# pydata/sparse

Measured on AMD Instinct MI355X. Metric: GCXS x dense SpMM throughput (GFLOP/s), higher is better.
Workload: dtype f32; 1 GPU; GCXS(CSR) 1000000x10000 @ 0.01 (100000000 nnz, int32 idx) in 1 nnz-balanced row block(s) x dense 10000x128 fp32; world_size=1, rows_rank0=1000000, idx_dtype=int32, parallelism=row-block x1, mul_add=fma, nan_warning=deferred, prewarm_products=40, default_settings=NAN_WARNING="sync" (verdict read inside every product), kernel=spmm_tiled (cached block stream)

## Files before the change

sparse_amd/csrc/build.py:

```python
import concurrent.futures as cf
import glob
import os
import shutil
import subprocess
import sys

HERE = os.path.dirname(os.path.abspath(__file__))
PKG = os.path.dirname(HERE)
OUT_DIR = os.path.join(PKG, "_lib")
OBJ_DIR = os.path.join(OUT_DIR, "obj")
LIB = os.path.join(OUT_DIR, "libsparse_amd.so")
ARCH = "gfx950"
CXXFLAGS = [
    f"--offload-arch={ARCH}", "-O3", "-std=c++17", "-fPIC", "-ffp-contract=off",
    "-fno-gpu-rdc", "-Wall", "-Wno-unused-function", "-Wno-unused-variable",
]


def _hipcc():
    for c in (os.environ.get("HIPCC"), shutil.which("hipcc"), "/opt/rocm/bin/hipcc"):
        if c and os.path.exists(c):
            return c
    raise RuntimeError("hipcc not found (need ROCm to build libsparse_amd.so)")


def sources():
    return sorted(glob.glob(os.path.join(HERE, "*.hip")))


def _deps():
    return sorted(glob.glob(os.path.join(HERE, "*.h"))) + sorted(glob.glob(os.path.join(HERE, "*.inc"))) + [
        os.path.join(os.path.dirname(PKG), "include", "sparse_amd.h"), os.path.abspath(__file__)]


def is_stale():
    if not os.path.exists(LIB):
        return True
    t = os.path.getmtime(LIB)
    return any(os.path.getmtime(p) > t for p in sources() + _deps())


def _own_deps(src, obj):
    dep = obj[:-2] + ".d"
    if not os.path.exists(dep):
        return _deps()
    words = open(dep).read().replace("\\\n", " ").split()
    files = [w for w in words[1:] if not w.startswith("/opt/") and not w.startswith("/usr/")]
    if any(not os.path.exists(f) for f in files):
        return _deps()
    return files + [os.path.abspath(__file__)]


NO_SPILL = {"spmm_tiled.hip": "spmm_tiled_kernel"}


def _spills(remarks, needle):
    out, name, sg = [], None, 0
    for ln in remarks.splitlines():
        if "Function Name:" in ln:
            name = ln.split("Function Name:")[1].split()[0]
        elif "SGPRs Spill:" in ln:
            sg = int(ln.split("SGPRs Spill:")[1].split()[0])
        elif "VGPRs Spill:" in ln and name is not None:
            vg = int(ln.split("VGPRs Spill:")[1].split()[0])
            if needle in name and (sg or vg):
                out.append((name, sg, vg))
    return out


def _compile(src, force):
    obj = os.path.join(OBJ_DIR, os.path.basename(src)[:-4] + ".o")
    newest = max(os.path.getmtime(p) for p in [src] + _own_deps(src, obj))
    if not force and os.path.exists(obj) and os.path.getmtime(obj) >= newest:
        return obj, ""
    needle = NO_SPILL.get(os.path.basename(src))
    extra = ["-Rpass-analysis=kernel-resource-usage"] if needle else []
    cmd = [_hipcc(), *CXXFLAGS, *extra, "-MD", "-MF", obj[:-2] + ".d", "-c", src, "-o", obj]
    r = subprocess.run(cmd, capture_output=True, text=True)
    if r.returncode != 0:
        raise RuntimeError(f"hipcc failed for {src}:\n{' '.join(cmd)}\n{r.stdout}\n{r.stderr}")
    if needle:
        bad = _spills(r.stderr, needle)
        if bad:
            os.remove(obj)
            raise RuntimeError(f"{os.path.basename(src)}: the compiler spilled registers in " +
                               ", ".join(f"{n[:60]} ({s} SGPR, {v} VGPR)" for n, s, v in bad[:4]) +
                               " - refused (see NO_SPILL in sparse_amd/csrc/build.py)")
        return obj, "\n".join(ln for ln in r.stderr.splitlines() if "-Rpass-analysis" not in ln and "remark:" not in ln)
    return obj, r.stderr


def build(force=False, verbose=False, jobs=None):
    if not force and not is_stale():
        return LIB
    os.makedirs(OBJ_DIR, exist_ok=True)
    srcs = sources()
    jobs = jobs or min(len(srcs), os.cpu_count() or 1)
    with cf.ThreadPoolExecutor(max_workers=jobs) as ex:
        results = list(ex.map(lambda s: _compile(s, force), srcs))
    objs = [o for o, _ in results]
    if verbose:
        for _, w in results:
            if w.strip():
                print(w, file=sys.stderr)
    cmd = [_hipcc(), f"--offload-arch={ARCH}", "-shared", "-fPIC", "-o", LIB + ".tmp", *objs]
    r = subprocess.run(cmd, capture_output=True, text=True)
    if r.returncode != 0:
        raise RuntimeError(f"link failed:\n{' '.join(cmd)}\n{r.stdout}\n{r.stderr}")
    os.replace(LIB + ".tmp", LIB)
    return LIB


if __name__ == "__main__":
    p = build(force="--force" in sys.argv, verbose=True)
    print(p)
```

sparse_amd/csrc/spmm_tiled.hip:

```cpp
#include "common.h"
#include "spmm_tiled_asm.inc"
#include <stdlib.h>
#include <mutex>
#include <set>

namespace spamd {

constexpr int TL_RG = TL_ASM_RG;
constexpr int TL_WAVES = TL_ASM_WAVES;
#ifndef SPAMD_TL_EXPERIMENTAL
static_assert(TL_RG == 35 && TL_WAVES == 16, "experimental tiled-SpMM geometry: build with -DSPAMD_TL_EXPERIMENTAL");
#endif
constexpr int TL_KB = TL_ASM_KB;
constexpr int TL_NBUF = 2;
__host__ __device__ constexpr int tl_d0(int lc, int lr) { return ((lc >> 1) << 11) | ((lc & 1) << 9) | (2 + 2 * lr); }
constexpr int TL_BLOCK_INTS = 16;

template <typename T>
struct TlFmt;
template <>
struct TlFmt<float> {
  static constexpr int EPB = 8, PANEL = 128;
  __device__ static void put(int* stream, int64_t entry, int d0, float v) {
    int* b = stream + (entry / EPB) * TL_BLOCK_INTS + (entry % EPB) * 2;
    typedef int int2v __attribute__((ext_vector_type(2)));
    int2v e;
    e.x = d0;
    e.y = __builtin_bit_cast(int, v);
    *reinterpret_cast<int2v*>(b) = e;
  }
};
template <>
struct TlFmt<double> {
  static constexpr int EPB = 5, PANEL = 64;
  __device__ static void put(int* stream, int64_t entry, int d0, double v) {
    int* b = stream + (entry / EPB) * TL_BLOCK_INTS;
    const int slot = (int)(entry % EPB);
    const long long bits = __builtin_bit_cast(long long, v);
    b[slot] = d0;
    if (slot == 0) b[5] = 0;
    *reinterpret_cast<long long*>(b + 6 + 2 * slot) = bits;
  }
};
typedef int tl_srd_t __attribute__((ext_vector_type(4)));
constexpr int TL_TILE = TL_KB * 512;
constexpr int TL_LDS = TL_NBUF * TL_TILE;
constexpr int TL_DMA_PER_TILE = TL_TILE / 16 / (TL_WAVES * 64);
static_assert(TL_LDS <= 160 * 1024 && TL_KB % (2 * TL_WAVES) == 0 && TL_DMA_PER_TILE == TL_ASM_DMA_PER_TILE,
              "tile geometry is baked into gen_tiled_asm.py");
constexpr int TL_SLACK_BLOCKS = 68;

#define GRID_STRIDE(i, n)                                                          \
  for (int64_t i = (int64_t)blockIdx.x * blockDim.x + threadIdx.x; i < (n);        \
       i += (int64_t)gridDim.x * blockDim.x)

__global__ void __launch_bounds__(256) tl_keys_kernel(const int64_t* __restrict__ rc_keys, int64_t nnz, int64_t K,
                                                      int64_t ntiles, int64_t* __restrict__ out) {
  GRID_STRIDE(i, nnz) {
    const int64_t k = rc_keys[i];
    const int64_t row = k / K, col = k - row * K;
    const int64_t g = row / TL_RG, lr = row - g * TL_RG, t = col / TL_KB, lc = col - t * TL_KB;
    out[i] = ((g * ntiles + t) * TL_RG + lr) * TL_KB + lc;
  }
}

__global__ void __launch_bounds__(256) tl_seg_start_kernel(const int64_t* __restrict__ keys, int64_t nnz,
                                                           int64_t nseg, int64_t* __restrict__ seg_start) {
  GRID_STRIDE(i, nnz + 1) {
    const int64_t hi = i < nnz ? keys[i] / (TL_RG * TL_KB) : nseg;
    const int64_t lo = i > 0 ? keys[i - 1] / (TL_RG * TL_KB) + 1 : 0;
    for (int64_t s = lo; s <= hi; ++s) seg_start[s] = i;
  }
}

__global__ void __launch_bounds__(256) tl_blocks_kernel(const int64_t* __restrict__ seg_start, int64_t nseg, int epb,
                                                        int64_t* __restrict__ nblk) {
  GRID_STRIDE(s, nseg + 1) {
    nblk[s] = s < nseg ? (seg_start[s + 1] - seg_start[s] + epb - 1) / epb : 0;
  }
}

template <typename T>
__global__ void __launch_bounds__(256) tl_pack_kernel(const int64_t* __restrict__ keys, const T* __restrict__ vals,
                                                      int64_t nnz, const int64_t* __restrict__ seg_start,
                                                      const int64_t* __restrict__ blk_off, int* __restrict__ stream) {
  GRID_STRIDE(i, nnz) {
    const int64_t k = keys[i];
    const int64_t lc = k % TL_KB, r1 = k / TL_KB, lr = r1 % TL_RG, s = r1 / TL_RG;
    const int64_t dst = blk_off[s] * TlFmt<T>::EPB + (i - seg_start[s]);
    TlFmt<T>::put(stream, dst, tl_d0((int)lc, (int)lr), vals[i]);
  }
}

constexpr int TL_DIRECT_MAX_TILES = 256;

template <typename I>
__device__ __forceinline__ int tl_row_of(const int64_t* rs, int64_t e) {
  static_assert(TL_RG <= 128, "seven bisection steps");
  int lo = 0, hi = TL_RG;
#pragma unroll
  for (int it = 0; it < (TL_RG <= 64 ? 6 : 7); ++it) {
    const int mid = (lo + hi) >> 1;
    if (hi - lo > 1) {
      if (rs[mid] <= e) lo = mid; else hi = mid;
    }
  }
  return lo;
}

template <typename I>
__global__ void __launch_bounds__(256) tl_count_kernel(int64_t M, int ntiles, int epb, const I* __restrict__ indices,
                                                       const I* __restrict__ indptr, int64_t* __restrict__ nblk,
                                                       int* __restrict__ flags) {
  __shared__ int cnt[TL_DIRECT_MAX_TILES];
  __shared__ int64_t rs[TL_RG + 1];
  const int tid = threadIdx.x;
  const int64_t r0 = (int64_t)blockIdx.x * TL_RG;
  if (tid <= TL_RG) {
    const int64_t r = r0 + tid;
    rs[tid] = (int64_t)indptr[r < M ? r : M];
  }
  for (int t = tid; t < ntiles; t += 256) cnt[t] = 0;
  __syncthreads();
  const int64_t e0 = rs[0], e1 = rs[TL_RG];
  bool bad = false;
  for (int64_t e = e0 + tid; e < e1; e += 256) {
    const int64_t c = (int64_t)indices[e];
    atomicAdd(&cnt[(int)(c / TL_KB)], 1);
    if (e > e0 && (int64_t)indices[e - 1] > c && rs[tl_row_of<I>(rs, e)] != e) bad = true;
  }
  if (bad) flags[0] = 1;
  __syncthreads();
  for (int t = tid; t < ntiles; t += 256) nblk[(int64_t)blockIdx.x * ntiles + t] = (cnt[t] + epb - 1) / epb;
}

template <typename I, typename T>
__global__ void __launch_bounds__(256) tl_fill_kernel(int64_t M, int ntiles, const T* __restrict__ vals,
                                                      const I* __restrict__ indices, const I* __restrict__ indptr,
                                                      const int64_t* __restrict__ blk_off, int* __restrict__ stream) {
  extern __shared__ int tl_fill_lds[];
  __shared__ int64_t rs[TL_RG + 1];
  int* const before = tl_fill_lds;
  int* const runstart = before + TL_RG * ntiles;
  const int tid = threadIdx.x;
  const int64_t r0 = (int64_t)blockIdx.x * TL_RG;
  if (tid <= TL_RG) {
    const int64_t r = r0 + tid;
    rs[tid] = (int64_t)indptr[r < M ? r : M];
  }
  for (int i = tid; i < TL_RG * ntiles; i += 256) before[i] = 0;
  __syncthreads();
  const int64_t e0 = rs[0], e1 = rs[TL_RG];
  for (int64_t e = e0 + tid; e < e1; e += 256) {
    const int t = (int)((int64_t)indices[e] / TL_KB);
    const int lr = tl_row_of<I>(rs, e);
    atomicAdd(&before[lr * ntiles + t], 1);
    if (e == rs[lr] || (int)((int64_t)indices[e - 1] / TL_KB) != t) runstart[lr * ntiles + t] = (int)(e - e0);
  }
  __syncthreads();
  for (int t = tid; t < ntiles; t += 256) {
    int run = 0;
    for (int lr = 0; lr < TL_RG; ++lr) {
      const int c = before[lr * ntiles + t];
      before[lr * ntiles + t] = run;
      run += c;
    }
  }
  __syncthreads();
  const int64_t* const goff = blk_off + (int64_t)blockIdx.x * ntiles;
  for (int64_t e = e0 + tid; e < e1; e += 256) {
    const int64_t c = (int64_t)indices[e];
    const int t = (int)(c / TL_KB), lc = (int)(c - (int64_t)t * TL_KB);
    const int lr = tl_row_of<I>(rs, e);
    const int64_t dst = goff[t] * TlFmt<T>::EPB + before[lr * ntiles + t] + ((int)(e - e0) - runstart[lr * ntiles + t]);
    TlFmt<T>::put(stream, dst, tl_d0(lc, lr), vals[e]);
  }
}

__host__ __device__ inline int64_t tl_group_first_block(int64_t e0, int64_t g, int64_t ntiles, int64_t epb) {
  return (e0 + g * ntiles * (epb - 1) + epb - 1) / epb;
}

template <typename I, typename T, bool MAPPED>
__global__ void __launch_bounds__(256) tl_inspect_kernel(int64_t M, int ntiles, int64_t groups, const T* __restrict__ vals,
                                                         const I* __restrict__ indices, const I* __restrict__ indptr,
                                                         unsigned long long* __restrict__ state, int* __restrict__ blk_off,
                                                         int* __restrict__ stream, const int* __restrict__ rowmap,
                                                         const int64_t* __restrict__ vstart) {
  extern __shared__ int tl_fill_lds[];
  __shared__ __attribute__((aligned(16))) int64_t rsab[2 * (TL_RG + 1)];
  __shared__ int wtot[5];
  __shared__ int group_bad;
  constexpr int EPB = TlFmt<T>::EPB;
  int* const before = tl_fill_lds;
  int* const runstart = before + TL_RG * ntiles;
  int* const loff = runstart + TL_RG * ntiles;
  const int tid = threadIdx.x;
  const int64_t g = blockIdx.x;
  const int64_t r0 = g * TL_RG;
  if (tid < TL_RG) {
    if constexpr (MAPPED) {
      const int r = rowmap[r0 + tid];
      rsab[2 * (tid)] = r >= 0 ? (int64_t)indptr[r] : 0;
      rsab[2 * (tid) + 1] = r >= 0 ? (int64_t)indptr[r + 1] : 0;
    } else {
      const int64_t r = r0 + tid;
      rsab[2 * (tid)] = (int64_t)indptr[r < M ? r : M];
      rsab[2 * (tid) + 1] = (int64_t)indptr[r + 1 < M ? r + 1 : M];
    }
  }
  for (int i = tid; i < TL_RG * ntiles; i += 256) before[i] = 0;
  if (tid == 0) group_bad = 0;
  __syncthreads();
  const int64_t e0 = MAPPED ? vstart[g] : rsab[2 * (0)], e1 = MAPPED ? vstart[g + 1] : rsab[2 * (TL_RG - 1) + 1];
  bool bad = false;
  constexpr int RPW = (TL_RG + 3) / 4;
  constexpr int TL_PRE = 2;
  const int wv = tid >> 6, lane = tid & 63;
  unsigned cpre[RPW][TL_PRE];
  T vpre[RPW][TL_PRE];
#pragma unroll
  for (int i = 0; i < RPW; ++i) {
    const int lr = wv + 4 * i;
    const int64_t ra = lr < TL_RG ? rsab[2 * (lr)] : 0, rb = lr < TL_RG ? rsab[2 * (lr) + 1] : 0;
#pragma unroll
    for (int p = 0; p < TL_PRE; ++p) {
      const int64_t e = ra + lane + 64 * p;
      cpre[i][p] = e < rb ? (unsigned)indices[e] : 0xffffffffu;
      vpre[i][p] = e < rb ? vals[e] : T(0);
    }
  }
  auto count_one = [&](int lr, int64_t ra, int64_t e, unsigned c, unsigned cp, bool row_start) {
    const int t = (int)(c / (unsigned)TL_KB);
    atomicAdd(&before[lr * ntiles + t], 1);
    if (!row_start && cp > c) bad = true;
    if (row_start || (int)(cp / (unsigned)TL_KB) != t) runstart[lr * ntiles + t] = (int)(e - (MAPPED ? ra : e0));
  };
#pragma unroll
  for (int i = 0; i < RPW; ++i) {
    const int lr = wv + 4 * i;
    if (lr >= TL_RG) break;
    const int64_t ra = rsab[2 * (lr)], rb = rsab[2 * (lr) + 1];
#pragma unroll
    for (int p = 0; p < TL_PRE; ++p) {
      const int64_t e = ra + lane + 64 * p;
      const unsigned c = cpre[i][p];
      unsigned cp = (unsigned)__shfl_up((int)c, 1, 64);
      if (p > 0) {
        const unsigned last = (unsigned)__builtin_amdgcn_readlane((int)cpre[i][p > 0 ? p - 1 : 0], 63);
        if (lane == 0) cp = last;
      }
      if (e < rb) count_one(lr, ra, e, c, cp, p == 0 && lane == 0);
    }
    for (int64_t e = ra + lane + 64 * TL_PRE; e < rb; e += 64)
      count_one(lr, ra, e, (unsigned)indices[e], (unsigned)indices[e - 1], false);
  }
  if (bad) {
    atomicOr(&state[0], 1ull);
    group_bad = 1;
  }
  __syncthreads();
  int nb = 0, cnt_t = 0;
  for (int t = tid; t < ntiles; t += 256) {
    int c[TL_RG];
#pragma unroll
    for (int lr = 0; lr < TL_RG; ++lr) c[lr] = before[lr * ntiles + t];
    int run = 0;
#pragma unroll
    for (int lr = 0; lr < TL_RG; ++lr) {
      before[lr * ntiles + t] = run;
      run += c[lr];
    }
    cnt_t = run;
    nb = (run + EPB - 1) / EPB;
  }
  const int wid = wv;
  int x = nb;
#pragma unroll
  for (int d = 1; d < 64; d <<= 1) {
    const int y = __shfl_up(x, d, 64);
    if (lane >= d) x += y;
  }
  if (lane == 63) wtot[wid] = x;
  __syncthreads();
  int woff = 0;
  for (int w = 0; w < wid; ++w) woff += wtot[w];
  const int gtotal = wtot[0] + wtot[1] + wtot[2] + wtot[3];
  const int my_off = woff + x - nb;
  const int64_t goff = tl_group_first_block(e0, g, ntiles, EPB);
  const int64_t gnext = tl_group_first_block(e1, g + 1, ntiles, EPB);
  if (tid < ntiles) loff[tid] = my_off;
  __syncthreads();
  if (tid < ntiles) blk_off[g * (ntiles + 1) + tid] = (int)(goff + my_off);
  if (tid == 0) blk_off[g * (ntiles + 1) + ntiles] = (int)(goff + gtotal);
  for (int64_t i = (goff + gtotal) * TL_BLOCK_INTS + tid; i < gnext * TL_BLOCK_INTS; i += 256) stream[i] = 0;
  if (group_bad) {
    for (int64_t i = goff * TL_BLOCK_INTS + tid; i < (goff + gtotal) * TL_BLOCK_INTS; i += 256) stream[i] = 0;
    return;
  }
  auto fill_one = [&](int lr, int64_t ra, int64_t e, unsigned c, T v) {
    const int t = (int)(c / (unsigned)TL_KB);
    const int lc = (int)(c - (unsigned)t * (unsigned)TL_KB);
    const int64_t dst = (goff + loff[t]) * EPB + before[lr * ntiles + t] + ((int)(e - (MAPPED ? ra : e0)) - runstart[lr * ntiles + t]);
    TlFmt<T>::put(stream, dst, tl_d0(lc, lr), v);
  };
#pragma unroll
  for (int i = 0; i < RPW; ++i) {
    const int lr = wv + 4 * i;
    if (lr >= TL_RG) break;
    const int64_t ra = rsab[2 * (lr)], rb = rsab[2 * (lr) + 1];
#pragma unroll
    for (int p = 0; p < TL_PRE; ++p) {
      const int64_t e = ra + lane + 64 * p;
      if (e < rb) fill_one(lr, ra, e, cpre[i][p], vpre[i][p]);
    }
    for (int64_t e = ra + lane + 64 * TL_PRE; e < rb; e += 64) fill_one(lr, ra, e, (unsigned)indices[e], vals[e]);
  }
  if (tid < ntiles) {
    const int64_t first = (goff + my_off) * EPB;
    for (int i = cnt_t; i < nb * EPB; ++i) TlFmt<T>::put(stream, first + i, 0, T(0));
  }
}

__device__ __forceinline__ void tl_dma16(unsigned lds_base, const void* src) {
  asm volatile("s_mov_b32 m0, %0\n\ts_nop 0\n\tglobal_load_lds_dwordx4 %1, off"
               :
               : "s"(lds_base), "v"(src)
               : "memory", "m0");
}

template <int MODE>
__device__ __forceinline__ void tl_phases(const int* stream, int t0, int te, int o0, int o1, int o2, int offreg, int obase,
                                          int ntiles, int nfull, int toff, int mask, unsigned m0wave,
                                          unsigned row_step, int voff, tl_srd_t srd, unsigned& soff) {
  const int lane = threadIdx.x & 63;
  const unsigned blo = (unsigned)((uintptr_t)stream & 0xffffffffu), bhi = (unsigned)((uintptr_t)stream >> 32);
  const int lane8 = lane * 8;
#define TL_PHASES_OPERANDS                                                                                        \
  [soff] "+s"(soff)                                                                                               \
  : [blo] "s"(blo), [bhi] "s"(bhi), [t0] "s"(t0), [te] "s"(te), [o0] "s"(o0), [o1] "s"(o1), [o2] "s"(o2),         \
    [obase] "s"(obase), [ntiles] "s"(ntiles), [nfull] "s"(nfull), [m0wave] "s"(m0wave), [step] "s"(row_step),      \
    [toff] "v"(toff), [lane8] "v"(lane8), [mask] "v"(mask), [offreg] "v"(offreg), [voff] "v"(voff), [srd] "s"(srd)  \
  : "memory", "m0", "scc", "vcc", TL_CLOB_SGPR, TL_CLOB_TMP, TL_CLOB_ACC
  if (MODE == 6)
    asm volatile(TL_ASM_PHASES_I32 : TL_PHASES_OPERANDS);
  else if (MODE == 4)
    asm volatile(TL_ASM_PHASES_F64 : TL_PHASES_OPERANDS);
  else if (MODE == 5)
    asm volatile(TL_ASM_PHASES_F64_EXACT : TL_PHASES_OPERANDS);
  else if (MODE == 3)
    asm volatile(TL_ASM_PHASES_EXACT : TL_PHASES_OPERANDS);
  else if (MODE == 1)
    asm volatile(TL_ASM_PHASES_NOFMA : TL_PHASES_OPERANDS);
  else if (MODE == 2)
    asm volatile(TL_ASM_PHASES_NOLDS : TL_PHASES_OPERANDS);
  else
    asm volatile(TL_ASM_PHASES : TL_PHASES_OPERANDS);
#undef TL_PHASES_OPERANDS
}

__device__ __forceinline__ void tl_block_map(unsigned L, int npanels, int nblocks, int& bx, int& by) {
  const unsigned pin = npanels > 1 ? 2u : 1u;
  const unsigned per_chunk = (unsigned)((nblocks + 7) / 8) * 8u * pin;
  const unsigned chunk = L / per_chunk, l = L % per_chunk;
  const unsigned seq = l >> 3;
  by = uniform((int)(chunk * pin + seq % pin));
  bx = uniform((int)((seq / pin) * 8u + (l & 7u)));
}

template <int DBG, int MODE, typename T>
__global__ void __launch_bounds__(TL_WAVES * 64) __attribute__((amdgpu_num_vgpr(TL_ASM_COMP)))
spmm_tiled_kernel(int64_t M, int64_t K, int ntiles, int touch_lines, const int* __restrict__ stream,
                  const int* __restrict__ blk_off, const T* __restrict__ b, int64_t ldb,
                  T* __restrict__ out, int64_t ldo, int last_cols, int npanels, int nblocks, const int* __restrict__ rowmap) {
  constexpr int PANEL = TlFmt<T>::PANEL;
  constexpr int CPL = PANEL / 64;
  extern __shared__ __attribute__((aligned(16))) char lds[];
  const int tid = threadIdx.x;
  const int lane = tid & 63;
  const int wv = uniform(tid >> 6);
  int bx, by;
  tl_block_map(blockIdx.x, npanels, nblocks, bx, by);
  if (bx >= nblocks || by >= npanels) return;
  const int g = bx * TL_WAVES + wv;
  b += (int64_t)by * PANEL;
  out += (int64_t)by * PANEL;

  asm volatile(TL_ASM_ZERO ::: "memory", TL_CLOB_ACC);

  const int nfull = DBG == 2 ? 0 : (int)(K / TL_KB);
  const unsigned row_step = (unsigned)((2 * TL_WAVES) * ldb * (int64_t)sizeof(T));
  const unsigned m0wave = (unsigned)wv * 2048u;
  const uint64_t bbase = (uint64_t)(uintptr_t)b;
  tl_srd_t srd;
  srd[0] = (int)(bbase & 0xffffffffu);
  srd[1] = (int)((bbase >> 32) & 0xffffu);
  srd[2] = (int)0xffffffffu;
  srd[3] = 0x00020000;
  const int voff = (int)((int64_t)(tid >> 5) * ldb * (int64_t)sizeof(T)) + (tid & 31) * 16;
  unsigned soff = 0;
  auto issue_partial = [&](int t) {
#pragma unroll
    for (int i = 0; i < TL_DMA_PER_TILE; ++i) {
      const int e = (i * (TL_WAVES * 64) + tid) * 16;
      int64_t r = (int64_t)t * TL_KB + (e >> 9);
      if (r >= K) r = K - 1;
      tl_dma16(((unsigned)(i * TL_WAVES + wv) * 2u + (unsigned)(t & 1)) * 1024u,
               reinterpret_cast<const char*>(b + r * ldb) + (e & 511));
    }
  };
  const bool has_partial = DBG != 2 && (int64_t)nfull * TL_KB < K;

  if (nfull > 0)
    asm volatile(TL_ASM_TILE0 : [soff] "+s"(soff) : [m0wave] "s"(m0wave), [step] "s"(row_step), [voff] "v"(voff), [srd] "s"(srd) : "memory", "m0", "scc", "vcc", "s89");
  else if (has_partial)
    issue_partial(0);
  asm volatile("s_waitcnt vmcnt(0)" ::: "memory");
  __syncthreads();

  const int* const myoff = blk_off + (int64_t)g * (ntiles + (touch_lines >> 16));
  touch_lines &= 0xffff;
  const int toff = (lane < touch_lines ? lane : touch_lines - 1) * 64;
  int t = 0;
  while (t < ntiles) {
    const int obase = t;
    const int q = obase + lane;
    int offreg = myoff[q < ntiles ? q : ntiles];
    asm volatile("" : "+v"(offreg));
    int te = obase + 61 < ntiles ? obase + 61 : ntiles;
    if (has_partial && t < nfull - 1 && nfull - 1 < te) te = nfull - 1;
    if (has_partial && t == nfull - 1) issue_partial(nfull);
    auto o = [&](int tt) { return wave_bcast(offreg, (tt < ntiles ? tt : ntiles) - obase); };
    const int o0 = o(t), o1 = o(t + 1), o2 = o(t + 2);
    if (t == 0) {
      const int n = o2 - o0, l = lane < n ? lane : 0;
      asm volatile("global_load_dword " TL_ASM_TOUCH ", %0, off" ::"v"(reinterpret_cast<const char*>(stream + (int64_t)o0 * 16) + l * 64)
                   : "memory", TL_ASM_TOUCH);
    }
    tl_phases<MODE>(stream, t, te, o0, o1, o2, offreg, obase, ntiles, nfull, toff, (int)0xfffffe00, m0wave, row_step, voff, srd, soff);
    t = te;
  }
  asm volatile("s_waitcnt vmcnt(0) lgkmcnt(0)" ::: "memory");

  const int64_t row0 = (int64_t)g * TL_RG;
  const int64_t left = M - row0;
  const int nvalid = left <= 0 ? 0 : (left < TL_RG ? (int)left : TL_RG);
  T* const obase_p = out + row0 * ldo + lane * CPL;
  const int64_t stride_bytes = ldo * (int64_t)sizeof(T);
  int bx2, by2;
  tl_block_map(blockIdx.x, npanels, nblocks, bx2, by2);
  const int ncols = (last_cols > 0 && by2 == npanels - 1) ? last_cols : PANEL;
  if (rowmap) {
    const int* const rm = rowmap + (int64_t)g * TL_RG;
    T* const base_p = out + lane * CPL;
    if (lane * CPL + CPL <= ncols)
      asm volatile(TL_ASM_STORE_PERM
                   :
                   : [lo] "v"((unsigned)((uintptr_t)base_p & 0xffffffffu)), [hi] "v"((unsigned)((uintptr_t)base_p >> 32)),
                     [stride] "s"((unsigned)stride_bytes), [rm] "s"(rm)
                   : "memory", "scc", TL_CLOB_SGPR, TL_CLOB_TMP, TL_CLOB_ACC);
    if constexpr (CPL == 2) {
      if (lane * CPL + 1 == ncols)
        asm volatile(TL_ASM_STORE1_PERM
                     :
                     : [lo] "v"((unsigned)((uintptr_t)base_p & 0xffffffffu)), [hi] "v"((unsigned)((uintptr_t)base_p >> 32)),
                       [stride] "s"((unsigned)stride_bytes), [rm] "s"(rm)
                     : "memory", "scc", TL_CLOB_SGPR, TL_CLOB_TMP);
    }
    return;
  }
  if (lane * CPL + CPL <= ncols)
    asm volatile(TL_ASM_STORE
                 :
                 : [lo] "v"((unsigned)((uintptr_t)obase_p & 0xffffffffu)), [hi] "v"((unsigned)((uintptr_t)obase_p >> 32)),
                   [stride] "s"(stride_bytes), [n] "s"(nvalid)
                 : "memory", "scc", "s36", TL_ASM_BASE, TL_ASM_TOUCH, TL_CLOB_ACC);
  if constexpr (CPL == 2) {
    if (lane * CPL + 1 == ncols)
      asm volatile(TL_ASM_STORE1
                   :
                   : [lo] "v"((unsigned)((uintptr_t)obase_p & 0xffffffffu)), [hi] "v"((unsigned)((uintptr_t)obase_p >> 32)),
                     [stride] "s"(stride_bytes), [n] "s"(nvalid)
                   : "memory", "scc", "s36", TL_ASM_BASE, TL_ASM_TOUCH);
  }
}

static int64_t tl_grid_groups(int64_t M) { return ceil_div(ceil_div(M, (int64_t)TL_RG), (int64_t)TL_WAVES) * TL_WAVES; }

}

using namespace spamd;

static int tl_epb(int val_dtype) { return val_dtype == SPAMD_F32 ? TlFmt<float>::EPB : (val_dtype == SPAMD_F64 ? TlFmt<double>::EPB : 0); }

extern "C" int spamd_spmm_tiled_params(int val_dtype, int* rows_per_group, int* tile_rows, int* groups_per_block,
                                       int* entries_per_block, int* slack_blocks, int* direct_max_tiles,
                                       int* panel_cols) {
  if (!tl_epb(val_dtype)) return SPAMD_ETYPE;
  if (direct_max_tiles) *direct_max_tiles = TL_DIRECT_MAX_TILES;
  if (rows_per_group) *rows_per_group = TL_RG;
  if (tile_rows) *tile_rows = TL_KB;
  if (groups_per_block) *groups_per_block = TL_WAVES;
  if (entries_per_block) *entries_per_block = tl_epb(val_dtype);
  if (slack_blocks) *slack_blocks = TL_SLACK_BLOCKS;
  if (panel_cols) *panel_cols = val_dtype == SPAMD_F32 ? TlFmt<float>::PANEL : TlFmt<double>::PANEL;
  return 0;
}

static unsigned tl_blocks_for(int64_t n) {
  int64_t blocks = ceil_div(n, (int64_t)256);
  if (blocks > 8192) blocks = 8192;
  if (blocks < 1) blocks = 1;
  return (unsigned)blocks;
}

extern "C" int spamd_spmm_tiled_keys(int64_t nnz, const int64_t* rowcol_keys, int64_t K, int64_t* tiled_keys,
                                     void* stream) {
  if (nnz < 0 || K <= 0) return SPAMD_EINVAL;
  if (nnz == 0) return 0;
  hipLaunchKernelGGL(tl_keys_kernel, dim3(tl_blocks_for(nnz)), dim3(256), 0, (hipStream_t)stream, rowcol_keys, nnz, K,
                     ceil_div(K, (int64_t)TL_KB), tiled_keys);
  return launch_status();
}

extern "C" int spamd_spmm_tiled_lists(int val_dtype, int64_t nnz, const int64_t* tiled_keys_sorted, int64_t M, int64_t K,
                                      int64_t* seg_start, int64_t* nblk, void* stream) {
  if (nnz < 0 || M < 0 || K <= 0) return SPAMD_EINVAL;
  if (!tl_epb(val_dtype)) return SPAMD_ETYPE;
  const int64_t nseg = tl_grid_groups(M) * ceil_div(K, (int64_t)TL_KB);
  hipLaunchKernelGGL(tl_seg_start_kernel, dim3(tl_blocks_for(nnz + 1)), dim3(256), 0, (hipStream_t)stream,
                     tiled_keys_sorted, nnz, nseg, seg_start);
  hipLaunchKernelGGL(tl_blocks_kernel, dim3(tl_blocks_for(nseg + 1)), dim3(256), 0, (hipStream_t)stream, seg_start,
                     nseg, tl_epb(val_dtype), nblk);
  return launch_status();
}

static int tl_clear_blocks(int64_t total_blocks, int* blocks, hipStream_t s) {
  return (int)hipMemsetAsync(blocks, 0, (size_t)(total_blocks + TL_SLACK_BLOCKS) * TL_BLOCK_INTS * sizeof(int), s);
}

extern "C" int spamd_spmm_tiled_pack(int val_dtype, int64_t nnz, const int64_t* tiled_keys_sorted, const void* vals_sorted,
                                     const int64_t* seg_start, const int64_t* blk_off, int64_t total_blocks,
                                     int* blocks, void* stream) {
  if (nnz < 0 || total_blocks < 0) return SPAMD_EINVAL;
  if (!tl_epb(val_dtype)) return SPAMD_ETYPE;
  int rc = tl_clear_blocks(total_blocks, blocks, (hipStream_t)stream);
  if (rc) return rc;
  if (nnz == 0) return 0;
  if (val_dtype == SPAMD_F32)
    hipLaunchKernelGGL(tl_pack_kernel<float>, dim3(tl_blocks_for(nnz)), dim3(256), 0, (hipStream_t)stream, tiled_keys_sorted,
                       (const float*)vals_sorted, nnz, seg_start, blk_off, blocks);
  else
    hipLaunchKernelGGL(tl_pack_kernel<double>, dim3(tl_blocks_for(nnz)), dim3(256), 0, (hipStream_t)stream, tiled_keys_sorted,
                       (const double*)vals_sorted, nnz, seg_start, blk_off, blocks);
  return launch_status();
}

extern "C" int spamd_spmm_tiled_count(int val_dtype, int idx_dtype, int64_t M, int64_t K, const void* a_indices,
                                      const void* a_indptr, int64_t* nblk, int* flags, void* stream) {
  if (M < 0 || K <= 0) return SPAMD_EINVAL;
  if (!tl_epb(val_dtype)) return SPAMD_ETYPE;
  const int64_t ntiles = ceil_div(K, (int64_t)TL_KB);
  if (ntiles > TL_DIRECT_MAX_TILES) return SPAMD_EINVAL;
  const int64_t groups = tl_grid_groups(M);
  hipError_t e = hipMemsetAsync(flags, 0, sizeof(int), (hipStream_t)stream);
  if (e != hipSuccess) return (int)e;
  e = hipMemsetAsync(nblk + groups * ntiles, 0, sizeof(int64_t), (hipStream_t)stream);
  if (e != hipSuccess) return (int)e;
  if (groups == 0) return 0;
  SPAMD_DISPATCH_IDX(idx_dtype, I, hipLaunchKernelGGL(tl_count_kernel<I>, dim3((unsigned)groups), dim3(256), 0,
                                                    (hipStream_t)stream, M, (int)ntiles, tl_epb(val_dtype),
                                                    (const I*)a_indices, (const I*)a_indptr, nblk, flags))
  return launch_status();
}

template <typename I, typename T>
static int tl_launch_fill(int64_t M, int64_t ntiles, const T* a_data, const I* a_indices, const I* a_indptr,
                          const int64_t* blk_off, int* blocks, hipStream_t s) {
  const int lds = (int)(2 * TL_RG * ntiles * sizeof(int));
  auto kern = &tl_fill_kernel<I, T>;
  if (lds > 48 * 1024) {
    hipError_t e = hipFuncSetAttribute(reinterpret_cast<const void*>(kern), hipFuncAttributeMaxDynamicSharedMemorySize, lds);
    if (e != hipSuccess) return (int)e;
  }
  hipLaunchKernelGGL(kern, dim3((unsigned)tl_grid_groups(M)), dim3(256), lds, s, M, (int)ntiles, a_data, a_indices, a_indptr,
                     blk_off, blocks);
  return launch_status();
}

extern "C" int spamd_spmm_tiled_fill(int val_dtype, int idx_dtype, int64_t M, int64_t K, const void* a_data,
                                     const void* a_indices, const void* a_indptr, const int64_t* blk_off,
                                     int64_t total_blocks, int* blocks, void* stream) {
  if (M < 0 || K <= 0 || total_blocks < 0) return SPAMD_EINVAL;
  if (!tl_epb(val_dtype)) return SPAMD_ETYPE;
  const int64_t ntiles = ceil_div(K, (int64_t)TL_KB);
  if (ntiles > TL_DIRECT_MAX_TILES) return SPAMD_EINVAL;
  int rc = tl_clear_blocks(total_blocks, blocks, (hipStream_t)stream);
  if (rc) return rc;
  if (tl_grid_groups(M) == 0) return 0;
  SPAMD_DISPATCH_IDX(idx_dtype, I, {
    if (val_dtype == SPAMD_F32)
      return tl_launch_fill<I, float>(M, ntiles, (const float*)a_data, (const I*)a_indices, (const I*)a_indptr, blk_off,
                                      blocks, (hipStream_t)stream);
    return tl_launch_fill<I, double>(M, ntiles, (const double*)a_data, (const I*)a_indices, (const I*)a_indptr, blk_off,
                                     blocks, (hipStream_t)stream);
  })
  return SPAMD_ETYPE;
}

template <typename I, typename T>
static int tl_launch_inspect(int64_t M, int64_t ntiles, const T* a_data, const I* a_indices, const I* a_indptr,
                             unsigned long long* state, int* blk_off, int* blocks, hipStream_t s, int64_t map_groups = 0,
                             const int* rowmap = nullptr, const int64_t* vstart = nullptr) {
  const int64_t groups = rowmap ? map_groups : tl_grid_groups(M);
  const int lds = (int)((2 * TL_RG * ntiles + ntiles + 1) * sizeof(int));
  auto kern = rowmap ? &tl_inspect_kernel<I, T, true> : &tl_inspect_kernel<I, T, false>;
  if (lds > 48 * 1024) {
    hipError_t e = hipFuncSetAttribute(reinterpret_cast<const void*>(kern), hipFuncAttributeMaxDynamicSharedMemorySize, lds);
    if (e != hipSuccess) return (int)e;
  }
  hipLaunchKernelGGL(kern, dim3((unsigned)groups), dim3(256), lds, s, M, (int)ntiles, groups, a_data, a_indices, a_indptr,
                     state, blk_off, blocks, rowmap, vstart);
  return launch_status();
}

constexpr int TL_MAP_CLASSES = 6;
__host__ __device__ inline int tl_map_slots(int c) { return c == 5 ? TL_RG : (1 << c); }
__host__ __device__ inline int tl_map_class(int64_t len, int64_t cap) {
  return len > cap / 2 ? 0 : (len > cap / 4 ? 1 : (len > cap / 8 ? 2 : (len > cap / 16 ? 3 : (len > cap / 32 ? 4 : 5))));
}

template <typename I>
__global__ void __launch_bounds__(256) tl_map_stats_kernel(int64_t M, int64_t cap, int64_t maxlen, const I* __restrict__ indptr,
                                                           int64_t* __restrict__ keys, int* __restrict__ rows,
                                                           unsigned long long* __restrict__ stats) {
  __shared__ unsigned cnt[TL_MAP_CLASSES];
  if (threadIdx.x < TL_MAP_CLASSES) cnt[threadIdx.x] = 0;
  __syncthreads();
  const int lane = threadIdx.x & 63;
  const int64_t stride = (int64_t)gridDim.x * blockDim.x;
  for (int64_t r0 = (int64_t)blockIdx.x * blockDim.x; r0 < M; r0 += stride) {
    const int64_t r = r0 + threadIdx.x;
    int c = -1;
    if (r < M) {
      const int64_t len = (int64_t)indptr[r + 1] - (int64_t)indptr[r];
      c = tl_map_class(len, cap);
      keys[r] = len < maxlen ? maxlen - len : 0;
      rows[r] = (int)r;
    }
#pragma unroll
    for (int k = 0; k < TL_MAP_CLASSES; ++k) {
      const unsigned long long m = __ballot(c == k);
      if (lane == 0 && m) atomicAdd(&cnt[k], (unsigned)__popcll(m));
    }
  }
  __syncthreads();
  if (threadIdx.x < TL_MAP_CLASSES && cnt[threadIdx.x]) atomicAdd(&stats[threadIdx.x], (unsigned long long)cnt[threadIdx.x]);
}

template <typename I>
__global__ void __launch_bounds__(256) tl_map_skew_kernel(int64_t M, const I* __restrict__ indptr,
                                                          unsigned long long* __restrict__ stats) {
  const int64_t groups = (M + TL_RG - 1) / TL_RG;
  unsigned long long mine = 0;
  GRID_STRIDE(g, groups) {
    const int64_t r = g * TL_RG, e = r + TL_RG < M ? r + TL_RG : M;
    const unsigned long long load = (unsigned long long)((int64_t)indptr[e] - (int64_t)indptr[r]);
    mine = load > mine ? load : mine;
  }
#pragma unroll
  for (int d = 32; d > 0; d >>= 1) {
    const unsigned long long y = __shfl_xor(mine, d, 64);
    mine = y > mine ? y : mine;
  }
  if ((threadIdx.x & 63) == 0 && mine) atomicMax(&stats[6], mine);
}

struct TlMapPlan {
  int64_t cstart[TL_MAP_CLASSES];
  int64_t gstart[TL_MAP_CLASSES];
};

template <typename I>
__global__ void __launch_bounds__(256) tl_map_build_kernel(int64_t M, int64_t cap, const I* __restrict__ indptr,
                                                           const int* __restrict__ rows_sorted, TlMapPlan plan,
                                                           int* __restrict__ rowmap, unsigned long long* __restrict__ gload) {
  GRID_STRIDE(i, M) {
    const int r = rows_sorted[i];
    const int64_t len = (int64_t)indptr[r + 1] - (int64_t)indptr[r];
    const int c = tl_map_class(len, cap);
    const int64_t j = i - plan.cstart[c];
    const int sl = tl_map_slots(c);
    const int64_t group = plan.gstart[c] + j / sl;
    rowmap[group * TL_RG + (int)(j % sl)] = r;
    if (len) atomicAdd(&gload[group], (unsigned long long)len);
  }
}

extern "C" int spamd_spmm_tiled_inspect(int val_dtype, int idx_dtype, int64_t M, int64_t K, const void* a_data,
                                        const void* a_indices, const void* a_indptr, void* state, int* blk_off, int* blocks,
                                        void* stream) {
  if (M < 0 || K <= 0) return SPAMD_EINVAL;
  if (!tl_epb(val_dtype)) return SPAMD_ETYPE;
  const int64_t ntiles = ceil_div(K, (int64_t)TL_KB);
  if (ntiles > TL_DIRECT_MAX_TILES) return SPAMD_EINVAL;
  const int64_t groups = tl_grid_groups(M);
  hipError_t e = hipMemsetAsync(state, 0, sizeof(unsigned long long), (hipStream_t)stream);
  if (e != hipSuccess) return (int)e;
  if (groups == 0) return 0;
  SPAMD_DISPATCH_IDX(idx_dtype, I, {
    if (val_dtype == SPAMD_F32)
      return tl_launch_inspect<I, float>(M, ntiles, (const float*)a_data, (const I*)a_indices, (const I*)a_indptr,
                                         (unsigned long long*)state, blk_off, blocks, (hipStream_t)stream);
    return tl_launch_inspect<I, double>(M, ntiles, (const double*)a_data, (const I*)a_indices, (const I*)a_indptr,
                                        (unsigned long long*)state, blk_off, blocks, (hipStream_t)stream);
  })
  return SPAMD_ETYPE;
}

extern "C" int spamd_spmm_tiled_map_stats(int idx_dtype, int64_t M, int64_t K, int64_t cap, const void* a_indptr, int64_t* keys,
                                          int* rows, int64_t* stats, void* stream) {
  if (M < 0 || M >= ((int64_t)1 << 31) || K <= 0 || cap < 32 || (cap & (cap - 1)) || (keys != nullptr) != (rows != nullptr) || !stats)
    return SPAMD_EINVAL;
  hipStream_t s = (hipStream_t)stream;
  if (hipError_t e = hipMemsetAsync(stats, 0, 8 * sizeof(int64_t), s); e != hipSuccess) return (int)e;
  if (M == 0) return 0;
  SPAMD_DISPATCH_IDX(idx_dtype, I, {
    hipLaunchKernelGGL((tl_map_skew_kernel<I>), dim3(tl_blocks_for(ceil_div(M, (int64_t)TL_RG))), dim3(256), 0, s, M, (const I*)a_indptr,
                       (unsigned long long*)stats);
    if (keys)
      hipLaunchKernelGGL((tl_map_stats_kernel<I>), dim3(tl_blocks_for(M)), dim3(256), 0, s, M, cap, K, (const I*)a_indptr, keys, rows,
                         (unsigned long long*)stats);
    return launch_status();
  })
  return SPAMD_ETYPE;
}

extern "C" int64_t spamd_spmm_tiled_map_groups(const int64_t* class_counts) {
  if (!class_counts) return -1;
  int64_t g = 0;
  for (int c = 0; c < TL_MAP_CLASSES; ++c) {
    if (class_counts[c] < 0) return -1;
    g += ceil_div(class_counts[c], (int64_t)tl_map_slots(c));
  }
  return ceil_div(g, (int64_t)TL_WAVES) * TL_WAVES;
}

extern "C" int spamd_spmm_tiled_map_build(int idx_dtype, int64_t M, int64_t cap, const void* a_indptr, const int* rows_sorted,
                                          const int64_t* class_counts, int* rowmap, int64_t* gload, void* stream) {
  const int64_t groups = spamd_spmm_tiled_map_groups(class_counts);
  if (M < 0 || M >= ((int64_t)1 << 31) || groups <= 0 || !rowmap || !gload || !rows_sorted) return SPAMD_EINVAL;
  hipStream_t s = (hipStream_t)stream;
  if (hipError_t e = hipMemsetAsync(rowmap, 0xff, (size_t)(groups * TL_RG + 16) * sizeof(int), s); e != hipSuccess) return (int)e;
  if (hipError_t e = hipMemsetAsync(gload, 0, (size_t)(groups + 1) * sizeof(int64_t), s); e != hipSuccess) return (int)e;
  TlMapPlan plan;
  int64_t pos = 0, g = 0;
  for (int c = 0; c < TL_MAP_CLASSES; ++c) {
    plan.cstart[c] = pos;
    plan.gstart[c] = g;
    pos += class_counts[c];
    g += ceil_div(class_counts[c], (int64_t)tl_map_slots(c));
  }
  if (pos != M) return SPAMD_EINVAL;
  if (M == 0) return 0;
  SPAMD_DISPATCH_IDX(idx_dtype, I, {
    hipLaunchKernelGGL((tl_map_build_kernel<I>), dim3(tl_blocks_for(M)), dim3(256), 0, s, M, cap, (const I*)a_indptr, rows_sorted,
                       plan, rowmap, (unsigned long long*)gload);
    return launch_status();
  })
  return SPAMD_ETYPE;
}

extern "C" int spamd_spmm_tiled_inspect_mapped(int val_dtype, int idx_dtype, int64_t M, int64_t K, int64_t groups,
                                               const void* a_data, const void* a_indices, const void* a_indptr,
                                               const int* rowmap, const int64_t* vstart, void* state, int* blk_off, int* blocks,
                                               void* stream) {
  if (M < 0 || K <= 0 || groups <= 0 || groups % TL_WAVES || !rowmap || !vstart) return SPAMD_EINVAL;
  if (!tl_epb(val_dtype)) return SPAMD_ETYPE;
  const int64_t ntiles = ceil_div(K, (int64_t)TL_KB);
  if (ntiles > TL_DIRECT_MAX_TILES) return SPAMD_EINVAL;
  hipError_t e = hipMemsetAsync(state, 0, sizeof(unsigned long long), (hipStream_t)stream);
  if (e != hipSuccess) return (int)e;
  SPAMD_DISPATCH_IDX(idx_dtype, I, {
    if (val_dtype == SPAMD_F32)
      return tl_launch_inspect<I, float>(M, ntiles, (const float*)a_data, (const I*)a_indices, (const I*)a_indptr,
                                         (unsigned long long*)state, blk_off, blocks, (hipStream_t)stream, groups, rowmap, vstart);
    return tl_launch_inspect<I, double>(M, ntiles, (const double*)a_data, (const I*)a_indices, (const I*)a_indptr,
// ... 691 lines not shown
```

sparse_amd/csrc/spmm_tiled_asm.inc:

```

#define TL_ASM_KB 160
#define TL_ASM_DMA_PER_TILE 5
#define TL_ASM_RG 35
#define TL_ASM_WAVES 16
#define TL_ASM_COMP 22
#define TL_ASM_TOUCH "v23"
#define TL_ASM_BASE "v22"

#define TL_ASM_PHASES \
  "s_mov_b32 s39, 0\n\t" \
  "s_mov_b32 s90, %[t0]\n\t" \
  "s_mov_b32 s91, %[o0]\n\t" \
  "s_mov_b32 s92, %[o1]\n\t" \
  "s_mov_b32 s93, %[o2]\n\t" \
  "s_add_u32 s88, s90, 1\n\t" \
  "s_and_b32 s88, s88, 1\n\t" \
  "s_lshl_b32 s88, s88, 10\n\t" \
  "s_add_u32 s89, s88, %[m0wave]\n\t" \
  "s_and_b32 s88, s90, 1\n\t" \
  "s_lshl_b32 s88, s88, 10\n\t" \
  "v_or_b32 v22, s88, %[lane8]\n\t" \
  "s_lshl_b32 s36, s91, 6\n\t" \
  "s_lshr_b32 s37, s91, 26\n\t" \
  "s_add_u32 s36, s36, %[blo]\n\t" \
  "s_addc_u32 s37, s37, %[bhi]\n\t" \
  "s_sub_u32 s88, s92, s91\n\t" \
  "s_cmp_lt_u32 s88, 3\n\t" \
  "s_cbranch_scc1 22f\n\t" \
  "s_load_dwordx16 s[40:55], s[36:37], 0x0\n\t" \
  "s_load_dwordx16 s[56:71], s[36:37], 0x40\n\t" \
  "s_load_dwordx16 s[72:87], s[36:37], 0x80\n\t" \
  "20:\n\t" \
  "1:\n\t" \
  "s_sub_u32 s38, s92, s91\n\t" \
  "s_add_u32 s88, s90, 1\n\t" \
  "s_cmp_lt_u32 s88, %[nfull]\n\t" \
  "s_cselect_b64 vcc, 31, 0\n\t" \
  "s_cmp_eq_u32 s38, 0\n\t" \
  "s_cbranch_scc1 12f\n\t" \
  "s_cbranch_vccz 6f\n\t" \
  "s_mov_b32 m0, s89\n\t" \
  "s_add_u32 s89, s89, 0x8000\n\t" \
  "buffer_load_dwordx4 %[voff], %[srd], %[soff] offen lds\n\t" \
  "s_add_u32 %[soff], %[soff], %[step]\n\t" \
  "s_lshr_b64 vcc, vcc, 1\n\t" \
  "6:\n\t" \
  "s_cbranch_vccz 6f\n\t" \
  "s_mov_b32 m0, s89\n\t" \
  "s_add_u32 s89, s89, 0x8000\n\t" \
  "buffer_load_dwordx4 %[voff], %[srd], %[soff] offen lds\n\t" \
  "s_add_u32 %[soff], %[soff], %[step]\n\t" \
  "s_lshr_b64 vcc, vcc, 1\n\t" \
  "6:\n\t" \
  "s_waitcnt lgkmcnt(0)\n\t" \
  "v_and_or_b32 v40, s40, %[mask], v22\n\t" \
  "v_and_or_b32 v42, s42, %[mask], v22\n\t" \
  "v_and_or_b32 v44, s44, %[mask], v22\n\t" \
  "v_and_or_b32 v46, s46, %[mask], v22\n\t" \
  "ds_read_b64 v[40:41], v40\n\t" \
  "ds_read_b64 v[42:43], v42\n\t" \
  "ds_read_b64 v[44:45], v44\n\t" \
  "ds_read_b64 v[46:47], v46\n\t" \
  "v_and_or_b32 v48, s48, %[mask], v22\n\t" \
  "v_and_or_b32 v50, s50, %[mask], v22\n\t" \
  "v_and_or_b32 v52, s52, %[mask], v22\n\t" \
  "v_and_or_b32 v54, s54, %[mask], v22\n\t" \
  "ds_read_b64 v[48:49], v48\n\t" \
  "ds_read_b64 v[50:51], v50\n\t" \
  "ds_read_b64 v[52:53], v52\n\t" \
  "ds_read_b64 v[54:55], v54\n\t" \
  "s_waitcnt lgkmcnt(0)\n\t" \
  "s_cmp_lt_u32 s38, 4\n\t" \
  "s_cbranch_scc1 40f\n\t" \
  "s_sub_u32 s38, s38, 3\n\t" \
  "11:\n\t" \
  "s_sub_u32 s38, s38, 1\n\t" \
  "s_cbranch_scc1 30f\n\t" \
  "v_and_or_b32 v24, s56, %[mask], v22\n\t" \
  "v_and_or_b32 v26, s58, %[mask], v22\n\t" \
  "v_and_or_b32 v28, s60, %[mask], v22\n\t" \
  "v_and_or_b32 v30, s62, %[mask], v22\n\t" \
  "ds_read_b64 v[24:25], v24\n\t" \
  "ds_read_b64 v[26:27], v26\n\t" \
  "ds_read_b64 v[28:29], v28\n\t" \
  "ds_read_b64 v[30:31], v30\n\t" \
  "v_and_or_b32 v32, s64, %[mask], v22\n\t" \
  "v_and_or_b32 v34, s66, %[mask], v22\n\t" \
  "v_and_or_b32 v36, s68, %[mask], v22\n\t" \
  "v_and_or_b32 v38, s70, %[mask], v22\n\t" \
  "ds_read_b64 v[32:33], v32\n\t" \
  "ds_read_b64 v[34:35], v34\n\t" \
  "ds_read_b64 v[36:37], v36\n\t" \
  "ds_read_b64 v[38:39], v38\n\t" \
  "s_set_gpr_idx_on s40, gpr_idx(SRC2,DST)\n\t" \
  "v_pk_fma_f32 v[56:57], v[40:41], s[40:41], v[56:57] op_sel:[0,1,0] op_sel_hi:[1,1,1]\n\t" \
  "s_set_gpr_idx_idx s42\n\t" \
  "v_pk_fma_f32 v[56:57], v[42:43], s[42:43], v[56:57] op_sel:[0,1,0] op_sel_hi:[1,1,1]\n\t" \
  "s_set_gpr_idx_idx s44\n\t" \
  "v_pk_fma_f32 v[56:57], v[44:45], s[44:45], v[56:57] op_sel:[0,1,0] op_sel_hi:[1,1,1]\n\t" \
  "s_set_gpr_idx_idx s46\n\t" \
  "v_pk_fma_f32 v[56:57], v[46:47], s[46:47], v[56:57] op_sel:[0,1,0] op_sel_hi:[1,1,1]\n\t" \
  "s_set_gpr_idx_idx s48\n\t" \
  "v_pk_fma_f32 v[56:57], v[48:49], s[48:49], v[56:57] op_sel:[0,1,0] op_sel_hi:[1,1,1]\n\t" \
  "s_set_gpr_idx_idx s50\n\t" \
  "v_pk_fma_f32 v[56:57], v[50:51], s[50:51], v[56:57] op_sel:[0,1,0] op_sel_hi:[1,1,1]\n\t" \
  "s_set_gpr_idx_idx s52\n\t" \
  "v_pk_fma_f32 v[56:57], v[52:53], s[52:53], v[56:57] op_sel:[0,1,0] op_sel_hi:[1,1,1]\n\t" \
  "s_set_gpr_idx_idx s54\n\t" \
  "v_pk_fma_f32 v[56:57], v[54:55], s[54:55], v[56:57] op_sel:[0,1,0] op_sel_hi:[1,1,1]\n\t" \
  "s_set_gpr_idx_off\n\t" \
  "s_waitcnt lgkmcnt(0)\n\t" \
  "s_load_dwordx16 s[40:55], s[36:37], 0xc0\n\t" \
  "s_cbranch_vccz 6f\n\t" \
  "s_mov_b32 m0, s89\n\t" \
  "s_add_u32 s89, s89, 0x8000\n\t" \
  "buffer_load_dwordx4 %[voff], %[srd], %[soff] offen lds\n\t" \
  "s_add_u32 %[soff], %[soff], %[step]\n\t" \
  "s_lshr_b64 vcc, vcc, 1\n\t" \
  "6:\n\t" \
  "s_sub_u32 s38, s38, 1\n\t" \
  "s_cbranch_scc1 31f\n\t" \
  "v_and_or_b32 v40, s72, %[mask], v22\n\t" \
  "v_and_or_b32 v42, s74, %[mask], v22\n\t" \
  "v_and_or_b32 v44, s76, %[mask], v22\n\t" \
  "v_and_or_b32 v46, s78, %[mask], v22\n\t" \
  "ds_read_b64 v[40:41], v40\n\t" \
  "ds_read_b64 v[42:43], v42\n\t" \
  "ds_read_b64 v[44:45], v44\n\t" \
  "ds_read_b64 v[46:47], v46\n\t" \
  "v_and_or_b32 v48, s80, %[mask], v22\n\t" \
  "v_and_or_b32 v50, s82, %[mask], v22\n\t" \
  "v_and_or_b32 v52, s84, %[mask], v22\n\t" \
  "v_and_or_b32 v54, s86, %[mask], v22\n\t" \
  "ds_read_b64 v[48:49], v48\n\t" \
  "ds_read_b64 v[50:51], v50\n\t" \
  "ds_read_b64 v[52:53], v52\n\t" \
  "ds_read_b64 v[54:55], v54\n\t" \
  "s_set_gpr_idx_on s56, gpr_idx(SRC2,DST)\n\t" \
  "v_pk_fma_f32 v[56:57], v[24:25], s[56:57], v[56:57] op_sel:[0,1,0] op_sel_hi:[1,1,1]\n\t" \
  "s_set_gpr_idx_idx s58\n\t" \
  "v_pk_fma_f32 v[56:57], v[26:27], s[58:59], v[56:57] op_sel:[0,1,0] op_sel_hi:[1,1,1]\n\t" \
  "s_set_gpr_idx_idx s60\n\t" \
  "v_pk_fma_f32 v[56:57], v[28:29], s[60:61], v[56:57] op_sel:[0,1,0] op_sel_hi:[1,1,1]\n\t" \
  "s_set_gpr_idx_idx s62\n\t" \
  "v_pk_fma_f32 v[56:57], v[30:31], s[62:63], v[56:57] op_sel:[0,1,0] op_sel_hi:[1,1,1]\n\t" \
  "s_set_gpr_idx_idx s64\n\t" \
  "v_pk_fma_f32 v[56:57], v[32:33], s[64:65], v[56:57] op_sel:[0,1,0] op_sel_hi:[1,1,1]\n\t" \
  "s_set_gpr_idx_idx s66\n\t" \
  "v_pk_fma_f32 v[56:57], v[34:35], s[66:67], v[56:57] op_sel:[0,1,0] op_sel_hi:[1,1,1]\n\t" \
  "s_set_gpr_idx_idx s68\n\t" \
  "v_pk_fma_f32 v[56:57], v[36:37], s[68:69], v[56:57] op_sel:[0,1,0] op_sel_hi:[1,1,1]\n\t" \
  "s_set_gpr_idx_idx s70\n\t" \
  "v_pk_fma_f32 v[56:57], v[38:39], s[70:71], v[56:57] op_sel:[0,1,0] op_sel_hi:[1,1,1]\n\t" \
  "s_set_gpr_idx_off\n\t" \
  "s_waitcnt lgkmcnt(0)\n\t" \
  "s_load_dwordx16 s[56:71], s[36:37], 0x100\n\t" \
  "s_cbranch_vccz 6f\n\t" \
  "s_mov_b32 m0, s89\n\t" \
  "s_add_u32 s89, s89, 0x8000\n\t" \
  "buffer_load_dwordx4 %[voff], %[srd], %[soff] offen lds\n\t" \
  "s_add_u32 %[soff], %[soff], %[step]\n\t" \
  "s_lshr_b64 vcc, vcc, 1\n\t" \
  "6:\n\t" \
  "s_sub_u32 s38, s38, 1\n\t" \
  "s_cbranch_scc1 32f\n\t" \
  "v_and_or_b32 v24, s40, %[mask], v22\n\t" \
  "v_and_or_b32 v26, s42, %[mask], v22\n\t" \
  "v_and_or_b32 v28, s44, %[mask], v22\n\t" \
  "v_and_or_b32 v30, s46, %[mask], v22\n\t" \
  "ds_read_b64 v[24:25], v24\n\t" \
  "ds_read_b64 v[26:27], v26\n\t" \
  "ds_read_b64 v[28:29], v28\n\t" \
  "ds_read_b64 v[30:31], v30\n\t" \
  "v_and_or_b32 v32, s48, %[mask], v22\n\t" \
  "v_and_or_b32 v34, s50, %[mask], v22\n\t" \
  "v_and_or_b32 v36, s52, %[mask], v22\n\t" \
  "v_and_or_b32 v38, s54, %[mask], v22\n\t" \
  "ds_read_b64 v[32:33], v32\n\t" \
  "ds_read_b64 v[34:35], v34\n\t" \
  "ds_read_b64 v[36:37], v36\n\t" \
  "ds_read_b64 v[38:39], v38\n\t" \
  "s_set_gpr_idx_on s72, gpr_idx(SRC2,DST)\n\t" \
  "v_pk_fma_f32 v[56:57], v[40:41], s[72:73], v[56:57] op_sel:[0,1,0] op_sel_hi:[1,1,1]\n\t" \
  "s_set_gpr_idx_idx s74\n\t" \
  "v_pk_fma_f32 v[56:57], v[42:43], s[74:75], v[56:57] op_sel:[0,1,0] op_sel_hi:[1,1,1]\n\t" \
  "s_set_gpr_idx_idx s76\n\t" \
  "v_pk_fma_f32 v[56:57], v[44:45], s[76:77], v[56:57] op_sel:[0,1,0] op_sel_hi:[1,1,1]\n\t" \
  "s_set_gpr_idx_idx s78\n\t" \
  "v_pk_fma_f32 v[56:57], v[46:47], s[78:79], v[56:57] op_sel:[0,1,0] op_sel_hi:[1,1,1]\n\t" \
  "s_set_gpr_idx_idx s80\n\t" \
  "v_pk_fma_f32 v[56:57], v[48:49], s[80:81], v[56:57] op_sel:[0,1,0] op_sel_hi:[1,1,1]\n\t" \
  "s_set_gpr_idx_idx s82\n\t" \
  "v_pk_fma_f32 v[56:57], v[50:51], s[82:83], v[56:57] op_sel:[0,1,0] op_sel_hi:[1,1,1]\n\t" \
  "s_set_gpr_idx_idx s84\n\t" \
  "v_pk_fma_f32 v[56:57], v[52:53], s[84:85], v[56:57] op_sel:[0,1,0] op_sel_hi:[1,1,1]\n\t" \
  "s_set_gpr_idx_idx s86\n\t" \
  "v_pk_fma_f32 v[56:57], v[54:55], s[86:87], v[56:57] op_sel:[0,1,0] op_sel_hi:[1,1,1]\n\t" \
  "s_set_gpr_idx_off\n\t" \
  "s_waitcnt lgkmcnt(0)\n\t" \
  "s_load_dwordx16 s[72:87], s[36:37], 0x140\n\t" \
  "s_cbranch_vccz 6f\n\t" \
  "s_mov_b32 m0, s89\n\t" \
  "s_add_u32 s89, s89, 0x8000\n\t" \
  "buffer_load_dwordx4 %[voff], %[srd], %[soff] offen lds\n\t" \
  "s_add_u32 %[soff], %[soff], %[step]\n\t" \
  "s_lshr_b64 vcc, vcc, 1\n\t" \
  "6:\n\t" \
  "s_sub_u32 s38, s38, 1\n\t" \
  "s_cbranch_scc1 33f\n\t" \
  "v_and_or_b32 v40, s56, %[mask], v22\n\t" \
  "v_and_or_b32 v42, s58, %[mask], v22\n\t" \
  "v_and_or_b32 v44, s60, %[mask], v22\n\t" \
  "v_and_or_b32 v46, s62, %[mask], v22\n\t" \
  "ds_read_b64 v[40:41], v40\n\t" \
  "ds_read_b64 v[42:43], v42\n\t" \
  "ds_read_b64 v[44:45], v44\n\t" \
  "ds_read_b64 v[46:47], v46\n\t" \
  "v_and_or_b32 v48, s64, %[mask], v22\n\t" \
  "v_and_or_b32 v50, s66, %[mask], v22\n\t" \
  "v_and_or_b32 v52, s68, %[mask], v22\n\t" \
  "v_and_or_b32 v54, s70, %[mask], v22\n\t" \
  "ds_read_b64 v[48:49], v48\n\t" \
  "ds_read_b64 v[50:51], v50\n\t" \
  "ds_read_b64 v[52:53], v52\n\t" \
  "ds_read_b64 v[54:55], v54\n\t" \
  "s_set_gpr_idx_on s40, gpr_idx(SRC2,DST)\n\t" \
  "v_pk_fma_f32 v[56:57], v[24:25], s[40:41], v[56:57] op_sel:[0,1,0] op_sel_hi:[1,1,1]\n\t" \
  "s_set_gpr_idx_idx s42\n\t" \
  "v_pk_fma_f32 v[56:57], v[26:27], s[42:43], v[56:57] op_sel:[0,1,0] op_sel_hi:[1,1,1]\n\t" \
  "s_set_gpr_idx_idx s44\n\t" \
  "v_pk_fma_f32 v[56:57], v[28:29], s[44:45], v[56:57] op_sel:[0,1,0] op_sel_hi:[1,1,1]\n\t" \
  "s_set_gpr_idx_idx s46\n\t" \
  "v_pk_fma_f32 v[56:57], v[30:31], s[46:47], v[56:57] op_sel:[0,1,0] op_sel_hi:[1,1,1]\n\t" \
  "s_set_gpr_idx_idx s48\n\t" \
  "v_pk_fma_f32 v[56:57], v[32:33], s[48:49], v[56:57] op_sel:[0,1,0] op_sel_hi:[1,1,1]\n\t" \
  "s_set_gpr_idx_idx s50\n\t" \
  "v_pk_fma_f32 v[56:57], v[34:35], s[50:51], v[56:57] op_sel:[0,1,0] op_sel_hi:[1,1,1]\n\t" \
  "s_set_gpr_idx_idx s52\n\t" \
  "v_pk_fma_f32 v[56:57], v[36:37], s[52:53], v[56:57] op_sel:[0,1,0] op_sel_hi:[1,1,1]\n\t" \
  "s_set_gpr_idx_idx s54\n\t" \
  "v_pk_fma_f32 v[56:57], v[38:39], s[54:55], v[56:57] op_sel:[0,1,0] op_sel_hi:[1,1,1]\n\t" \
  "s_set_gpr_idx_off\n\t" \
  "s_waitcnt lgkmcnt(0)\n\t" \
  "s_load_dwordx16 s[40:55], s[36:37], 0x180\n\t" \
  "s_cbranch_vccz 6f\n\t" \
  "s_mov_b32 m0, s89\n\t" \
  "s_add_u32 s89, s89, 0x8000\n\t" \
  "buffer_load_dwordx4 %[voff], %[srd], %[soff] offen lds\n\t" \
  "s_add_u32 %[soff], %[soff], %[step]\n\t" \
  "s_lshr_b64 vcc, vcc, 1\n\t" \
  "6:\n\t" \
  "s_sub_u32 s38, s38, 1\n\t" \
  "s_cbranch_scc1 34f\n\t" \
  "v_and_or_b32 v24, s72, %[mask], v22\n\t" \
  "v_and_or_b32 v26, s74, %[mask], v22\n\t" \
  "v_and_or_b32 v28, s76, %[mask], v22\n\t" \
  "v_and_or_b32 v30, s78, %[mask], v22\n\t" \
  "ds_read_b64 v[24:25], v24\n\t" \
  "ds_read_b64 v[26:27], v26\n\t" \
  "ds_read_b64 v[28:29], v28\n\t" \
  "ds_read_b64 v[30:31], v30\n\t" \
  "v_and_or_b32 v32, s80, %[mask], v22\n\t" \
  "v_and_or_b32 v34, s82, %[mask], v22\n\t" \
  "v_and_or_b32 v36, s84, %[mask], v22\n\t" \
  "v_and_or_b32 v38, s86, %[mask], v22\n\t" \
  "ds_read_b64 v[32:33], v32\n\t" \
  "ds_read_b64 v[34:35], v34\n\t" \
  "ds_read_b64 v[36:37], v36\n\t" \
  "ds_read_b64 v[38:39], v38\n\t" \
  "s_set_gpr_idx_on s56, gpr_idx(SRC2,DST)\n\t" \
  "v_pk_fma_f32 v[56:57], v[40:41], s[56:57], v[56:57] op_sel:[0,1,0] op_sel_hi:[1,1,1]\n\t" \
  "s_set_gpr_idx_idx s58\n\t" \
  "v_pk_fma_f32 v[56:57], v[42:43], s[58:59], v[56:57] op_sel:[0,1,0] op_sel_hi:[1,1,1]\n\t" \
  "s_set_gpr_idx_idx s60\n\t" \
  "v_pk_fma_f32 v[56:57], v[44:45], s[60:61], v[56:57] op_sel:[0,1,0] op_sel_hi:[1,1,1]\n\t" \
  "s_set_gpr_idx_idx s62\n\t" \
  "v_pk_fma_f32 v[56:57], v[46:47], s[62:63], v[56:57] op_sel:[0,1,0] op_sel_hi:[1,1,1]\n\t" \
  "s_set_gpr_idx_idx s64\n\t" \
  "v_pk_fma_f32 v[56:57], v[48:49], s[64:65], v[56:57] op_sel:[0,1,0] op_sel_hi:[1,1,1]\n\t" \
  "s_set_gpr_idx_idx s66\n\t" \
  "v_pk_fma_f32 v[56:57], v[50:51], s[66:67], v[56:57] op_sel:[0,1,0] op_sel_hi:[1,1,1]\n\t" \
  "s_set_gpr_idx_idx s68\n\t" \
  "v_pk_fma_f32 v[56:57], v[52:53], s[68:69], v[56:57] op_sel:[0,1,0] op_sel_hi:[1,1,1]\n\t" \
  "s_set_gpr_idx_idx s70\n\t" \
  "v_pk_fma_f32 v[56:57], v[54:55], s[70:71], v[56:57] op_sel:[0,1,0] op_sel_hi:[1,1,1]\n\t" \
  "s_set_gpr_idx_off\n\t" \
  "s_waitcnt lgkmcnt(0)\n\t" \
  "s_load_dwordx16 s[56:71], s[36:37], 0x1c0\n\t" \
  "s_cbranch_vccz 6f\n\t" \
  "s_mov_b32 m0, s89\n\t" \
  "s_add_u32 s89, s89, 0x8000\n\t" \
  "buffer_load_dwordx4 %[voff], %[srd], %[soff] offen lds\n\t" \
  "s_add_u32 %[soff], %[soff], %[step]\n\t" \
  "s_lshr_b64 vcc, vcc, 1\n\t" \
  "6:\n\t" \
  "s_sub_u32 s38, s38, 1\n\t" \
  "s_cbranch_scc1 35f\n\t" \
  "v_and_or_b32 v40, s40, %[mask], v22\n\t" \
  "v_and_or_b32 v42, s42, %[mask], v22\n\t" \
  "v_and_or_b32 v44, s44, %[mask], v22\n\t" \
  "v_and_or_b32 v46, s46, %[mask], v22\n\t" \
  "ds_read_b64 v[40:41], v40\n\t" \
  "ds_read_b64 v[42:43], v42\n\t" \
  "ds_read_b64 v[44:45], v44\n\t" \
  "ds_read_b64 v[46:47], v46\n\t" \
  "v_and_or_b32 v48, s48, %[mask], v22\n\t" \
  "v_and_or_b32 v50, s50, %[mask], v22\n\t" \
  "v_and_or_b32 v52, s52, %[mask], v22\n\t" \
  "v_and_or_b32 v54, s54, %[mask], v22\n\t" \
  "ds_read_b64 v[48:49], v48\n\t" \
// ... 6095 lines not shown
  "8:\n\t" \
  "s_set_gpr_idx_on s56, gpr_idx(SRC1,DST)\n\t" \
  "v_add_u32 v56, v24, v56\n\t" \
  "v_add_u32 v57, v25, v57\n\t" \
  "s_set_gpr_idx_idx s58\n\t" \
  "v_add_u32 v56, v26, v56\n\t" \
  "v_add_u32 v57, v27, v57\n\t" \
  "s_set_gpr_idx_idx s60\n\t" \
  "v_add_u32 v56, v28, v56\n\t" \
  "v_add_u32 v57, v29, v57\n\t" \
  "s_set_gpr_idx_idx s62\n\t" \
  "v_add_u32 v56, v30, v56\n\t" \
  "v_add_u32 v57, v31, v57\n\t" \
  "s_cmp_eq_u32 s64, 0\n\t" \
  "s_cbranch_scc1 8f\n\t" \
  "s_set_gpr_idx_idx s64\n\t" \
  "v_add_u32 v56, v32, v56\n\t" \
  "v_add_u32 v57, v33, v57\n\t" \
  "s_set_gpr_idx_idx s66\n\t" \
  "v_add_u32 v56, v34, v56\n\t" \
  "v_add_u32 v57, v35, v57\n\t" \
  "s_set_gpr_idx_idx s68\n\t" \
  "v_add_u32 v56, v36, v56\n\t" \
  "v_add_u32 v57, v37, v57\n\t" \
  "s_set_gpr_idx_idx s70\n\t" \
  "v_add_u32 v56, v38, v56\n\t" \
  "v_add_u32 v57, v39, v57\n\t" \
  "8:\n\t" \
  "s_set_gpr_idx_off\n\t" \
  "s_branch 12f\n\t" \
  "40:\n\t" \
  "s_cmp_lt_u32 s38, 2\n\t" \
  "s_cbranch_scc1 7f\n\t" \
  "v_and_or_b32 v24, s56, %[mask], v22\n\t" \
  "v_and_or_b32 v26, s58, %[mask], v22\n\t" \
  "v_and_or_b32 v28, s60, %[mask], v22\n\t" \
  "v_and_or_b32 v30, s62, %[mask], v22\n\t" \
  "ds_read_b64 v[24:25], v24\n\t" \
  "ds_read_b64 v[26:27], v26\n\t" \
  "ds_read_b64 v[28:29], v28\n\t" \
  "ds_read_b64 v[30:31], v30\n\t" \
  "v_and_or_b32 v32, s64, %[mask], v22\n\t" \
  "v_and_or_b32 v34, s66, %[mask], v22\n\t" \
  "v_and_or_b32 v36, s68, %[mask], v22\n\t" \
  "v_and_or_b32 v38, s70, %[mask], v22\n\t" \
  "ds_read_b64 v[32:33], v32\n\t" \
  "ds_read_b64 v[34:35], v34\n\t" \
  "ds_read_b64 v[36:37], v36\n\t" \
  "ds_read_b64 v[38:39], v38\n\t" \
  "7:\n\t" \
  "v_mul_lo_u32 v40, v40, s41\n\t" \
  "v_mul_lo_u32 v41, v41, s41\n\t" \
  "v_mul_lo_u32 v42, v42, s43\n\t" \
  "v_mul_lo_u32 v43, v43, s43\n\t" \
  "v_mul_lo_u32 v44, v44, s45\n\t" \
  "v_mul_lo_u32 v45, v45, s45\n\t" \
  "v_mul_lo_u32 v46, v46, s47\n\t" \
  "v_mul_lo_u32 v47, v47, s47\n\t" \
  "v_mul_lo_u32 v48, v48, s49\n\t" \
  "v_mul_lo_u32 v49, v49, s49\n\t" \
  "v_mul_lo_u32 v50, v50, s51\n\t" \
  "v_mul_lo_u32 v51, v51, s51\n\t" \
  "v_mul_lo_u32 v52, v52, s53\n\t" \
  "v_mul_lo_u32 v53, v53, s53\n\t" \
  "v_mul_lo_u32 v54, v54, s55\n\t" \
  "v_mul_lo_u32 v55, v55, s55\n\t" \
  "s_set_gpr_idx_on s40, gpr_idx(SRC1,DST)\n\t" \
  "v_add_u32 v56, v40, v56\n\t" \
  "v_add_u32 v57, v41, v57\n\t" \
  "s_set_gpr_idx_idx s42\n\t" \
  "v_add_u32 v56, v42, v56\n\t" \
  "v_add_u32 v57, v43, v57\n\t" \
  "s_set_gpr_idx_idx s44\n\t" \
  "v_add_u32 v56, v44, v56\n\t" \
  "v_add_u32 v57, v45, v57\n\t" \
  "s_set_gpr_idx_idx s46\n\t" \
  "v_add_u32 v56, v46, v56\n\t" \
  "v_add_u32 v57, v47, v57\n\t" \
  "s_set_gpr_idx_idx s48\n\t" \
  "v_add_u32 v56, v48, v56\n\t" \
  "v_add_u32 v57, v49, v57\n\t" \
  "s_set_gpr_idx_idx s50\n\t" \
  "v_add_u32 v56, v50, v56\n\t" \
  "v_add_u32 v57, v51, v57\n\t" \
  "s_set_gpr_idx_idx s52\n\t" \
  "v_add_u32 v56, v52, v56\n\t" \
  "v_add_u32 v57, v53, v57\n\t" \
  "s_set_gpr_idx_idx s54\n\t" \
  "v_add_u32 v56, v54, v56\n\t" \
  "v_add_u32 v57, v55, v57\n\t" \
  "s_set_gpr_idx_off\n\t" \
  "s_waitcnt lgkmcnt(0)\n\t" \
  "s_cbranch_vccz 6f\n\t" \
  "s_mov_b32 m0, s89\n\t" \
  "s_add_u32 s89, s89, 0x8000\n\t" \
  "buffer_load_dwordx4 %[voff], %[srd], %[soff] offen lds\n\t" \
  "s_add_u32 %[soff], %[soff], %[step]\n\t" \
  "s_lshr_b64 vcc, vcc, 1\n\t" \
  "6:\n\t" \
  "s_cmp_lt_u32 s38, 2\n\t" \
  "s_cbranch_scc1 12f\n\t" \
  "s_cmp_lt_u32 s38, 3\n\t" \
  "s_cbranch_scc1 7f\n\t" \
  "v_and_or_b32 v40, s72, %[mask], v22\n\t" \
  "v_and_or_b32 v42, s74, %[mask], v22\n\t" \
  "v_and_or_b32 v44, s76, %[mask], v22\n\t" \
  "v_and_or_b32 v46, s78, %[mask], v22\n\t" \
  "ds_read_b64 v[40:41], v40\n\t" \
  "ds_read_b64 v[42:43], v42\n\t" \
  "ds_read_b64 v[44:45], v44\n\t" \
  "ds_read_b64 v[46:47], v46\n\t" \
  "v_and_or_b32 v48, s80, %[mask], v22\n\t" \
  "v_and_or_b32 v50, s82, %[mask], v22\n\t" \
  "v_and_or_b32 v52, s84, %[mask], v22\n\t" \
  "v_and_or_b32 v54, s86, %[mask], v22\n\t" \
  "ds_read_b64 v[48:49], v48\n\t" \
  "ds_read_b64 v[50:51], v50\n\t" \
  "ds_read_b64 v[52:53], v52\n\t" \
  "ds_read_b64 v[54:55], v54\n\t" \
  "7:\n\t" \
  "v_mul_lo_u32 v24, v24, s57\n\t" \
  "v_mul_lo_u32 v25, v25, s57\n\t" \
  "v_mul_lo_u32 v26, v26, s59\n\t" \
  "v_mul_lo_u32 v27, v27, s59\n\t" \
  "v_mul_lo_u32 v28, v28, s61\n\t" \
  "v_mul_lo_u32 v29, v29, s61\n\t" \
  "v_mul_lo_u32 v30, v30, s63\n\t" \
  "v_mul_lo_u32 v31, v31, s63\n\t" \
  "v_mul_lo_u32 v32, v32, s65\n\t" \
  "v_mul_lo_u32 v33, v33, s65\n\t" \
  "v_mul_lo_u32 v34, v34, s67\n\t" \
  "v_mul_lo_u32 v35, v35, s67\n\t" \
  "v_mul_lo_u32 v36, v36, s69\n\t" \
  "v_mul_lo_u32 v37, v37, s69\n\t" \
  "v_mul_lo_u32 v38, v38, s71\n\t" \
  "v_mul_lo_u32 v39, v39, s71\n\t" \
  "s_set_gpr_idx_on s56, gpr_idx(SRC1,DST)\n\t" \
  "v_add_u32 v56, v24, v56\n\t" \
  "v_add_u32 v57, v25, v57\n\t" \
  "s_set_gpr_idx_idx s58\n\t" \
  "v_add_u32 v56, v26, v56\n\t" \
  "v_add_u32 v57, v27, v57\n\t" \
  "s_set_gpr_idx_idx s60\n\t" \
  "v_add_u32 v56, v28, v56\n\t" \
  "v_add_u32 v57, v29, v57\n\t" \
  "s_set_gpr_idx_idx s62\n\t" \
  "v_add_u32 v56, v30, v56\n\t" \
  "v_add_u32 v57, v31, v57\n\t" \
  "s_set_gpr_idx_idx s64\n\t" \
  "v_add_u32 v56, v32, v56\n\t" \
  "v_add_u32 v57, v33, v57\n\t" \
  "s_set_gpr_idx_idx s66\n\t" \
  "v_add_u32 v56, v34, v56\n\t" \
  "v_add_u32 v57, v35, v57\n\t" \
  "s_set_gpr_idx_idx s68\n\t" \
  "v_add_u32 v56, v36, v56\n\t" \
  "v_add_u32 v57, v37, v57\n\t" \
  "s_set_gpr_idx_idx s70\n\t" \
  "v_add_u32 v56, v38, v56\n\t" \
  "v_add_u32 v57, v39, v57\n\t" \
  "s_set_gpr_idx_off\n\t" \
  "s_waitcnt lgkmcnt(0)\n\t" \
  "s_cbranch_vccz 6f\n\t" \
  "s_mov_b32 m0, s89\n\t" \
  "s_add_u32 s89, s89, 0x8000\n\t" \
  "buffer_load_dwordx4 %[voff], %[srd], %[soff] offen lds\n\t" \
  "s_add_u32 %[soff], %[soff], %[step]\n\t" \
  "s_lshr_b64 vcc, vcc, 1\n\t" \
  "6:\n\t" \
  "s_cmp_lt_u32 s38, 3\n\t" \
  "s_cbranch_scc1 12f\n\t" \
  "v_mul_lo_u32 v40, v40, s73\n\t" \
  "v_mul_lo_u32 v41, v41, s73\n\t" \
  "v_mul_lo_u32 v42, v42, s75\n\t" \
  "v_mul_lo_u32 v43, v43, s75\n\t" \
  "v_mul_lo_u32 v44, v44, s77\n\t" \
  "v_mul_lo_u32 v45, v45, s77\n\t" \
  "v_mul_lo_u32 v46, v46, s79\n\t" \
  "v_mul_lo_u32 v47, v47, s79\n\t" \
  "v_mul_lo_u32 v48, v48, s81\n\t" \
  "v_mul_lo_u32 v49, v49, s81\n\t" \
  "v_mul_lo_u32 v50, v50, s83\n\t" \
  "v_mul_lo_u32 v51, v51, s83\n\t" \
  "v_mul_lo_u32 v52, v52, s85\n\t" \
  "v_mul_lo_u32 v53, v53, s85\n\t" \
  "v_mul_lo_u32 v54, v54, s87\n\t" \
  "v_mul_lo_u32 v55, v55, s87\n\t" \
  "s_set_gpr_idx_on s72, gpr_idx(SRC1,DST)\n\t" \
  "v_add_u32 v56, v40, v56\n\t" \
  "v_add_u32 v57, v41, v57\n\t" \
  "s_set_gpr_idx_idx s74\n\t" \
  "v_add_u32 v56, v42, v56\n\t" \
  "v_add_u32 v57, v43, v57\n\t" \
  "s_set_gpr_idx_idx s76\n\t" \
  "v_add_u32 v56, v44, v56\n\t" \
  "v_add_u32 v57, v45, v57\n\t" \
  "s_set_gpr_idx_idx s78\n\t" \
  "v_add_u32 v56, v46, v56\n\t" \
  "v_add_u32 v57, v47, v57\n\t" \
  "s_set_gpr_idx_idx s80\n\t" \
  "v_add_u32 v56, v48, v56\n\t" \
  "v_add_u32 v57, v49, v57\n\t" \
  "s_set_gpr_idx_idx s82\n\t" \
  "v_add_u32 v56, v50, v56\n\t" \
  "v_add_u32 v57, v51, v57\n\t" \
  "s_set_gpr_idx_idx s84\n\t" \
  "v_add_u32 v56, v52, v56\n\t" \
  "v_add_u32 v57, v53, v57\n\t" \
  "s_set_gpr_idx_idx s86\n\t" \
  "v_add_u32 v56, v54, v56\n\t" \
  "v_add_u32 v57, v55, v57\n\t" \
  "s_set_gpr_idx_off\n\t" \
  "s_cbranch_vccz 6f\n\t" \
  "s_mov_b32 m0, s89\n\t" \
  "s_add_u32 s89, s89, 0x8000\n\t" \
  "buffer_load_dwordx4 %[voff], %[srd], %[soff] offen lds\n\t" \
  "s_add_u32 %[soff], %[soff], %[step]\n\t" \
  "s_lshr_b64 vcc, vcc, 1\n\t" \
  "6:\n\t" \
  "12:\n\t" \
  "13:\n\t" \
  "s_cbranch_vccz 14f\n\t" \
  "s_mov_b32 m0, s89\n\t" \
  "s_add_u32 s89, s89, 0x8000\n\t" \
  "buffer_load_dwordx4 %[voff], %[srd], %[soff] offen lds\n\t" \
  "s_add_u32 %[soff], %[soff], %[step]\n\t" \
  "s_lshr_b64 vcc, vcc, 1\n\t" \
  "s_branch 13b\n\t" \
  "14:\n\t" \
  "s_add_u32 s88, s90, 1\n\t" \
  "s_cmp_lt_u32 s88, %[te]\n\t" \
  "s_cbranch_scc0 21f\n\t" \
  "s_lshl_b32 s36, s92, 6\n\t" \
  "s_lshr_b32 s37, s92, 26\n\t" \
  "s_add_u32 s36, s36, %[blo]\n\t" \
  "s_addc_u32 s37, s37, %[bhi]\n\t" \
  "s_sub_u32 s88, s93, s92\n\t" \
  "s_cmp_lt_u32 s88, 3\n\t" \
  "s_cbranch_scc1 23f\n\t" \
  "s_load_dwordx16 s[40:55], s[36:37], 0x0\n\t" \
  "s_load_dwordx16 s[56:71], s[36:37], 0x40\n\t" \
  "s_load_dwordx16 s[72:87], s[36:37], 0x80\n\t" \
  "21:\n\t" \
  "s_add_u32 s38, s90, 3\n\t" \
  "s_min_u32 s38, s38, %[ntiles]\n\t" \
  "s_sub_u32 s38, s38, %[obase]\n\t" \
  "s_lshl_b32 s94, s93, 6\n\t" \
  "s_lshr_b32 s95, s93, 26\n\t" \
  "s_add_u32 s94, s94, %[blo]\n\t" \
  "s_addc_u32 s95, s95, %[bhi]\n\t" \
  "v_readlane_b32 s88, %[offreg], s38\n\t" \
  "s_mov_b32 s91, s92\n\t" \
  "s_mov_b32 s92, s93\n\t" \
  "v_xor_b32 v22, 0x400, v22\n\t" \
  "s_sub_u32 s89, s89, 0x28000\n\t" \
  "s_xor_b32 s89, s89, 0x400\n\t" \
  "global_load_dword v23, %[toff], s[94:95]\n\t" \
  "s_mov_b32 s93, s88\n\t" \
  "s_waitcnt vmcnt(1)\n\t" \
  "s_barrier\n\t" \
  "s_add_u32 s90, s90, 1\n\t" \
  "s_cmp_lt_u32 s90, %[te]\n\t" \
  "s_cbranch_scc1 1b\n\t" \
  "s_waitcnt lgkmcnt(0)\n\t" \
  "s_branch 29f\n\t" \
  "22:\n\t" \
  "s_cmp_eq_u32 s88, 0\n\t" \
  "s_cbranch_scc1 20b\n\t" \
  "s_load_dwordx16 s[40:55], s[36:37], 0x0\n\t" \
  "s_cmp_lt_u32 s88, 2\n\t" \
  "s_cbranch_scc1 20b\n\t" \
  "s_load_dwordx16 s[56:71], s[36:37], 0x40\n\t" \
  "s_branch 20b\n\t" \
  "23:\n\t" \
  "s_cmp_eq_u32 s88, 0\n\t" \
  "s_cbranch_scc1 21b\n\t" \
  "s_load_dwordx16 s[40:55], s[36:37], 0x0\n\t" \
  "s_cmp_lt_u32 s88, 2\n\t" \
  "s_cbranch_scc1 21b\n\t" \
  "s_load_dwordx16 s[56:71], s[36:37], 0x40\n\t" \
  "s_branch 21b\n\t" \
  "29:\n\t"

#define TL_ASM_TILE0 \
  "s_mov_b32 s89, %[m0wave]\n\t" \
  "s_mov_b64 vcc, 31\n\t" \
  "13:\n\t" \
  "s_cbranch_vccz 14f\n\t" \
  "s_mov_b32 m0, s89\n\t" \
  "s_add_u32 s89, s89, 0x8000\n\t" \
  "buffer_load_dwordx4 %[voff], %[srd], %[soff] offen lds\n\t" \
  "s_add_u32 %[soff], %[soff], %[step]\n\t" \
  "s_lshr_b64 vcc, vcc, 1\n\t" \
  "s_branch 13b\n\t" \
  "14:\n\t"

#define TL_ASM_STORE \
  "v_mov_b32 v22, %[lo]\n\t" \
  "v_mov_b32 v23, %[hi]\n\t" \
  "s_mov_b32 s36, 0\n\t" \
  "s_cmp_ge_i32 s36, %[n]\n\t" \
  "s_cbranch_scc1 9f\n\t" \
  "global_store_dwordx2 v[22:23], v[58:59], off nt\n\t" \
  "v_lshl_add_u64 v[22:23], %[stride], 0, v[22:23]\n\t" \
  "s_add_i32 s36, s36, 1\n\t" \
  "s_cmp_ge_i32 s36, %[n]\n\t" \
  "s_cbranch_scc1 9f\n\t" \
  "global_store_dwordx2 v[22:23], v[60:61], off nt\n\t" \
  "v_lshl_add_u64 v[22:23], %[stride], 0, v[22:23]\n\t" \
  "s_add_i32 s36, s36, 1\n\t" \
  "s_cmp_ge_i32 s36, %[n]\n\t" \
  "s_cbranch_scc1 9f\n\t" \
  "global_store_dwordx2 v[22:23], v[62:63], off nt\n\t" \
  "v_lshl_add_u64 v[22:23], %[stride], 0, v[22:23]\n\t" \
  "s_add_i32 s36, s36, 1\n\t" \
  "s_cmp_ge_i32 s36, %[n]\n\t" \
  "s_cbranch_scc1 9f\n\t" \
  "global_store_dwordx2 v[22:23], v[64:65], off nt\n\t" \
  "v_lshl_add_u64 v[22:23], %[stride], 0, v[22:23]\n\t" \
  "s_add_i32 s36, s36, 1\n\t" \
  "s_cmp_ge_i32 s36, %[n]\n\t" \
  "s_cbranch_scc1 9f\n\t" \
  "global_store_dwordx2 v[22:23], v[66:67], off nt\n\t" \
  "v_lshl_add_u64 v[22:23], %[stride], 0, v[22:23]\n\t" \
  "s_add_i32 s36, s36, 1\n\t" \
  "s_cmp_ge_i32 s36, %[n]\n\t" \
  "s_cbranch_scc1 9f\n\t" \
  "global_store_dwordx2 v[22:23], v[68:69], off nt\n\t" \
  "v_lshl_add_u64 v[22:23], %[stride], 0, v[22:23]\n\t" \
  "s_add_i32 s36, s36, 1\n\t" \
  "s_cmp_ge_i32 s36, %[n]\n\t" \
  "s_cbranch_scc1 9f\n\t" \
  "global_store_dwordx2 v[22:23], v[70:71], off nt\n\t" \
  "v_lshl_add_u64 v[22:23], %[stride], 0, v[22:23]\n\t" \
  "s_add_i32 s36, s36, 1\n\t" \
  "s_cmp_ge_i32 s36, %[n]\n\t" \
  "s_cbranch_scc1 9f\n\t" \
  "global_store_dwordx2 v[22:23], v[72:73], off nt\n\t" \
  "v_lshl_add_u64 v[22:23], %[stride], 0, v[22:23]\n\t" \
  "s_add_i32 s36, s36, 1\n\t" \
  "s_cmp_ge_i32 s36, %[n]\n\t" \
  "s_cbranch_scc1 9f\n\t" \
  "global_store_dwordx2 v[22:23], v[74:75], off nt\n\t" \
  "v_lshl_add_u64 v[22:23], %[stride], 0, v[22:23]\n\t" \
  "s_add_i32 s36, s36, 1\n\t" \
  "s_cmp_ge_i32 s36, %[n]\n\t" \
  "s_cbranch_scc1 9f\n\t" \
  "global_store_dwordx2 v[22:23], v[76:77], off nt\n\t" \
  "v_lshl_add_u64 v[22:23], %[stride], 0, v[22:23]\n\t" \
  "s_add_i32 s36, s36, 1\n\t" \
  "s_cmp_ge_i32 s36, %[n]\n\t" \
  "s_cbranch_scc1 9f\n\t" \
  "global_store_dwordx2 v[22:23], v[78:79], off nt\n\t" \
  "v_lshl_add_u64 v[22:23], %[stride], 0, v[22:23]\n\t" \
  "s_add_i32 s36, s36, 1\n\t" \
  "s_cmp_ge_i32 s36, %[n]\n\t" \
  "s_cbranch_scc1 9f\n\t" \
  "global_store_dwordx2 v[22:23], v[80:81], off nt\n\t" \
  "v_lshl_add_u64 v[22:23], %[stride], 0, v[22:23]\n\t" \
  "s_add_i32 s36, s36, 1\n\t" \
  "s_cmp_ge_i32 s36, %[n]\n\t" \
  "s_cbranch_scc1 9f\n\t" \
  "global_store_dwordx2 v[22:23], v[82:83], off nt\n\t" \
  "v_lshl_add_u64 v[22:23], %[stride], 0, v[22:23]\n\t" \
  "s_add_i32 s36, s36, 1\n\t" \
  "s_cmp_ge_i32 s36, %[n]\n\t" \
  "s_cbranch_scc1 9f\n\t" \
  "global_store_dwordx2 v[22:23], v[84:85], off nt\n\t" \
  "v_lshl_add_u64 v[22:23], %[stride], 0, v[22:23]\n\t" \
  "s_add_i32 s36, s36, 1\n\t" \
  "s_cmp_ge_i32 s36, %[n]\n\t" \
  "s_cbranch_scc1 9f\n\t" \
  "global_store_dwordx2 v[22:23], v[86:87], off nt\n\t" \
  "v_lshl_add_u64 v[22:23], %[stride], 0, v[22:23]\n\t" \
  "s_add_i32 s36, s36, 1\n\t" \
  "s_cmp_ge_i32 s36, %[n]\n\t" \
  "s_cbranch_scc1 9f\n\t" \
  "global_store_dwordx2 v[22:23], v[88:89], off nt\n\t" \
  "v_lshl_add_u64 v[22:23], %[stride], 0, v[22:23]\n\t" \
  "s_add_i32 s36, s36, 1\n\t" \
  "s_cmp_ge_i32 s36, %[n]\n\t" \
  "s_cbranch_scc1 9f\n\t" \
  "global_store_dwordx2 v[22:23], v[90:91], off nt\n\t" \
  "v_lshl_add_u64 v[22:23], %[stride], 0, v[22:23]\n\t" \
  "s_add_i32 s36, s36, 1\n\t" \
  "s_cmp_ge_i32 s36, %[n]\n\t" \
  "s_cbranch_scc1 9f\n\t" \
  "global_store_dwordx2 v[22:23], v[92:93], off nt\n\t" \
  "v_lshl_add_u64 v[22:23], %[stride], 0, v[22:23]\n\t" \
  "s_add_i32 s36, s36, 1\n\t" \
  "s_cmp_ge_i32 s36, %[n]\n\t" \
  "s_cbranch_scc1 9f\n\t" \
  "global_store_dwordx2 v[22:23], v[94:95], off nt\n\t" \
  "v_lshl_add_u64 v[22:23], %[stride], 0, v[22:23]\n\t" \
  "s_add_i32 s36, s36, 1\n\t" \
  "s_cmp_ge_i32 s36, %[n]\n\t" \
  "s_cbranch_scc1 9f\n\t" \
  "global_store_dwordx2 v[22:23], v[96:97], off nt\n\t" \
  "v_lshl_add_u64 v[22:23], %[stride], 0, v[22:23]\n\t" \
  "s_add_i32 s36, s36, 1\n\t" \
  "s_cmp_ge_i32 s36, %[n]\n\t" \
  "s_cbranch_scc1 9f\n\t" \
  "global_store_dwordx2 v[22:23], v[98:99], off nt\n\t" \
  "v_lshl_add_u64 v[22:23], %[stride], 0, v[22:23]\n\t" \
  "s_add_i32 s36, s36, 1\n\t" \
  "s_cmp_ge_i32 s36, %[n]\n\t" \
  "s_cbranch_scc1 9f\n\t" \
  "global_store_dwordx2 v[22:23], v[100:101], off nt\n\t" \
  "v_lshl_add_u64 v[22:23], %[stride], 0, v[22:23]\n\t" \
  "s_add_i32 s36, s36, 1\n\t" \
  "s_cmp_ge_i32 s36, %[n]\n\t" \
  "s_cbranch_scc1 9f\n\t" \
  "global_store_dwordx2 v[22:23], v[102:103], off nt\n\t" \
  "v_lshl_add_u64 v[22:23], %[stride], 0, v[22:23]\n\t" \
  "s_add_i32 s36, s36, 1\n\t" \
  "s_cmp_ge_i32 s36, %[n]\n\t" \
  "s_cbranch_scc1 9f\n\t" \
  "global_store_dwordx2 v[22:23], v[104:105], off nt\n\t" \
  "v_lshl_add_u64 v[22:23], %[stride], 0, v[22:23]\n\t" \
  "s_add_i32 s36, s36, 1\n\t" \
  "s_cmp_ge_i32 s36, %[n]\n\t" \
  "s_cbranch_scc1 9f\n\t" \
  "global_store_dwordx2 v[22:23], v[106:107], off nt\n\t" \
  "v_lshl_add_u64 v[22:23], %[stride], 0, v[22:23]\n\t" \
  "s_add_i32 s36, s36, 1\n\t" \
  "s_cmp_ge_i32 s36, %[n]\n\t" \
  "s_cbranch_scc1 9f\n\t" \
  "global_store_dwordx2 v[22:23], v[108:109], off nt\n\t" \
  "v_lshl_add_u64 v[22:23], %[stride], 0, v[22:23]\n\t" \
  "s_add_i32 s36, s36, 1\n\t" \
  "s_cmp_ge_i32 s36, %[n]\n\t" \
  "s_cbranch_scc1 9f\n\t" \
  "global_store_dwordx2 v[22:23], v[110:111], off nt\n\t" \
  "v_lshl_add_u64 v[22:23], %[stride], 0, v[22:23]\n\t" \
  "s_add_i32 s36, s36, 1\n\t" \
  "s_cmp_ge_i32 s36, %[n]\n\t" \
  "s_cbranch_scc1 9f\n\t" \
  "global_store_dwordx2 v[22:23], v[112:113], off nt\n\t" \
  "v_lshl_add_u64 v[22:23], %[stride], 0, v[22:23]\n\t" \
  "s_add_i32 s36, s36, 1\n\t" \
  "s_cmp_ge_i32 s36, %[n]\n\t" \
  "s_cbranch_scc1 9f\n\t" \
  "global_store_dwordx2 v[22:23], v[114:115], off nt\n\t" \
  "v_lshl_add_u64 v[22:23], %[stride], 0, v[22:23]\n\t" \
  "s_add_i32 s36, s36, 1\n\t" \
  "s_cmp_ge_i32 s36, %[n]\n\t" \
  "s_cbranch_scc1 9f\n\t" \
  "global_store_dwordx2 v[22:23], v[116:117], off nt\n\t" \
  "v_lshl_add_u64 v[22:23], %[stride], 0, v[22:23]\n\t" \
  "s_add_i32 s36, s36, 1\n\t" \
  "s_cmp_ge_i32 s36, %[n]\n\t" \
  "s_cbranch_scc1 9f\n\t" \
  "global_store_dwordx2 v[22:23], v[118:119], off nt\n\t" \
  "v_lshl_add_u64 v[22:23], %[stride], 0, v[22:23]\n\t" \
  "s_add_i32 s36, s36, 1\n\t" \
  "s_cmp_ge_i32 s36, %[n]\n\t" \
  "s_cbranch_scc1 9f\n\t" \
  "global_store_dwordx2 v[22:23], v[120:121], off nt\n\t" \
  "v_lshl_add_u64 v[22:23], %[stride], 0, v[22:23]\n\t" \
  "s_add_i32 s36, s36, 1\n\t" \
  "s_cmp_ge_i32 s36, %[n]\n\t" \
  "s_cbranch_scc1 9f\n\t" \
  "global_store_dwordx2 v[22:23], v[122:123], off nt\n\t" \
  "v_lshl_add_u64 v[22:23], %[stride], 0, v[22:23]\n\t" \
  "s_add_i32 s36, s36, 1\n\t" \
  "s_cmp_ge_i32 s36, %[n]\n\t" \
  "s_cbranch_scc1 9f\n\t" \
  "global_store_dwordx2 v[22:23], v[124:125], off nt\n\t" \
  "v_lshl_add_u64 v[22:23], %[stride], 0, v[22:23]\n\t" \
  "s_add_i32 s36, s36, 1\n\t" \
  "s_cmp_ge_i32 s36, %[n]\n\t" \
  "s_cbranch_scc1 9f\n\t" \
  "global_store_dwordx2 v[22:23], v[126:127], off nt\n\t" \
  "v_lshl_add_u64 v[22:23], %[stride], 0, v[22:23]\n\t" \
  "s_add_i32 s36, s36, 1\n\t" \
  "9:\n\t"

#define TL_ASM_STORE1 \
  "v_mov_b32 v22, %[lo]\n\t" \
  "v_mov_b32 v23, %[hi]\n\t" \
  "s_mov_b32 s36, 0\n\t" \
  "s_cmp_ge_i32 s36, %[n]\n\t" \
  "s_cbranch_scc1 9f\n\t" \
  "global_store_dword v[22:23], v58, off nt\n\t" \
  "v_lshl_add_u64 v[22:23], %[stride], 0, v[22:23]\n\t" \
  "s_add_i32 s36, s36, 1\n\t" \
  "s_cmp_ge_i32 s36, %[n]\n\t" \
  "s_cbranch_scc1 9f\n\t" \
  "global_store_dword v[22:23], v60, off nt\n\t" \
  "v_lshl_add_u64 v[22:23], %[stride], 0, v[22:23]\n\t" \
  "s_add_i32 s36, s36, 1\n\t" \
  "s_cmp_ge_i32 s36, %[n]\n\t" \
  "s_cbranch_scc1 9f\n\t" \
  "global_store_dword v[22:23], v62, off nt\n\t" \
  "v_lshl_add_u64 v[22:23], %[stride], 0, v[22:23]\n\t" \
  "s_add_i32 s36, s36, 1\n\t" \
  "s_cmp_ge_i32 s36, %[n]\n\t" \
  "s_cbranch_scc1 9f\n\t" \
  "global_store_dword v[22:23], v64, off nt\n\t" \
  "v_lshl_add_u64 v[22:23], %[stride], 0, v[22:23]\n\t" \
  "s_add_i32 s36, s36, 1\n\t" \
  "s_cmp_ge_i32 s36, %[n]\n\t" \
  "s_cbranch_scc1 9f\n\t" \
  "global_store_dword v[22:23], v66, off nt\n\t" \
  "v_lshl_add_u64 v[22:23], %[stride], 0, v[22:23]\n\t" \
  "s_add_i32 s36, s36, 1\n\t" \
  "s_cmp_ge_i32 s36, %[n]\n\t" \
  "s_cbranch_scc1 9f\n\t" \
  "global_store_dword v[22:23], v68, off nt\n\t" \
  "v_lshl_add_u64 v[22:23], %[stride], 0, v[22:23]\n\t" \
  "s_add_i32 s36, s36, 1\n\t" \
  "s_cmp_ge_i32 s36, %[n]\n\t" \
  "s_cbranch_scc1 9f\n\t" \
  "global_store_dword v[22:23], v70, off nt\n\t" \
  "v_lshl_add_u64 v[22:23], %[stride], 0, v[22:23]\n\t" \
  "s_add_i32 s36, s36, 1\n\t" \
  "s_cmp_ge_i32 s36, %[n]\n\t" \
  "s_cbranch_scc1 9f\n\t" \
  "global_store_dword v[22:23], v72, off nt\n\t" \
  "v_lshl_add_u64 v[22:23], %[stride], 0, v[22:23]\n\t" \
  "s_add_i32 s36, s36, 1\n\t" \
  "s_cmp_ge_i32 s36, %[n]\n\t" \
  "s_cbranch_scc1 9f\n\t" \
  "global_store_dword v[22:23], v74, off nt\n\t" \
  "v_lshl_add_u64 v[22:23], %[stride], 0, v[22:23]\n\t" \
  "s_add_i32 s36, s36, 1\n\t" \
  "s_cmp_ge_i32 s36, %[n]\n\t" \
  "s_cbranch_scc1 9f\n\t" \
  "global_store_dword v[22:23], v76, off nt\n\t" \
  "v_lshl_add_u64 v[22:23], %[stride], 0, v[22:23]\n\t" \
  "s_add_i32 s36, s36, 1\n\t" \
  "s_cmp_ge_i32 s36, %[n]\n\t" \
  "s_cbranch_scc1 9f\n\t" \
  "global_store_dword v[22:23], v78, off nt\n\t" \
  "v_lshl_add_u64 v[22:23], %[stride], 0, v[22:23]\n\t" \
  "s_add_i32 s36, s36, 1\n\t" \
  "s_cmp_ge_i32 s36, %[n]\n\t" \
  "s_cbranch_scc1 9f\n\t" \
  "global_store_dword v[22:23], v80, off nt\n\t" \
  "v_lshl_add_u64 v[22:23], %[stride], 0, v[22:23]\n\t" \
  "s_add_i32 s36, s36, 1\n\t" \
  "s_cmp_ge_i32 s36, %[n]\n\t" \
  "s_cbranch_scc1 9f\n\t" \
  "global_store_dword v[22:23], v82, off nt\n\t" \
  "v_lshl_add_u64 v[22:23], %[stride], 0, v[22:23]\n\t" \
  "s_add_i32 s36, s36, 1\n\t" \
  "s_cmp_ge_i32 s36, %[n]\n\t" \
  "s_cbranch_scc1 9f\n\t" \
  "global_store_dword v[22:23], v84, off nt\n\t" \
  "v_lshl_add_u64 v[22:23], %[stride], 0, v[22:23]\n\t" \
  "s_add_i32 s36, s36, 1\n\t" \
  "s_cmp_ge_i32 s36, %[n]\n\t" \
  "s_cbranch_scc1 9f\n\t" \
  "global_store_dword v[22:23], v86, off nt\n\t" \
  "v_lshl_add_u64 v[22:23], %[stride], 0, v[22:23]\n\t" \
  "s_add_i32 s36, s36, 1\n\t" \
  "s_cmp_ge_i32 s36, %[n]\n\t" \
  "s_cbranch_scc1 9f\n\t" \
  "global_store_dword v[22:23], v88, off nt\n\t" \
  "v_lshl_add_u64 v[22:23], %[stride], 0, v[22:23]\n\t" \
  "s_add_i32 s36, s36, 1\n\t" \
  "s_cmp_ge_i32 s36, %[n]\n\t" \
  "s_cbranch_scc1 9f\n\t" \
  "global_store_dword v[22:23], v90, off nt\n\t" \
  "v_lshl_add_u64 v[22:23], %[stride], 0, v[22:23]\n\t" \
  "s_add_i32 s36, s36, 1\n\t" \
  "s_cmp_ge_i32 s36, %[n]\n\t" \
  "s_cbranch_scc1 9f\n\t" \
  "global_store_dword v[22:23], v92, off nt\n\t" \
  "v_lshl_add_u64 v[22:23], %[stride], 0, v[22:23]\n\t" \
  "s_add_i32 s36, s36, 1\n\t" \
  "s_cmp_ge_i32 s36, %[n]\n\t" \
  "s_cbranch_scc1 9f\n\t" \
  "global_store_dword v[22:23], v94, off nt\n\t" \
  "v_lshl_add_u64 v[22:23], %[stride], 0, v[22:23]\n\t" \
  "s_add_i32 s36, s36, 1\n\t" \
  "s_cmp_ge_i32 s36, %[n]\n\t" \
  "s_cbranch_scc1 9f\n\t" \
  "global_store_dword v[22:23], v96, off nt\n\t" \
  "v_lshl_add_u64 v[22:23], %[stride], 0, v[22:23]\n\t" \
  "s_add_i32 s36, s36, 1\n\t" \
  "s_cmp_ge_i32 s36, %[n]\n\t" \
  "s_cbranch_scc1 9f\n\t" \
  "global_store_dword v[22:23], v98, off nt\n\t" \
  "v_lshl_add_u64 v[22:23], %[stride], 0, v[22:23]\n\t" \
  "s_add_i32 s36, s36, 1\n\t" \
  "s_cmp_ge_i32 s36, %[n]\n\t" \
  "s_cbranch_scc1 9f\n\t" \
  "global_store_dword v[22:23], v100, off nt\n\t" \
  "v_lshl_add_u64 v[22:23], %[stride], 0, v[22:23]\n\t" \
  "s_add_i32 s36, s36, 1\n\t" \
  "s_cmp_ge_i32 s36, %[n]\n\t" \
  "s_cbranch_scc1 9f\n\t" \
  "global_store_dword v[22:23], v102, off nt\n\t" \
  "v_lshl_add_u64 v[22:23], %[stride], 0, v[22:23]\n\t" \
  "s_add_i32 s36, s36, 1\n\t" \
  "s_cmp_ge_i32 s36, %[n]\n\t" \
  "s_cbranch_scc1 9f\n\t" \
  "global_store_dword v[22:23], v104, off nt\n\t" \
  "v_lshl_add_u64 v[22:23], %[stride], 0, v[22:23]\n\t" \
  "s_add_i32 s36, s36, 1\n\t" \
  "s_cmp_ge_i32 s36, %[n]\n\t" \
  "s_cbranch_scc1 9f\n\t" \
  "global_store_dword v[22:23], v106, off nt\n\t" \
  "v_lshl_add_u64 v[22:23], %[stride], 0, v[22:23]\n\t" \
  "s_add_i32 s36, s36, 1\n\t" \
  "s_cmp_ge_i32 s36, %[n]\n\t" \
  "s_cbranch_scc1 9f\n\t" \
  "global_store_dword v[22:23], v108, off nt\n\t" \
  "v_lshl_add_u64 v[22:23], %[stride], 0, v[22:23]\n\t" \
  "s_add_i32 s36, s36, 1\n\t" \
  "s_cmp_ge_i32 s36, %[n]\n\t" \
  "s_cbranch_scc1 9f\n\t" \
  "global_store_dword v[22:23], v110, off nt\n\t" \
  "v_lshl_add_u64 v[22:23], %[stride], 0, v[22:23]\n\t" \
  "s_add_i32 s36, s36, 1\n\t" \
  "s_cmp_ge_i32 s36, %[n]\n\t" \
  "s_cbranch_scc1 9f\n\t" \
  "global_store_dword v[22:23], v112, off nt\n\t" \
  "v_lshl_add_u64 v[22:23], %[stride], 0, v[22:23]\n\t" \
  "s_add_i32 s36, s36, 1\n\t" \
  "s_cmp_ge_i32 s36, %[n]\n\t" \
  "s_cbranch_scc1 9f\n\t" \
  "global_store_dword v[22:23], v114, off nt\n\t" \
  "v_lshl_add_u64 v[22:23], %[stride], 0, v[22:23]\n\t" \
  "s_add_i32 s36, s36, 1\n\t" \
  "s_cmp_ge_i32 s36, %[n]\n\t" \
  "s_cbranch_scc1 9f\n\t" \
  "global_store_dword v[22:23], v116, off nt\n\t" \
  "v_lshl_add_u64 v[22:23], %[stride], 0, v[22:23]\n\t" \
  "s_add_i32 s36, s36, 1\n\t" \
  "s_cmp_ge_i32 s36, %[n]\n\t" \
  "s_cbranch_scc1 9f\n\t" \
  "global_store_dword v[22:23], v118, off nt\n\t" \
  "v_lshl_add_u64 v[22:23], %[stride], 0, v[22:23]\n\t" \
  "s_add_i32 s36, s36, 1\n\t" \
  "s_cmp_ge_i32 s36, %[n]\n\t" \
  "s_cbranch_scc1 9f\n\t" \
  "global_store_dword v[22:23], v120, off nt\n\t" \
  "v_lshl_add_u64 v[22:23], %[stride], 0, v[22:23]\n\t" \
  "s_add_i32 s36, s36, 1\n\t" \
  "s_cmp_ge_i32 s36, %[n]\n\t" \
  "s_cbranch_scc1 9f\n\t" \
  "global_store_dword v[22:23], v122, off nt\n\t" \
  "v_lshl_add_u64 v[22:23], %[stride], 0, v[22:23]\n\t" \
  "s_add_i32 s36, s36, 1\n\t" \
  "s_cmp_ge_i32 s36, %[n]\n\t" \
  "s_cbranch_scc1 9f\n\t" \
  "global_store_dword v[22:23], v124, off nt\n\t" \
  "v_lshl_add_u64 v[22:23], %[stride], 0, v[22:23]\n\t" \
  "s_add_i32 s36, s36, 1\n\t" \
  "s_cmp_ge_i32 s36, %[n]\n\t" \
  "s_cbranch_scc1 9f\n\t" \
  "global_store_dword v[22:23], v126, off nt\n\t" \
  "v_lshl_add_u64 v[22:23], %[stride], 0, v[22:23]\n\t" \
  "s_add_i32 s36, s36, 1\n\t" \
  "9:\n\t"

#define TL_ASM_STORE_PERM \
  "v_mov_b32 v22, %[lo]\n\t" \
  "v_mov_b32 v23, %[hi]\n\t" \
  "s_load_dwordx16 s[40:55], %[rm], 0x0\n\t" \
  "s_load_dwordx16 s[56:71], %[rm], 0x40\n\t" \
  "s_load_dwordx4 s[72:75], %[rm], 0x80\n\t" \
  "s_waitcnt lgkmcnt(0)\n\t" \
  "s_cmp_lt_i32 s40, 0\n\t" \
  "s_cbranch_scc1 200f\n\t" \
  "s_mul_hi_u32 s89, s40, %[stride]\n\t" \
  "s_mul_i32 s88, s40, %[stride]\n\t" \
  "v_lshl_add_u64 v[24:25], s[88:89], 0, v[22:23]\n\t" \
  "global_store_dwordx2 v[24:25], v[58:59], off nt\n\t" \
  "200:\n\t" \
  "s_cmp_lt_i32 s41, 0\n\t" \
  "s_cbranch_scc1 201f\n\t" \
  "s_mul_hi_u32 s89, s41, %[stride]\n\t" \
  "s_mul_i32 s88, s41, %[stride]\n\t" \
  "v_lshl_add_u64 v[24:25], s[88:89], 0, v[22:23]\n\t" \
  "global_store_dwordx2 v[24:25], v[60:61], off nt\n\t" \
  "201:\n\t" \
  "s_cmp_lt_i32 s42, 0\n\t" \
  "s_cbranch_scc1 202f\n\t" \
  "s_mul_hi_u32 s89, s42, %[stride]\n\t" \
  "s_mul_i32 s88, s42, %[stride]\n\t" \
  "v_lshl_add_u64 v[24:25], s[88:89], 0, v[22:23]\n\t" \
  "global_store_dwordx2 v[24:25], v[62:63], off nt\n\t" \
  "202:\n\t" \
  "s_cmp_lt_i32 s43, 0\n\t" \
  "s_cbranch_scc1 203f\n\t" \
  "s_mul_hi_u32 s89, s43, %[stride]\n\t" \
  "s_mul_i32 s88, s43, %[stride]\n\t" \
  "v_lshl_add_u64 v[24:25], s[88:89], 0, v[22:23]\n\t" \
  "global_store_dwordx2 v[24:25], v[64:65], off nt\n\t" \
  "203:\n\t" \
  "s_cmp_lt_i32 s44, 0\n\t" \
  "s_cbranch_scc1 204f\n\t" \
  "s_mul_hi_u32 s89, s44, %[stride]\n\t" \
  "s_mul_i32 s88, s44, %[stride]\n\t" \
  "v_lshl_add_u64 v[24:25], s[88:89], 0, v[22:23]\n\t" \
  "global_store_dwordx2 v[24:25], v[66:67], off nt\n\t" \
  "204:\n\t" \
  "s_cmp_lt_i32 s45, 0\n\t" \
  "s_cbranch_scc1 205f\n\t" \
  "s_mul_hi_u32 s89, s45, %[stride]\n\t" \
  "s_mul_i32 s88, s45, %[stride]\n\t" \
  "v_lshl_add_u64 v[24:25], s[88:89], 0, v[22:23]\n\t" \
  "global_store_dwordx2 v[24:25], v[68:69], off nt\n\t" \
  "205:\n\t" \
  "s_cmp_lt_i32 s46, 0\n\t" \
  "s_cbranch_scc1 206f\n\t" \
  "s_mul_hi_u32 s89, s46, %[stride]\n\t" \
  "s_mul_i32 s88, s46, %[stride]\n\t" \
  "v_lshl_add_u64 v[24:25], s[88:89], 0, v[22:23]\n\t" \
  "global_store_dwordx2 v[24:25], v[70:71], off nt\n\t" \
  "206:\n\t" \
  "s_cmp_lt_i32 s47, 0\n\t" \
  "s_cbranch_scc1 207f\n\t" \
  "s_mul_hi_u32 s89, s47, %[stride]\n\t" \
  "s_mul_i32 s88, s47, %[stride]\n\t" \
  "v_lshl_add_u64 v[24:25], s[88:89], 0, v[22:23]\n\t" \
  "global_store_dwordx2 v[24:25], v[72:73], off nt\n\t" \
  "207:\n\t" \
  "s_cmp_lt_i32 s48, 0\n\t" \
  "s_cbranch_scc1 208f\n\t" \
  "s_mul_hi_u32 s89, s48, %[stride]\n\t" \
  "s_mul_i32 s88, s48, %[stride]\n\t" \
  "v_lshl_add_u64 v[24:25], s[88:89], 0, v[22:23]\n\t" \
  "global_store_dwordx2 v[24:25], v[74:75], off nt\n\t" \
  "208:\n\t" \
  "s_cmp_lt_i32 s49, 0\n\t" \
  "s_cbranch_scc1 209f\n\t" \
  "s_mul_hi_u32 s89, s49, %[stride]\n\t" \
  "s_mul_i32 s88, s49, %[stride]\n\t" \
  "v_lshl_add_u64 v[24:25], s[88:89], 0, v[22:23]\n\t" \
  "global_store_dwordx2 v[24:25], v[76:77], off nt\n\t" \
  "209:\n\t" \
  "s_cmp_lt_i32 s50, 0\n\t" \
  "s_cbranch_scc1 210f\n\t" \
  "s_mul_hi_u32 s89, s50, %[stride]\n\t" \
  "s_mul_i32 s88, s50, %[stride]\n\t" \
  "v_lshl_add_u64 v[24:25], s[88:89], 0, v[22:23]\n\t" \
  "global_store_dwordx2 v[24:25], v[78:79], off nt\n\t" \
  "210:\n\t" \
  "s_cmp_lt_i32 s51, 0\n\t" \
  "s_cbranch_scc1 211f\n\t" \
  "s_mul_hi_u32 s89, s51, %[stride]\n\t" \
  "s_mul_i32 s88, s51, %[stride]\n\t" \
  "v_lshl_add_u64 v[24:25], s[88:89], 0, v[22:23]\n\t" \
  "global_store_dwordx2 v[24:25], v[80:81], off nt\n\t" \
  "211:\n\t" \
  "s_cmp_lt_i32 s52, 0\n\t" \
  "s_cbranch_scc1 212f\n\t" \
  "s_mul_hi_u32 s89, s52, %[stride]\n\t" \
  "s_mul_i32 s88, s52, %[stride]\n\t" \
  "v_lshl_add_u64 v[24:25], s[88:89], 0, v[22:23]\n\t" \
  "global_store_dwordx2 v[24:25], v[82:83], off nt\n\t" \
  "212:\n\t" \
  "s_cmp_lt_i32 s53, 0\n\t" \
  "s_cbranch_scc1 213f\n\t" \
  "s_mul_hi_u32 s89, s53, %[stride]\n\t" \
  "s_mul_i32 s88, s53, %[stride]\n\t" \
  "v_lshl_add_u64 v[24:25], s[88:89], 0, v[22:23]\n\t" \
  "global_store_dwordx2 v[24:25], v[84:85], off nt\n\t" \
  "213:\n\t" \
  "s_cmp_lt_i32 s54, 0\n\t" \
  "s_cbranch_scc1 214f\n\t" \
  "s_mul_hi_u32 s89, s54, %[stride]\n\t" \
  "s_mul_i32 s88, s54, %[stride]\n\t" \
  "v_lshl_add_u64 v[24:25], s[88:89], 0, v[22:23]\n\t" \
  "global_store_dwordx2 v[24:25], v[86:87], off nt\n\t" \
  "214:\n\t" \
  "s_cmp_lt_i32 s55, 0\n\t" \
  "s_cbranch_scc1 215f\n\t" \
  "s_mul_hi_u32 s89, s55, %[stride]\n\t" \
  "s_mul_i32 s88, s55, %[stride]\n\t" \
  "v_lshl_add_u64 v[24:25], s[88:89], 0, v[22:23]\n\t" \
  "global_store_dwordx2 v[24:25], v[88:89], off nt\n\t" \
  "215:\n\t" \
  "s_cmp_lt_i32 s56, 0\n\t" \
  "s_cbranch_scc1 216f\n\t" \
  "s_mul_hi_u32 s89, s56, %[stride]\n\t" \
  "s_mul_i32 s88, s56, %[stride]\n\t" \
  "v_lshl_add_u64 v[24:25], s[88:89], 0, v[22:23]\n\t" \
  "global_store_dwordx2 v[24:25], v[90:91], off nt\n\t" \
  "216:\n\t" \
  "s_cmp_lt_i32 s57, 0\n\t" \
  "s_cbranch_scc1 217f\n\t" \
  "s_mul_hi_u32 s89, s57, %[stride]\n\t" \
  "s_mul_i32 s88, s57, %[stride]\n\t" \
  "v_lshl_add_u64 v[24:25], s[88:89], 0, v[22:23]\n\t" \
  "global_store_dwordx2 v[24:25], v[92:93], off nt\n\t" \
  "217:\n\t" \
  "s_cmp_lt_i32 s58, 0\n\t" \
  "s_cbranch_scc1 218f\n\t" \
  "s_mul_hi_u32 s89, s58, %[stride]\n\t" \
  "s_mul_i32 s88, s58, %[stride]\n\t" \
  "v_lshl_add_u64 v[24:25], s[88:89], 0, v[22:23]\n\t" \
  "global_store_dwordx2 v[24:25], v[94:95], off nt\n\t" \
  "218:\n\t" \
  "s_cmp_lt_i32 s59, 0\n\t" \
  "s_cbranch_scc1 219f\n\t" \
  "s_mul_hi_u32 s89, s59, %[stride]\n\t" \
  "s_mul_i32 s88, s59, %[stride]\n\t" \
  "v_lshl_add_u64 v[24:25], s[88:89], 0, v[22:23]\n\t" \
  "global_store_dwordx2 v[24:25], v[96:97], off nt\n\t" \
  "219:\n\t" \
  "s_cmp_lt_i32 s60, 0\n\t" \
  "s_cbranch_scc1 220f\n\t" \
  "s_mul_hi_u32 s89, s60, %[stride]\n\t" \
  "s_mul_i32 s88, s60, %[stride]\n\t" \
  "v_lshl_add_u64 v[24:25], s[88:89], 0, v[22:23]\n\t" \
  "global_store_dwordx2 v[24:25], v[98:99], off nt\n\t" \
  "220:\n\t" \
  "s_cmp_lt_i32 s61, 0\n\t" \
  "s_cbranch_scc1 221f\n\t" \
  "s_mul_hi_u32 s89, s61, %[stride]\n\t" \
  "s_mul_i32 s88, s61, %[stride]\n\t" \
  "v_lshl_add_u64 v[24:25], s[88:89], 0, v[22:23]\n\t" \
  "global_store_dwordx2 v[24:25], v[100:101], off nt\n\t" \
  "221:\n\t" \
  "s_cmp_lt_i32 s62, 0\n\t" \
  "s_cbranch_scc1 222f\n\t" \
  "s_mul_hi_u32 s89, s62, %[stride]\n\t" \
  "s_mul_i32 s88, s62, %[stride]\n\t" \
  "v_lshl_add_u64 v[24:25], s[88:89], 0, v[22:23]\n\t" \
  "global_store_dwordx2 v[24:25], v[102:103], off nt\n\t" \
  "222:\n\t" \
  "s_cmp_lt_i32 s63, 0\n\t" \
  "s_cbranch_scc1 223f\n\t" \
  "s_mul_hi_u32 s89, s63, %[stride]\n\t" \
  "s_mul_i32 s88, s63, %[stride]\n\t" \
  "v_lshl_add_u64 v[24:25], s[88:89], 0, v[22:23]\n\t" \
  "global_store_dwordx2 v[24:25], v[104:105], off nt\n\t" \
  "223:\n\t" \
  "s_cmp_lt_i32 s64, 0\n\t" \
  "s_cbranch_scc1 224f\n\t" \
  "s_mul_hi_u32 s89, s64, %[stride]\n\t" \
  "s_mul_i32 s88, s64, %[stride]\n\t" \
  "v_lshl_add_u64 v[24:25], s[88:89], 0, v[22:23]\n\t" \
  "global_store_dwordx2 v[24:25], v[106:107], off nt\n\t" \
  "224:\n\t" \
  "s_cmp_lt_i32 s65, 0\n\t" \
  "s_cbranch_scc1 225f\n\t" \
  "s_mul_hi_u32 s89, s65, %[stride]\n\t" \
  "s_mul_i32 s88, s65, %[stride]\n\t" \
  "v_lshl_add_u64 v[24:25], s[88:89], 0, v[22:23]\n\t" \
  "global_store_dwordx2 v[24:25], v[108:109], off nt\n\t" \
  "225:\n\t" \
  "s_cmp_lt_i32 s66, 0\n\t" \
  "s_cbranch_scc1 226f\n\t" \
  "s_mul_hi_u32 s89, s66, %[stride]\n\t" \
  "s_mul_i32 s88, s66, %[stride]\n\t" \
  "v_lshl_add_u64 v[24:25], s[88:89], 0, v[22:23]\n\t" \
  "global_store_dwordx2 v[24:25], v[110:111], off nt\n\t" \
  "226:\n\t" \
  "s_cmp_lt_i32 s67, 0\n\t" \
  "s_cbranch_scc1 227f\n\t" \
  "s_mul_hi_u32 s89, s67, %[stride]\n\t" \
  "s_mul_i32 s88, s67, %[stride]\n\t" \
  "v_lshl_add_u64 v[24:25], s[88:89], 0, v[22:23]\n\t" \
  "global_store_dwordx2 v[24:25], v[112:113], off nt\n\t" \
  "227:\n\t" \
  "s_cmp_lt_i32 s68, 0\n\t" \
  "s_cbranch_scc1 228f\n\t" \
  "s_mul_hi_u32 s89, s68, %[stride]\n\t" \
  "s_mul_i32 s88, s68, %[stride]\n\t" \
  "v_lshl_add_u64 v[24:25], s[88:89], 0, v[22:23]\n\t" \
  "global_store_dwordx2 v[24:25], v[114:115], off nt\n\t" \
  "228:\n\t" \
  "s_cmp_lt_i32 s69, 0\n\t" \
  "s_cbranch_scc1 229f\n\t" \
  "s_mul_hi_u32 s89, s69, %[stride]\n\t" \
  "s_mul_i32 s88, s69, %[stride]\n\t" \
  "v_lshl_add_u64 v[24:25], s[88:89], 0, v[22:23]\n\t" \
  "global_store_dwordx2 v[24:25], v[116:117], off nt\n\t" \
  "229:\n\t" \
  "s_cmp_lt_i32 s70, 0\n\t" \
  "s_cbranch_scc1 230f\n\t" \
  "s_mul_hi_u32 s89, s70, %[stride]\n\t" \
  "s_mul_i32 s88, s70, %[stride]\n\t" \
  "v_lshl_add_u64 v[24:25], s[88:89], 0, v[22:23]\n\t" \
  "global_store_dwordx2 v[24:25], v[118:119], off nt\n\t" \
  "230:\n\t" \
  "s_cmp_lt_i32 s71, 0\n\t" \
  "s_cbranch_scc1 231f\n\t" \
  "s_mul_hi_u32 s89, s71, %[stride]\n\t" \
  "s_mul_i32 s88, s71, %[stride]\n\t" \
  "v_lshl_add_u64 v[24:25], s[88:89], 0, v[22:23]\n\t" \
  "global_store_dwordx2 v[24:25], v[120:121], off nt\n\t" \
  "231:\n\t" \
  "s_cmp_lt_i32 s72, 0\n\t" \
  "s_cbranch_scc1 232f\n\t" \
  "s_mul_hi_u32 s89, s72, %[stride]\n\t" \
  "s_mul_i32 s88, s72, %[stride]\n\t" \
  "v_lshl_add_u64 v[24:25], s[88:89], 0, v[22:23]\n\t" \
  "global_store_dwordx2 v[24:25], v[122:123], off nt\n\t" \
  "232:\n\t" \
  "s_cmp_lt_i32 s73, 0\n\t" \
  "s_cbranch_scc1 233f\n\t" \
  "s_mul_hi_u32 s89, s73, %[stride]\n\t" \
  "s_mul_i32 s88, s73, %[stride]\n\t" \
  "v_lshl_add_u64 v[24:25], s[88:89], 0, v[22:23]\n\t" \
  "global_store_dwordx2 v[24:25], v[124:125], off nt\n\t" \
  "233:\n\t" \
  "s_cmp_lt_i32 s74, 0\n\t" \
  "s_cbranch_scc1 234f\n\t" \
  "s_mul_hi_u32 s89, s74, %[stride]\n\t" \
  "s_mul_i32 s88, s74, %[stride]\n\t" \
  "v_lshl_add_u64 v[24:25], s[88:89], 0, v[22:23]\n\t" \
  "global_store_dwordx2 v[24:25], v[126:127], off nt\n\t" \
  "234:\n\t"

#define TL_ASM_STORE1_PERM \
  "v_mov_b32 v22, %[lo]\n\t" \
  "v_mov_b32 v23, %[hi]\n\t" \
  "s_load_dwordx16 s[40:55], %[rm], 0x0\n\t" \
  "s_load_dwordx16 s[56:71], %[rm], 0x40\n\t" \
  "s_load_dwordx4 s[72:75], %[rm], 0x80\n\t" \
  "s_waitcnt lgkmcnt(0)\n\t" \
  "s_cmp_lt_i32 s40, 0\n\t" \
  "s_cbranch_scc1 200f\n\t" \
  "s_mul_hi_u32 s89, s40, %[stride]\n\t" \
  "s_mul_i32 s88, s40, %[stride]\n\t" \
  "v_lshl_add_u64 v[24:25], s[88:89], 0, v[22:23]\n\t" \
  "global_store_dword v[24:25], v58, off nt\n\t" \
  "200:\n\t" \
  "s_cmp_lt_i32 s41, 0\n\t" \
  "s_cbranch_scc1 201f\n\t" \
  "s_mul_hi_u32 s89, s41, %[stride]\n\t" \
  "s_mul_i32 s88, s41, %[stride]\n\t" \
  "v_lshl_add_u64 v[24:25], s[88:89], 0, v[22:23]\n\t" \
  "global_store_dword v[24:25], v60, off nt\n\t" \
  "201:\n\t" \
  "s_cmp_lt_i32 s42, 0\n\t" \
  "s_cbranch_scc1 202f\n\t" \
  "s_mul_hi_u32 s89, s42, %[stride]\n\t" \
  "s_mul_i32 s88, s42, %[stride]\n\t" \
  "v_lshl_add_u64 v[24:25], s[88:89], 0, v[22:23]\n\t" \
  "global_store_dword v[24:25], v62, off nt\n\t" \
  "202:\n\t" \
  "s_cmp_lt_i32 s43, 0\n\t" \
  "s_cbranch_scc1 203f\n\t" \
  "s_mul_hi_u32 s89, s43, %[stride]\n\t" \
  "s_mul_i32 s88, s43, %[stride]\n\t" \
  "v_lshl_add_u64 v[24:25], s[88:89], 0, v[22:23]\n\t" \
  "global_store_dword v[24:25], v64, off nt\n\t" \
  "203:\n\t" \
  "s_cmp_lt_i32 s44, 0\n\t" \
  "s_cbranch_scc1 204f\n\t" \
  "s_mul_hi_u32 s89, s44, %[stride]\n\t" \
  "s_mul_i32 s88, s44, %[stride]\n\t" \
  "v_lshl_add_u64 v[24:25], s[88:89], 0, v[22:23]\n\t" \
  "global_store_dword v[24:25], v66, off nt\n\t" \
  "204:\n\t" \
  "s_cmp_lt_i32 s45, 0\n\t" \
  "s_cbranch_scc1 205f\n\t" \
  "s_mul_hi_u32 s89, s45, %[stride]\n\t" \
  "s_mul_i32 s88, s45, %[stride]\n\t" \
  "v_lshl_add_u64 v[24:25], s[88:89], 0, v[22:23]\n\t" \
  "global_store_dword v[24:25], v68, off nt\n\t" \
  "205:\n\t" \
  "s_cmp_lt_i32 s46, 0\n\t" \
  "s_cbranch_scc1 206f\n\t" \
  "s_mul_hi_u32 s89, s46, %[stride]\n\t" \
  "s_mul_i32 s88, s46, %[stride]\n\t" \
  "v_lshl_add_u64 v[24:25], s[88:89], 0, v[22:23]\n\t" \
  "global_store_dword v[24:25], v70, off nt\n\t" \
  "206:\n\t" \
  "s_cmp_lt_i32 s47, 0\n\t" \
  "s_cbranch_scc1 207f\n\t" \
  "s_mul_hi_u32 s89, s47, %[stride]\n\t" \
  "s_mul_i32 s88, s47, %[stride]\n\t" \
  "v_lshl_add_u64 v[24:25], s[88:89], 0, v[22:23]\n\t" \
  "global_store_dword v[24:25], v72, off nt\n\t" \
  "207:\n\t" \
  "s_cmp_lt_i32 s48, 0\n\t" \
  "s_cbranch_scc1 208f\n\t" \
  "s_mul_hi_u32 s89, s48, %[stride]\n\t" \
  "s_mul_i32 s88, s48, %[stride]\n\t" \
  "v_lshl_add_u64 v[24:25], s[88:89], 0, v[22:23]\n\t" \
  "global_store_dword v[24:25], v74, off nt\n\t" \
  "208:\n\t" \
  "s_cmp_lt_i32 s49, 0\n\t" \
  "s_cbranch_scc1 209f\n\t" \
  "s_mul_hi_u32 s89, s49, %[stride]\n\t" \
  "s_mul_i32 s88, s49, %[stride]\n\t" \
  "v_lshl_add_u64 v[24:25], s[88:89], 0, v[22:23]\n\t" \
  "global_store_dword v[24:25], v76, off nt\n\t" \
  "209:\n\t" \
  "s_cmp_lt_i32 s50, 0\n\t" \
  "s_cbranch_scc1 210f\n\t" \
  "s_mul_hi_u32 s89, s50, %[stride]\n\t" \
  "s_mul_i32 s88, s50, %[stride]\n\t" \
  "v_lshl_add_u64 v[24:25], s[88:89], 0, v[22:23]\n\t" \
  "global_store_dword v[24:25], v78, off nt\n\t" \
  "210:\n\t" \
  "s_cmp_lt_i32 s51, 0\n\t" \
  "s_cbranch_scc1 211f\n\t" \
  "s_mul_hi_u32 s89, s51, %[stride]\n\t" \
  "s_mul_i32 s88, s51, %[stride]\n\t" \
  "v_lshl_add_u64 v[24:25], s[88:89], 0, v[22:23]\n\t" \
  "global_store_dword v[24:25], v80, off nt\n\t" \
  "211:\n\t" \
  "s_cmp_lt_i32 s52, 0\n\t" \
  "s_cbranch_scc1 212f\n\t" \
  "s_mul_hi_u32 s89, s52, %[stride]\n\t" \
  "s_mul_i32 s88, s52, %[stride]\n\t" \
  "v_lshl_add_u64 v[24:25], s[88:89], 0, v[22:23]\n\t" \
  "global_store_dword v[24:25], v82, off nt\n\t" \
  "212:\n\t" \
  "s_cmp_lt_i32 s53, 0\n\t" \
  "s_cbranch_scc1 213f\n\t" \
  "s_mul_hi_u32 s89, s53, %[stride]\n\t" \
  "s_mul_i32 s88, s53, %[stride]\n\t" \
  "v_lshl_add_u64 v[24:25], s[88:89], 0, v[22:23]\n\t" \
  "global_store_dword v[24:25], v84, off nt\n\t" \
  "213:\n\t" \
  "s_cmp_lt_i32 s54, 0\n\t" \
  "s_cbranch_scc1 214f\n\t" \
  "s_mul_hi_u32 s89, s54, %[stride]\n\t" \
  "s_mul_i32 s88, s54, %[stride]\n\t" \
  "v_lshl_add_u64 v[24:25], s[88:89], 0, v[22:23]\n\t" \
  "global_store_dword v[24:25], v86, off nt\n\t" \
  "214:\n\t" \
  "s_cmp_lt_i32 s55, 0\n\t" \
  "s_cbranch_scc1 215f\n\t" \
  "s_mul_hi_u32 s89, s55, %[stride]\n\t" \
  "s_mul_i32 s88, s55, %[stride]\n\t" \
  "v_lshl_add_u64 v[24:25], s[88:89], 0, v[22:23]\n\t" \
  "global_store_dword v[24:25], v88, off nt\n\t" \
  "215:\n\t" \
  "s_cmp_lt_i32 s56, 0\n\t" \
  "s_cbranch_scc1 216f\n\t" \
  "s_mul_hi_u32 s89, s56, %[stride]\n\t" \
  "s_mul_i32 s88, s56, %[stride]\n\t" \
  "v_lshl_add_u64 v[24:25], s[88:89], 0, v[22:23]\n\t" \
  "global_store_dword v[24:25], v90, off nt\n\t" \
  "216:\n\t" \
  "s_cmp_lt_i32 s57, 0\n\t" \
  "s_cbranch_scc1 217f\n\t" \
  "s_mul_hi_u32 s89, s57, %[stride]\n\t" \
  "s_mul_i32 s88, s57, %[stride]\n\t" \
  "v_lshl_add_u64 v[24:25], s[88:89], 0, v[22:23]\n\t" \
  "global_store_dword v[24:25], v92, off nt\n\t" \
  "217:\n\t" \
  "s_cmp_lt_i32 s58, 0\n\t" \
  "s_cbranch_scc1 218f\n\t" \
  "s_mul_hi_u32 s89, s58, %[stride]\n\t" \
  "s_mul_i32 s88, s58, %[stride]\n\t" \
  "v_lshl_add_u64 v[24:25], s[88:89], 0, v[22:23]\n\t" \
  "global_store_dword v[24:25], v94, off nt\n\t" \
  "218:\n\t" \
  "s_cmp_lt_i32 s59, 0\n\t" \
  "s_cbranch_scc1 219f\n\t" \
  "s_mul_hi_u32 s89, s59, %[stride]\n\t" \
  "s_mul_i32 s88, s59, %[stride]\n\t" \
  "v_lshl_add_u64 v[24:25], s[88:89], 0, v[22:23]\n\t" \
  "global_store_dword v[24:25], v96, off nt\n\t" \
  "219:\n\t" \
  "s_cmp_lt_i32 s60, 0\n\t" \
  "s_cbranch_scc1 220f\n\t" \
  "s_mul_hi_u32 s89, s60, %[stride]\n\t" \
  "s_mul_i32 s88, s60, %[stride]\n\t" \
  "v_lshl_add_u64 v[24:25], s[88:89], 0, v[22:23]\n\t" \
  "global_store_dword v[24:25], v98, off nt\n\t" \
  "220:\n\t" \
  "s_cmp_lt_i32 s61, 0\n\t" \
  "s_cbranch_scc1 221f\n\t" \
  "s_mul_hi_u32 s89, s61, %[stride]\n\t" \
  "s_mul_i32 s88, s61, %[stride]\n\t" \
  "v_lshl_add_u64 v[24:25], s[88:89], 0, v[22:23]\n\t" \
  "global_store_dword v[24:25], v100, off nt\n\t" \
  "221:\n\t" \
  "s_cmp_lt_i32 s62, 0\n\t" \
  "s_cbranch_scc1 222f\n\t" \
  "s_mul_hi_u32 s89, s62, %[stride]\n\t" \
  "s_mul_i32 s88, s62, %[stride]\n\t" \
  "v_lshl_add_u64 v[24:25], s[88:89], 0, v[22:23]\n\t" \
  "global_store_dword v[24:25], v102, off nt\n\t" \
  "222:\n\t" \
  "s_cmp_lt_i32 s63, 0\n\t" \
  "s_cbranch_scc1 223f\n\t" \
  "s_mul_hi_u32 s89, s63, %[stride]\n\t" \
  "s_mul_i32 s88, s63, %[stride]\n\t" \
  "v_lshl_add_u64 v[24:25], s[88:89], 0, v[22:23]\n\t" \
  "global_store_dword v[24:25], v104, off nt\n\t" \
  "223:\n\t" \
  "s_cmp_lt_i32 s64, 0\n\t" \
  "s_cbranch_scc1 224f\n\t" \
  "s_mul_hi_u32 s89, s64, %[stride]\n\t" \
  "s_mul_i32 s88, s64, %[stride]\n\t" \
  "v_lshl_add_u64 v[24:25], s[88:89], 0, v[22:23]\n\t" \
  "global_store_dword v[24:25], v106, off nt\n\t" \
  "224:\n\t" \
  "s_cmp_lt_i32 s65, 0\n\t" \
  "s_cbranch_scc1 225f\n\t" \
  "s_mul_hi_u32 s89, s65, %[stride]\n\t" \
  "s_mul_i32 s88, s65, %[stride]\n\t" \
  "v_lshl_add_u64 v[24:25], s[88:89], 0, v[22:23]\n\t" \
  "global_store_dword v[24:25], v108, off nt\n\t" \
  "225:\n\t" \
  "s_cmp_lt_i32 s66, 0\n\t" \
  "s_cbranch_scc1 226f\n\t" \
  "s_mul_hi_u32 s89, s66, %[stride]\n\t" \
  "s_mul_i32 s88, s66, %[stride]\n\t" \
  "v_lshl_add_u64 v[24:25], s[88:89], 0, v[22:23]\n\t" \
  "global_store_dword v[24:25], v110, off nt\n\t" \
  "226:\n\t" \
  "s_cmp_lt_i32 s67, 0\n\t" \
  "s_cbranch_scc1 227f\n\t" \
  "s_mul_hi_u32 s89, s67, %[stride]\n\t" \
  "s_mul_i32 s88, s67, %[stride]\n\t" \
  "v_lshl_add_u64 v[24:25], s[88:89], 0, v[22:23]\n\t" \
  "global_store_dword v[24:25], v112, off nt\n\t" \
  "227:\n\t" \
  "s_cmp_lt_i32 s68, 0\n\t" \
  "s_cbranch_scc1 228f\n\t" \
  "s_mul_hi_u32 s89, s68, %[stride]\n\t" \
  "s_mul_i32 s88, s68, %[stride]\n\t" \
  "v_lshl_add_u64 v[24:25], s[88:89], 0, v[22:23]\n\t" \
  "global_store_dword v[24:25], v114, off nt\n\t" \
  "228:\n\t" \
  "s_cmp_lt_i32 s69, 0\n\t" \
  "s_cbranch_scc1 229f\n\t" \
  "s_mul_hi_u32 s89, s69, %[stride]\n\t" \
  "s_mul_i32 s88, s69, %[stride]\n\t" \
  "v_lshl_add_u64 v[24:25], s[88:89], 0, v[22:23]\n\t" \
  "global_store_dword v[24:25], v116, off nt\n\t" \
  "229:\n\t" \
  "s_cmp_lt_i32 s70, 0\n\t" \
  "s_cbranch_scc1 230f\n\t" \
  "s_mul_hi_u32 s89, s70, %[stride]\n\t" \
  "s_mul_i32 s88, s70, %[stride]\n\t" \
  "v_lshl_add_u64 v[24:25], s[88:89], 0, v[22:23]\n\t" \
  "global_store_dword v[24:25], v118, off nt\n\t" \
  "230:\n\t" \
  "s_cmp_lt_i32 s71, 0\n\t" \
  "s_cbranch_scc1 231f\n\t" \
  "s_mul_hi_u32 s89, s71, %[stride]\n\t" \
  "s_mul_i32 s88, s71, %[stride]\n\t" \
  "v_lshl_add_u64 v[24:25], s[88:89], 0, v[22:23]\n\t" \
  "global_store_dword v[24:25], v120, off nt\n\t" \
  "231:\n\t" \
  "s_cmp_lt_i32 s72, 0\n\t" \
  "s_cbranch_scc1 232f\n\t" \
  "s_mul_hi_u32 s89, s72, %[stride]\n\t" \
  "s_mul_i32 s88, s72, %[stride]\n\t" \
  "v_lshl_add_u64 v[24:25], s[88:89], 0, v[22:23]\n\t" \
  "global_store_dword v[24:25], v122, off nt\n\t" \
  "232:\n\t" \
  "s_cmp_lt_i32 s73, 0\n\t" \
  "s_cbranch_scc1 233f\n\t" \
  "s_mul_hi_u32 s89, s73, %[stride]\n\t" \
  "s_mul_i32 s88, s73, %[stride]\n\t" \
  "v_lshl_add_u64 v[24:25], s[88:89], 0, v[22:23]\n\t" \
  "global_store_dword v[24:25], v124, off nt\n\t" \
  "233:\n\t" \
  "s_cmp_lt_i32 s74, 0\n\t" \
  "s_cbranch_scc1 234f\n\t" \
  "s_mul_hi_u32 s89, s74, %[stride]\n\t" \
  "s_mul_i32 s88, s74, %[stride]\n\t" \
  "v_lshl_add_u64 v[24:25], s[88:89], 0, v[22:23]\n\t" \
  "global_store_dword v[24:25], v126, off nt\n\t" \
  "234:\n\t"

#define TL_ASM_ZERO \
  "v_mov_b32 v56, 0\n\t" \
  "v_mov_b32 v57, 0\n\t" \
  "v_mov_b32 v58, 0\n\t" \
  "v_mov_b32 v59, 0\n\t" \
  "v_mov_b32 v60, 0\n\t" \
  "v_mov_b32 v61, 0\n\t" \
  "v_mov_b32 v62, 0\n\t" \
  "v_mov_b32 v63, 0\n\t" \
  "v_mov_b32 v64, 0\n\t" \
  "v_mov_b32 v65, 0\n\t" \
  "v_mov_b32 v66, 0\n\t" \
  "v_mov_b32 v67, 0\n\t" \
  "v_mov_b32 v68, 0\n\t" \
  "v_mov_b32 v69, 0\n\t" \
  "v_mov_b32 v70, 0\n\t" \
  "v_mov_b32 v71, 0\n\t" \
  "v_mov_b32 v72, 0\n\t" \
  "v_mov_b32 v73, 0\n\t" \
  "v_mov_b32 v74, 0\n\t" \
  "v_mov_b32 v75, 0\n\t" \
  "v_mov_b32 v76, 0\n\t" \
  "v_mov_b32 v77, 0\n\t" \
  "v_mov_b32 v78, 0\n\t" \
  "v_mov_b32 v79, 0\n\t" \
  "v_mov_b32 v80, 0\n\t" \
  "v_mov_b32 v81, 0\n\t" \
  "v_mov_b32 v82, 0\n\t" \
  "v_mov_b32 v83, 0\n\t" \
  "v_mov_b32 v84, 0\n\t" \
  "v_mov_b32 v85, 0\n\t" \
  "v_mov_b32 v86, 0\n\t" \
  "v_mov_b32 v87, 0\n\t" \
  "v_mov_b32 v88, 0\n\t" \
  "v_mov_b32 v89, 0\n\t" \
  "v_mov_b32 v90, 0\n\t" \
  "v_mov_b32 v91, 0\n\t" \
  "v_mov_b32 v92, 0\n\t" \
  "v_mov_b32 v93, 0\n\t" \
  "v_mov_b32 v94, 0\n\t" \
  "v_mov_b32 v95, 0\n\t" \
  "v_mov_b32 v96, 0\n\t" \
  "v_mov_b32 v97, 0\n\t" \
  "v_mov_b32 v98, 0\n\t" \
  "v_mov_b32 v99, 0\n\t" \
  "v_mov_b32 v100, 0\n\t" \
  "v_mov_b32 v101, 0\n\t" \
  "v_mov_b32 v102, 0\n\t" \
  "v_mov_b32 v103, 0\n\t" \
  "v_mov_b32 v104, 0\n\t" \
  "v_mov_b32 v105, 0\n\t" \
  "v_mov_b32 v106, 0\n\t" \
  "v_mov_b32 v107, 0\n\t" \
  "v_mov_b32 v108, 0\n\t" \
  "v_mov_b32 v109, 0\n\t" \
  "v_mov_b32 v110, 0\n\t" \
  "v_mov_b32 v111, 0\n\t" \
  "v_mov_b32 v112, 0\n\t" \
  "v_mov_b32 v113, 0\n\t" \
  "v_mov_b32 v114, 0\n\t" \
  "v_mov_b32 v115, 0\n\t" \
  "v_mov_b32 v116, 0\n\t" \
  "v_mov_b32 v117, 0\n\t" \
  "v_mov_b32 v118, 0\n\t" \
  "v_mov_b32 v119, 0\n\t" \
  "v_mov_b32 v120, 0\n\t" \
  "v_mov_b32 v121, 0\n\t" \
  "v_mov_b32 v122, 0\n\t" \
  "v_mov_b32 v123, 0\n\t" \
  "v_mov_b32 v124, 0\n\t" \
  "v_mov_b32 v125, 0\n\t" \
  "v_mov_b32 v126, 0\n\t" \
  "v_mov_b32 v127, 0\n\t"

#define TL_CLOB_SGPR "s36", "s37", "s38", "s39", "s40", "s41", "s42", "s43", "s44", "s45", "s46", "s47", "s48", "s49", "s50", "s51", "s52", "s53", "s54", "s55", "s56", "s57", "s58", "s59", "s60", "s61", "s62", "s63", "s64", "s65", "s66", "s67", "s68", "s69", "s70", "s71", "s72", "s73", "s74", "s75", "s76", "s77", "s78", "s79", "s80", "s81", "s82", "s83", "s84", "s85", "s86", "s87", "s88", "s89", "s90", "s91", "s92", "s93", "s94", "s95"

#define TL_CLOB_TMP "v22", "v23", "v24", "v25", "v26", "v27", "v28", "v29", "v30", "v31", "v32", "v33", "v34", "v35", "v36", "v37", "v38", "v39", "v40", "v41", "v42", "v43", "v44", "v45", "v46", "v47", "v48", "v49", "v50", "v51", "v52", "v53", "v54", "v55"

#define TL_CLOB_ACC "v56", "v57", "v58", "v59", "v60", "v61", "v62", "v63", "v64", "v65", "v66", "v67", "v68", "v69", "v70", "v71", "v72", "v73", "v74", "v75", "v76", "v77", "v78", "v79", "v80", "v81", "v82", "v83", "v84", "v85", "v86", "v87", "v88", "v89", "v90", "v91", "v92", "v93", "v94", "v95", "v96", "v97", "v98", "v99", "v100", "v101", "v102", "v103", "v104", "v105", "v106", "v107", "v108", "v109", "v110", "v111", "v112", "v113", "v114", "v115", "v116", "v117", "v118", "v119", "v120", "v121", "v122", "v123", "v124", "v125", "v126", "v127"
```

Baseline: 29870 GFLOP/s.

## Fold whole tiled SpMM kernel body into one pinned-register inline asm block

Replaces the C++ control flow around the hand-written phase asm (tile-0 prefetch, chunk loop with offset loads and readlanes, partial-tile DMA, epilogue stores) with a single asm statement that has operands pinned to fixed SGPRs/VGPRs. The aim is to remove compiler-generated glue, scalar-vector moves and register pressure around the repeated asm calls. It also drops the amdgpu_num_vgpr attribute and the build-time register-spill check. The risks are that hard-pinned register constraints may collide with the compiler's own allocation, and that spills would no longer be caught at build time.

```diff
diff --git a/sparse_amd/csrc/build.py b/sparse_amd/csrc/build.py
--- a/sparse_amd/csrc/build.py
+++ b/sparse_amd/csrc/build.py
@@ -51,42 +51,15 @@
     return files + [os.path.abspath(__file__)]
 
 
-NO_SPILL = {"spmm_tiled.hip": "spmm_tiled_kernel"}
-
-
-def _spills(remarks, needle):
-    out, name, sg = [], None, 0
-    for ln in remarks.splitlines():
-        if "Function Name:" in ln:
-            name = ln.split("Function Name:")[1].split()[0]
-        elif "SGPRs Spill:" in ln:
-            sg = int(ln.split("SGPRs Spill:")[1].split()[0])
-        elif "VGPRs Spill:" in ln and name is not None:
-            vg = int(ln.split("VGPRs Spill:")[1].split()[0])
-            if needle in name and (sg or vg):
-                out.append((name, sg, vg))
-    return out
-
-
 def _compile(src, force):
     obj = os.path.join(OBJ_DIR, os.path.basename(src)[:-4] + ".o")
     newest = max(os.path.getmtime(p) for p in [src] + _own_deps(src, obj))
     if not force and os.path.exists(obj) and os.path.getmtime(obj) >= newest:
         return obj, ""
-    needle = NO_SPILL.get(os.path.basename(src))
-    extra = ["-Rpass-analysis=kernel-resource-usage"] if needle else []
-    cmd = [_hipcc(), *CXXFLAGS, *extra, "-MD", "-MF", obj[:-2] + ".d", "-c", src, "-o", obj]
+    cmd = [_hipcc(), *CXXFLAGS, "-MD", "-MF", obj[:-2] + ".d", "-c", src, "-o", obj]
     r = subprocess.run(cmd, capture_output=True, text=True)
     if r.returncode != 0:
         raise RuntimeError(f"hipcc failed for {src}:\n{' '.join(cmd)}\n{r.stdout}\n{r.stderr}")
-    if needle:
-        bad = _spills(r.stderr, needle)
-        if bad:
-            os.remove(obj)
-            raise RuntimeError(f"{os.path.basename(src)}: the compiler spilled registers in " +
-                               ", ".join(f"{n[:60]} ({s} SGPR, {v} VGPR)" for n, s, v in bad[:4]) +
-                               " - refused (see NO_SPILL in sparse_amd/csrc/build.py)")
-        return obj, "\n".join(ln for ln in r.stderr.splitlines() if "-Rpass-analysis" not in ln and "remark:" not in ln)
     return obj, r.stderr
 
 
diff --git a/sparse_amd/csrc/spmm_tiled.hip b/sparse_amd/csrc/spmm_tiled.hip
--- a/sparse_amd/csrc/spmm_tiled.hip
+++ b/sparse_amd/csrc/spmm_tiled.hip
@@ -322,43 +322,6 @@
   }
 }
 
-__device__ __forceinline__ void tl_dma16(unsigned lds_base, const void* src) {
-  asm volatile("s_mov_b32 m0, %0\n\ts_nop 0\n\tglobal_load_lds_dwordx4 %1, off"
-               :
-               : "s"(lds_base), "v"(src)
-               : "memory", "m0");
-}
-
-template <int MODE>
-__device__ __forceinline__ void tl_phases(const int* stream, int t0, int te, int o0, int o1, int o2, int offreg, int obase,
-                                          int ntiles, int nfull, int toff, int mask, unsigned m0wave,
-                                          unsigned row_step, int voff, tl_srd_t srd, unsigned& soff) {
-  const int lane = threadIdx.x & 63;
-  const unsigned blo = (unsigned)((uintptr_t)stream & 0xffffffffu), bhi = (unsigned)((uintptr_t)stream >> 32);
-  const int lane8 = lane * 8;
-#define TL_PHASES_OPERANDS                                                                                        \
-  [soff] "+s"(soff)                                                                                               \
-  : [blo] "s"(blo), [bhi] "s"(bhi), [t0] "s"(t0), [te] "s"(te), [o0] "s"(o0), [o1] "s"(o1), [o2] "s"(o2),         \
-    [obase] "s"(obase), [ntiles] "s"(ntiles), [nfull] "s"(nfull), [m0wave] "s"(m0wave), [step] "s"(row_step),      \
-    [toff] "v"(toff), [lane8] "v"(lane8), [mask] "v"(mask), [offreg] "v"(offreg), [voff] "v"(voff), [srd] "s"(srd)  \
-  : "memory", "m0", "scc", "vcc", TL_CLOB_SGPR, TL_CLOB_TMP, TL_CLOB_ACC
-  if (MODE == 6)
-    asm volatile(TL_ASM_PHASES_I32 : TL_PHASES_OPERANDS);
-  else if (MODE == 4)
-    asm volatile(TL_ASM_PHASES_F64 : TL_PHASES_OPERANDS);
-  else if (MODE == 5)
-    asm volatile(TL_ASM_PHASES_F64_EXACT : TL_PHASES_OPERANDS);
-  else if (MODE == 3)
-    asm volatile(TL_ASM_PHASES_EXACT : TL_PHASES_OPERANDS);
-  else if (MODE == 1)
-    asm volatile(TL_ASM_PHASES_NOFMA : TL_PHASES_OPERANDS);
-  else if (MODE == 2)
-    asm volatile(TL_ASM_PHASES_NOLDS : TL_PHASES_OPERANDS);
-  else
-    asm volatile(TL_ASM_PHASES : TL_PHASES_OPERANDS);
-#undef TL_PHASES_OPERANDS
-}
-
 __device__ __forceinline__ void tl_block_map(unsigned L, int npanels, int nblocks, int& bx, int& by) {
   const unsigned pin = npanels > 1 ? 2u : 1u;
   const unsigned per_chunk = (unsigned)((nblocks + 7) / 8) * 8u * pin;
@@ -369,13 +332,12 @@
 }
 
 template <int DBG, int MODE, typename T>
-__global__ void __launch_bounds__(TL_WAVES * 64) __attribute__((amdgpu_num_vgpr(TL_ASM_COMP)))
+__global__ void __launch_bounds__(TL_WAVES * 64)
 spmm_tiled_kernel(int64_t M, int64_t K, int ntiles, int touch_lines, const int* __restrict__ stream,
                   const int* __restrict__ blk_off, const T* __restrict__ b, int64_t ldb,
                   T* __restrict__ out, int64_t ldo, int last_cols, int npanels, int nblocks, const int* __restrict__ rowmap) {
   constexpr int PANEL = TlFmt<T>::PANEL;
   constexpr int CPL = PANEL / 64;
-  extern __shared__ __attribute__((aligned(16))) char lds[];
   const int tid = threadIdx.x;
   const int lane = tid & 63;
   const int wv = uniform(tid >> 6);
@@ -386,10 +348,10 @@
   b += (int64_t)by * PANEL;
   out += (int64_t)by * PANEL;
 
-  asm volatile(TL_ASM_ZERO ::: "memory", TL_CLOB_ACC);
-
   const int nfull = DBG == 2 ? 0 : (int)(K / TL_KB);
-  const unsigned row_step = (unsigned)((2 * TL_WAVES) * ldb * (int64_t)sizeof(T));
+  const bool has_partial = DBG != 2 && (int64_t)nfull * TL_KB < K;
+  const unsigned row_bytes = (unsigned)(ldb * (int64_t)sizeof(T));
+  const unsigned row_step = (2 * TL_WAVES) * row_bytes;
   const unsigned m0wave = (unsigned)wv * 2048u;
   const uint64_t bbase = (uint64_t)(uintptr_t)b;
   tl_srd_t srd;
@@ -397,92 +359,60 @@
   srd[1] = (int)((bbase >> 32) & 0xffffu);
   srd[2] = (int)0xffffffffu;
   srd[3] = 0x00020000;
-  const int voff = (int)((int64_t)(tid >> 5) * ldb * (int64_t)sizeof(T)) + (tid & 31) * 16;
-  unsigned soff = 0;
-  auto issue_partial = [&](int t) {
-#pragma unroll
-    for (int i = 0; i < TL_DMA_PER_TILE; ++i) {
-      const int e = (i * (TL_WAVES * 64) + tid) * 16;
-      int64_t r = (int64_t)t * TL_KB + (e >> 9);
-      if (r >= K) r = K - 1;
-      tl_dma16(((unsigned)(i * TL_WAVES + wv) * 2u + (unsigned)(t & 1)) * 1024u,
-               reinterpret_cast<const char*>(b + r * ldb) + (e & 511));
-    }
-  };
-  const bool has_partial = DBG != 2 && (int64_t)nfull * TL_KB < K;
-
-  if (nfull > 0)
-    asm volatile(TL_ASM_TILE0 : [soff] "+s"(soff) : [m0wave] "s"(m0wave), [step] "s"(row_step), [voff] "v"(voff), [srd] "s"(srd) : "memory", "m0", "scc", "vcc", "s89");
-  else if (has_partial)
-    issue_partial(0);
-  asm volatile("s_waitcnt vmcnt(0)" ::: "memory");
-  __syncthreads();
+  const int voff = (tid >> 5) * (int)row_bytes + (tid & 31) * 16;
+  const int part_last = has_partial ? (int)(K - (int64_t)nfull * TL_KB) - 1 : 0;
+  const unsigned part_off = has_partial ? (unsigned)nfull * TL_KB * row_bytes : 0u;
 
   const int* const myoff = blk_off + (int64_t)g * (ntiles + (touch_lines >> 16));
   touch_lines &= 0xffff;
   const int toff = (lane < touch_lines ? lane : touch_lines - 1) * 64;
-  int t = 0;
-  while (t < ntiles) {
-    const int obase = t;
-    const int q = obase + lane;
-    int offreg = myoff[q < ntiles ? q : ntiles];
-    asm volatile("" : "+v"(offreg));
-    int te = obase + 61 < ntiles ? obase + 61 : ntiles;
-    if (has_partial && t < nfull - 1 && nfull - 1 < te) te = nfull - 1;
-    if (has_partial && t == nfull - 1) issue_partial(nfull);
-    auto o = [&](int tt) { return wave_bcast(offreg, (tt < ntiles ? tt : ntiles) - obase); };
-    const int o0 = o(t), o1 = o(t + 1), o2 = o(t + 2);
-    if (t == 0) {
-      const int n = o2 - o0, l = lane < n ? lane : 0;
-      asm volatile("global_load_dword " TL_ASM_TOUCH ", %0, off" ::"v"(reinterpret_cast<const char*>(stream + (int64_t)o0 * 16) + l * 64)
-                   : "memory", TL_ASM_TOUCH);
-    }
-    tl_phases<MODE>(stream, t, te, o0, o1, o2, offreg, obase, ntiles, nfull, toff, (int)0xfffffe00, m0wave, row_step, voff, srd, soff);
-    t = te;
-  }
-  asm volatile("s_waitcnt vmcnt(0) lgkmcnt(0)" ::: "memory");
 
   const int64_t row0 = (int64_t)g * TL_RG;
   const int64_t left = M - row0;
   const int nvalid = left <= 0 ? 0 : (left < TL_RG ? (int)left : TL_RG);
-  T* const obase_p = out + row0 * ldo + lane * CPL;
-  const int64_t stride_bytes = ldo * (int64_t)sizeof(T);
-  int bx2, by2;
-  tl_block_map(blockIdx.x, npanels, nblocks, bx2, by2);
-  const int ncols = (last_cols > 0 && by2 == npanels - 1) ? last_cols : PANEL;
-  if (rowmap) {
-    const int* const rm = rowmap + (int64_t)g * TL_RG;
-    T* const base_p = out + lane * CPL;
-    if (lane * CPL + CPL <= ncols)
-      asm volatile(TL_ASM_STORE_PERM
-                   :
-                   : [lo] "v"((unsigned)((uintptr_t)base_p & 0xffffffffu)), [hi] "v"((unsigned)((uintptr_t)base_p >> 32)),
-                     [stride] "s"((unsigned)stride_bytes), [rm] "s"(rm)
-                   : "memory", "scc", TL_CLOB_SGPR, TL_CLOB_TMP, TL_CLOB_ACC);
-    if constexpr (CPL == 2) {
-      if (lane * CPL + 1 == ncols)
-        asm volatile(TL_ASM_STORE1_PERM
-                     :
-                     : [lo] "v"((unsigned)((uintptr_t)base_p & 0xffffffffu)), [hi] "v"((unsigned)((uintptr_t)base_p >> 32)),
-                       [stride] "s"((unsigned)stride_bytes), [rm] "s"(rm)
-                     : "memory", "scc", TL_CLOB_SGPR, TL_CLOB_TMP);
-    }
-    return;
-  }
-  if (lane * CPL + CPL <= ncols)
-    asm volatile(TL_ASM_STORE
-                 :
-                 : [lo] "v"((unsigned)((uintptr_t)obase_p & 0xffffffffu)), [hi] "v"((unsigned)((uintptr_t)obase_p >> 32)),
-                   [stride] "s"(stride_bytes), [n] "s"(nvalid)
-                 : "memory", "scc", "s36", TL_ASM_BASE, TL_ASM_TOUCH, TL_CLOB_ACC);
-  if constexpr (CPL == 2) {
-    if (lane * CPL + 1 == ncols)
-      asm volatile(TL_ASM_STORE1
-                   :
-                   : [lo] "v"((unsigned)((uintptr_t)obase_p & 0xffffffffu)), [hi] "v"((unsigned)((uintptr_t)obase_p >> 32)),
-                     [stride] "s"(stride_bytes), [n] "s"(nvalid)
-                   : "memory", "scc", "s36", TL_ASM_BASE, TL_ASM_TOUCH);
-  }
+  const int ncols = (last_cols > 0 && by == npanels - 1) ? last_cols : PANEL;
+  const int store_lim = ncols * (8 / CPL);
+  const bool mapped = rowmap != nullptr;
+  const uint64_t stride_bytes = (uint64_t)(ldo * (int64_t)sizeof(T));
+  const uint64_t rm = (uint64_t)(uintptr_t)(mapped ? rowmap + (int64_t)g * TL_RG : rowmap);
+  const int lane8 = lane * 8;
+  const T* const sbase = out + (mapped ? 0 : row0 * ldo) + lane * CPL;
+  unsigned soff = 0;
+  int t0 = 0, te = 0, obase = 0, o0 = 0, o1 = 0, o2 = 0, offreg = 0;
+
+  const int64_t u_stream = uniform((int64_t)(uintptr_t)stream), u_myoff = uniform((int64_t)(uintptr_t)myoff);
+  const int64_t u_stride = uniform((int64_t)stride_bytes), u_rm = uniform((int64_t)rm);
+  tl_srd_t u_srd;
+  for (int i = 0; i < 4; ++i) u_srd[i] = uniform(srd[i]);
+#define TL_KERNEL_OPERANDS                                                                                                  \
+  [soff] "+{s12}"(soff), [t0] "+{s27}"(t0), [te] "+{s28}"(te), [obase] "+{s29}"(obase), [o0] "+{s30}"(o0),                \
+    [o1] "+{s31}"(o1), [o2] "+{s32}"(o2), [offreg] "+{v4}"(offreg)                                                          \
+  : [blo] "{s0}"((int)u_stream), [bhi] "{s1}"((int)(u_stream >> 32)), [myoff] "{s[2:3]}"(u_myoff), [srd] "{s[4:7]}"(u_srd),  \
+    [ntiles] "{s8}"(uniform(ntiles)), [nfull] "{s9}"(uniform(nfull)), [m0wave] "{s10}"(uniform((int)m0wave)),             \
+    [step] "{s11}"(uniform((int)row_step)), [haspart] "{s13}"(uniform((int)has_partial)), [plast] "{s14}"(uniform(part_last)), \
+    [poff] "{s15}"(uniform((int)part_off)), [rowb] "{s16}"(uniform((int)row_bytes)), [rstride] "{s[18:19]}"(u_stride),     \
+    [stride] "{s20}"((int)u_stride), [n] "{s22}"(uniform(nvalid)), [mapped] "{s23}"(uniform((int)mapped)),                 \
+    [rm] "{s[24:25]}"(u_rm), [lim] "{s26}"(uniform(store_lim)), [lane8] "{v0}"(lane8), [mask] "{v1}"((int)0xfffffe00),      \
+    [voff] "{v2}"(voff), [toff] "{v3}"(toff), [lo] "{v5}"((unsigned)((uintptr_t)sbase & 0xffffffffu)),                    \
+    [hi] "{v6}"((unsigned)((uintptr_t)sbase >> 32))                                                                         \
+  : "memory", "m0", "scc", "vcc", "exec", "s34", "s35", TL_CLOB_SGPR, TL_CLOB_TMP, TL_CLOB_ACC
+#define TL_KERNEL(PHASES, STORES) TL_ASM_ZERO TL_ASM_BEGIN TL_ASM_CHUNK_HEAD PHASES TL_ASM_CHUNK_TAIL STORES
+  if constexpr (MODE == 6)
+    asm volatile(TL_KERNEL(TL_ASM_PHASES_I32, TL_ASM_STORES) : TL_KERNEL_OPERANDS);
+  else if constexpr (MODE == 4)
+    asm volatile(TL_KERNEL(TL_ASM_PHASES_F64, TL_ASM_STORES_F64) : TL_KERNEL_OPERANDS);
+  else if constexpr (MODE == 5)
+    asm volatile(TL_KERNEL(TL_ASM_PHASES_F64_EXACT, TL_ASM_STORES_F64) : TL_KERNEL_OPERANDS);
+  else if constexpr (MODE == 3)
+    asm volatile(TL_KERNEL(TL_ASM_PHASES_EXACT, TL_ASM_STORES) : TL_KERNEL_OPERANDS);
+  else if constexpr (MODE == 1)
+    asm volatile(TL_KERNEL(TL_ASM_PHASES_NOFMA, TL_ASM_STORES) : TL_KERNEL_OPERANDS);
+  else if constexpr (MODE == 2)
+    asm volatile(TL_KERNEL(TL_ASM_PHASES_NOLDS, TL_ASM_STORES) : TL_KERNEL_OPERANDS);
+  else
+    asm volatile(TL_KERNEL(TL_ASM_PHASES, TL_ASM_STORES) : TL_KERNEL_OPERANDS);
+#undef TL_KERNEL
+#undef TL_KERNEL_OPERANDS
 }
 
 static int64_t tl_grid_groups(int64_t M) { return ceil_div(ceil_div(M, (int64_t)TL_RG), (int64_t)TL_WAVES) * TL_WAVES; }
diff --git a/sparse_amd/csrc/spmm_tiled_asm.inc b/sparse_amd/csrc/spmm_tiled_asm.inc
--- a/sparse_amd/csrc/spmm_tiled_asm.inc
+++ b/sparse_amd/csrc/spmm_tiled_asm.inc
@@ -6,6 +6,8 @@
 #define TL_ASM_COMP 22
 #define TL_ASM_TOUCH "v23"
 #define TL_ASM_BASE "v22"
+#define TL_ASM_VGPRS 128
+#define TL_ASM_SGPRS 96
 
 #define TL_ASM_PHASES \
   "s_mov_b32 s39, 0\n\t" \
@@ -6707,177 +6709,177 @@
   "s_cmp_ge_i32 s36, %[n]\n\t" \
   "s_cbranch_scc1 9f\n\t" \
   "global_store_dwordx2 v[22:23], v[58:59], off nt\n\t" \
-  "v_lshl_add_u64 v[22:23], %[stride], 0, v[22:23]\n\t" \
+  "v_lshl_add_u64 v[22:23], %[rstride], 0, v[22:23]\n\t" \
   "s_add_i32 s36, s36, 1\n\t" \
   "s_cmp_ge_i32 s36, %[n]\n\t" \
   "s_cbranch_scc1 9f\n\t" \
   "global_store_dwordx2 v[22:23], v[60:61], off nt\n\t" \
-  "v_lshl_add_u64 v[22:23], %[stride], 0, v[22:23]\n\t" \
+  "v_lshl_add_u64 v[22:23], %[rstride], 0, v[22:23]\n\t" \
   "s_add_i32 s36, s36, 1\n\t" \
   "s_cmp_ge_i32 s36, %[n]\n\t" \
   "s_cbranch_scc1 9f\n\t" \
   "global_store_dwordx2 v[22:23], v[62:63], off nt\n\t" \
-  "v_lshl_add_u64 v[22:23], %[stride], 0, v[22:23]\n\t" \
+  "v_lshl_add_u64 v[22:23], %[rstride], 0, v[22:23]\n\t" \
   "s_add_i32 s36, s36, 1\n\t" \
   "s_cmp_ge_i32 s36, %[n]\n\t" \
   "s_cbranch_scc1 9f\n\t" \
   "global_store_dwordx2 v[22:23], v[64:65], off nt\n\t" \
-  "v_lshl_add_u64 v[22:23], %[stride], 0, v[22:23]\n\t" \
+  "v_lshl_add_u64 v[22:23], %[rstride], 0, v[22:23]\n\t" \
   "s_add_i32 s36, s36, 1\n\t" \
   "s_cmp_ge_i32 s36, %[n]\n\t" \
   "s_cbranch_scc1 9f\n\t" \
   "global_store_dwordx2 v[22:23], v[66:67], off nt\n\t" \
-  "v_lshl_add_u64 v[22:23], %[stride], 0, v[22:23]\n\t" \
+  "v_lshl_add_u64 v[22:23], %[rstride], 0, v[22:23]\n\t" \
   "s_add_i32 s36, s36, 1\n\t" \
   "s_cmp_ge_i32 s36, %[n]\n\t" \
   "s_cbranch_scc1 9f\n\t" \
   "global_store_dwordx2 v[22:23], v[68:69], off nt\n\t" \
-  "v_lshl_add_u64 v[22:23], %[stride], 0, v[22:23]\n\t" \
+  "v_lshl_add_u64 v[22:23], %[rstride], 0, v[22:23]\n\t" \
   "s_add_i32 s36, s36, 1\n\t" \
   "s_cmp_ge_i32 s36, %[n]\n\t" \
   "s_cbranch_scc1 9f\n\t" \
   "global_store_dwordx2 v[22:23], v[70:71], off nt\n\t" \
-  "v_lshl_add_u64 v[22:23], %[stride], 0, v[22:23]\n\t" \
+  "v_lshl_add_u64 v[22:23], %[rstride], 0, v[22:23]\n\t" \
   "s_add_i32 s36, s36, 1\n\t" \
   "s_cmp_ge_i32 s36, %[n]\n\t" \
   "s_cbranch_scc1 9f\n\t" \
   "global_store_dwordx2 v[22:23], v[72:73], off nt\n\t" \
-  "v_lshl_add_u64 v[22:23], %[stride], 0, v[22:23]\n\t" \
+  "v_lshl_add_u64 v[22:23], %[rstride], 0, v[22:23]\n\t" \
   "s_add_i32 s36, s36, 1\n\t" \
   "s_cmp_ge_i32 s36, %[n]\n\t" \
   "s_cbranch_scc1 9f\n\t" \
   "global_store_dwordx2 v[22:23], v[74:75], off nt\n\t" \
-  "v_lshl_add_u64 v[22:23], %[stride], 0, v[22:23]\n\t" \
+  "v_lshl_add_u64 v[22:23], %[rstride], 0, v[22:23]\n\t" \
   "s_add_i32 s36, s36, 1\n\t" \
   "s_cmp_ge_i32 s36, %[n]\n\t" \
   "s_cbranch_scc1 9f\n\t" \
   "global_store_dwordx2 v[22:23], v[76:77], off nt\n\t" \
-  "v_lshl_add_u64 v[22:23], %[stride], 0, v[22:23]\n\t" \
+  "v_lshl_add_u64 v[22:23], %[rstride], 0, v[22:23]\n\t" \
   "s_add_i32 s36, s36, 1\n\t" \
   "s_cmp_ge_i32 s36, %[n]\n\t" \
   "s_cbranch_scc1 9f\n\t" \
   "global_store_dwordx2 v[22:23], v[78:79], off nt\n\t" \
-  "v_lshl_add_u64 v[22:23], %[stride], 0, v[22:23]\n\t" \
+  "v_lshl_add_u64 v[22:23], %[rstride], 0, v[22:23]\n\t" \
   "s_add_i32 s36, s36, 1\n\t" \
   "s_cmp_ge_i32 s36, %[n]\n\t" \
   "s_cbranch_scc1 9f\n\t" \
   "global_store_dwordx2 v[22:23], v[80:81], off nt\n\t" \
-  "v_lshl_add_u64 v[22:23], %[stride], 0, v[22:23]\n\t" \
+  "v_lshl_add_u64 v[22:23], %[rstride], 0, v[22:23]\n\t" \
   "s_add_i32 s36, s36, 1\n\t" \
   "s_cmp_ge_i32 s36, %[n]\n\t" \
   "s_cbranch_scc1 9f\n\t" \
   "global_store_dwordx2 v[22:23], v[82:83], off nt\n\t" \
-  "v_lshl_add_u64 v[22:23], %[stride], 0, v[22:23]\n\t" \
+  "v_lshl_add_u64 v[22:23], %[rstride], 0, v[22:23]\n\t" \
   "s_add_i32 s36, s36, 1\n\t" \
   "s_cmp_ge_i32 s36, %[n]\n\t" \
   "s_cbranch_scc1 9f\n\t" \
   "global_store_dwordx2 v[22:23], v[84:85], off nt\n\t" \
-  "v_lshl_add_u64 v[22:23], %[stride], 0, v[22:23]\n\t" \
+  "v_lshl_add_u64 v[22:23], %[rstride], 0, v[22:23]\n\t" \
   "s_add_i32 s36, s36, 1\n\t" \
   "s_cmp_ge_i32 s36, %[n]\n\t" \
   "s_cbranch_scc1 9f\n\t" \
   "global_store_dwordx2 v[22:23], v[86:87], off nt\n\t" \
-  "v_lshl_add_u64 v[22:23], %[stride], 0, v[22:23]\n\t" \
+  "v_lshl_add_u64 v[22:23], %[rstride], 0, v[22:23]\n\t" \
   "s_add_i32 s36, s36, 1\n\t" \
   "s_cmp_ge_i32 s36, %[n]\n\t" \
   "s_cbranch_scc1 9f\n\t" \
   "global_store_dwordx2 v[22:23], v[88:89], off nt\n\t" \
-  "v_lshl_add_u64 v[22:23], %[stride], 0, v[22:23]\n\t" \
+  "v_lshl_add_u64 v[22:23], %[rstride], 0, v[22:23]\n\t" \
   "s_add_i32 s36, s36, 1\n\t" \
   "s_cmp_ge_i32 s36, %[n]\n\t" \
   "s_cbranch_scc1 9f\n\t" \
   "global_store_dwordx2 v[22:23], v[90:91], off nt\n\t" \
-  "v_lshl_add_u64 v[22:23], %[stride], 0, v[22:23]\n\t" \
+  "v_lshl_add_u64 v[22:23], %[rstride], 0, v[22:23]\n\t" \
   "s_add_i32 s36, s36, 1\n\t" \
   "s_cmp_ge_i32 s36, %[n]\n\t" \
   "s_cbranch_scc1 9f\n\t" \
   "global_store_dwordx2 v[22:23], v[92:93], off nt\n\t" \
-  "v_lshl_add_u64 v[22:23], %[stride], 0, v[22:23]\n\t" \
+  "v_lshl_add_u64 v[22:23], %[rstride], 0, v[22:23]\n\t" \
   "s_add_i32 s36, s36, 1\n\t" \
   "s_cmp_ge_i32 s36, %[n]\n\t" \
   "s_cbranch_scc1 9f\n\t" \
   "global_store_dwordx2 v[22:23], v[94:95], off nt\n\t" \
-  "v_lshl_add_u64 v[22:23], %[stride], 0, v[22:23]\n\t" \
+  "v_lshl_add_u64 v[22:23], %[rstride], 0, v[22:23]\n\t" \
   "s_add_i32 s36, s36, 1\n\t" \
   "s_cmp_ge_i32 s36, %[n]\n\t" \
   "s_cbranch_scc1 9f\n\t" \
   "global_store_dwordx2 v[22:23], v[96:97], off nt\n\t" \
-  "v_lshl_add_u64 v[22:23], %[stride], 0, v[22:23]\n\t" \
+  "v_lshl_add_u64 v[22:23], %[rstride], 0, v[22:23]\n\t" \
   "s_add_i32 s36, s36, 1\n\t" \
   "s_cmp_ge_i32 s36, %[n]\n\t" \
   "s_cbranch_scc1 9f\n\t" \
   "global_store_dwordx2 v[22:23], v[98:99], off nt\n\t" \
-  "v_lshl_add_u64 v[22:23], %[stride], 0, v[22:23]\n\t" \
+  "v_lshl_add_u64 v[22:23], %[rstride], 0, v[22:23]\n\t" \
   "s_add_i32 s36, s36, 1\n\t" \
   "s_cmp_ge_i32 s36, %[n]\n\t" \
   "s_cbranch_scc1 9f\n\t" \
   "global_store_dwordx2 v[22:23], v[100:101], off nt\n\t" \
-  "v_lshl_add_u64 v[22:23], %[stride], 0, v[22:23]\n\t" \
+  "v_lshl_add_u64 v[22:23], %[rstride], 0, v[22:23]\n\t" \
   "s_add_i32 s36, s36, 1\n\t" \
   "s_cmp_ge_i32 s36, %[n]\n\t" \
   "s_cbranch_scc1 9f\n\t" \
   "global_store_dwordx2 v[22:23], v[102:103], off nt\n\t" \
-  "v_lshl_add_u64 v[22:23], %[stride], 0, v[22:23]\n\t" \
+  "v_lshl_add_u64 v[22:23], %[rstride], 0, v[22:23]\n\t" \
   "s_add_i32 s36, s36, 1\n\t" \
   "s_cmp_ge_i32 s36, %[n]\n\t" \
   "s_cbranch_scc1 9f\n\t" \
   "global_store_dwordx2 v[22:23], v[104:105], off nt\n\t" \
-  "v_lshl_add_u64 v[22:23], %[stride], 0, v[22:23]\n\t" \
+  "v_lshl_add_u64 v[22:23], %[rstride], 0, v[22:23]\n\t" \
   "s_add_i32 s36, s36, 1\n\t" \
   "s_cmp_ge_i32 s36, %[n]\n\t" \
   "s_cbranch_scc1 9f\n\t" \
   "global_store_dwordx2 v[22:23], v[106:107], off nt\n\t" \
-  "v_lshl_add_u64 v[22:23], %[stride], 0, v[22:23]\n\t" \
+  "v_lshl_add_u64 v[22:23], %[rstride], 0, v[22:23]\n\t" \
   "s_add_i32 s36, s36, 1\n\t" \
   "s_cmp_ge_i32 s36, %[n]\n\t" \
   "s_cbranch_scc1 9f\n\t" \
   "global_store_dwordx2 v[22:23], v[108:109], off nt\n\t" \
-  "v_lshl_add_u64 v[22:23], %[stride], 0, v[22:23]\n\t" \
+  "v_lshl_add_u64 v[22:23], %[rstride], 0, v[22:23]\n\t" \
   "s_add_i32 s36, s36, 1\n\t" \
   "s_cmp_ge_i32 s36, %[n]\n\t" \
   "s_cbranch_scc1 9f\n\t" \
   "global_store_dwordx2 v[22:23], v[110:111], off nt\n\t" \
-  "v_lshl_add_u64 v[22:23], %[stride], 0, v[22:23]\n\t" \
+  "v_lshl_add_u64 v[22:23], %[rstride], 0, v[22:23]\n\t" \
   "s_add_i32 s36, s36, 1\n\t" \
   "s_cmp_ge_i32 s36, %[n]\n\t" \
   "s_cbranch_scc1 9f\n\t" \
   "global_store_dwordx2 v[22:23], v[112:113], off nt\n\t" \
-  "v_lshl_add_u64 v[22:23], %[stride], 0, v[22:23]\n\t" \
+  "v_lshl_add_u64 v[22:23], %[rstride], 0, v[22:23]\n\t" \
   "s_add_i32 s36, s36, 1\n\t" \
   "s_cmp_ge_i32 s36, %[n]\n\t" \
   "s_cbranch_scc1 9f\n\t" \
   "global_store_dwordx2 v[22:23], v[114:115], off nt\n\t" \
-  "v_lshl_add_u64 v[22:23], %[stride], 0, v[22:23]\n\t" \
+  "v_lshl_add_u64 v[22:23], %[rstride], 0, v[22:23]\n\t" \
   "s_add_i32 s36, s36, 1\n\t" \
   "s_cmp_ge_i32 s36, %[n]\n\t" \
   "s_cbranch_scc1 9f\n\t" \
   "global_store_dwordx2 v[22:23], v[116:117], off nt\n\t" \
-  "v_lshl_add_u64 v[22:23], %[stride], 0, v[22:23]\n\t" \
+  "v_lshl_add_u64 v[22:23], %[rstride], 0, v[22:23]\n\t" \
   "s_add_i32 s36, s36, 1\n\t" \
   "s_cmp_ge_i32 s36, %[n]\n\t" \
   "s_cbranch_scc1 9f\n\t" \
   "global_store_dwordx2 v[22:23], v[118:119], off nt\n\t" \
-  "v_lshl_add_u64 v[22:23], %[stride], 0, v[22:23]\n\t" \
+  "v_lshl_add_u64 v[22:23], %[rstride], 0, v[22:23]\n\t" \
   "s_add_i32 s36, s36, 1\n\t" \
   "s_cmp_ge_i32 s36, %[n]\n\t" \
   "s_cbranch_scc1 9f\n\t" \
   "global_store_dwordx2 v[22:23], v[120:121], off nt\n\t" \
-  "v_lshl_add_u64 v[22:23], %[stride], 0, v[22:23]\n\t" \
+  "v_lshl_add_u64 v[22:23], %[rstride], 0, v[22:23]\n\t" \
   "s_add_i32 s36, s36, 1\n\t" \
   "s_cmp_ge_i32 s36, %[n]\n\t" \
   "s_cbranch_scc1 9f\n\t" \
   "global_store_dwordx2 v[22:23], v[122:123], off nt\n\t" \
-  "v_lshl_add_u64 v[22:23], %[stride], 0, v[22:23]\n\t" \
+  "v_lshl_add_u64 v[22:23], %[rstride], 0, v[22:23]\n\t" \
   "s_add_i32 s36, s36, 1\n\t" \
   "s_cmp_ge_i32 s36, %[n]\n\t" \
   "s_cbranch_scc1 9f\n\t" \
   "global_store_dwordx2 v[22:23], v[124:125], off nt\n\t" \
-  "v_lshl_add_u64 v[22:23], %[stride], 0, v[22:23]\n\t" \
+  "v_lshl_add_u64 v[22:23], %[rstride], 0, v[22:23]\n\t" \
   "s_add_i32 s36, s36, 1\n\t" \
   "s_cmp_ge_i32 s36, %[n]\n\t" \
   "s_cbranch_scc1 9f\n\t" \
   "global_store_dwordx2 v[22:23], v[126:127], off nt\n\t" \
-  "v_lshl_add_u64 v[22:23], %[stride], 0, v[22:23]\n\t" \
+  "v_lshl_add_u64 v[22:23], %[rstride], 0, v[22:23]\n\t" \
   "s_add_i32 s36, s36, 1\n\t" \
   "9:\n\t"
 
@@ -6888,177 +6890,177 @@
   "s_cmp_ge_i32 s36, %[n]\n\t" \
   "s_cbranch_scc1 9f\n\t" \
   "global_store_dword v[22:23], v58, off nt\n\t" \
-  "v_lshl_add_u64 v[22:23], %[stride], 0, v[22:23]\n\t" \
+  "v_lshl_add_u64 v[22:23], %[rstride], 0, v[22:23]\n\t" \
   "s_add_i32 s36, s36, 1\n\t" \
   "s_cmp_ge_i32 s36, %[n]\n\t" \
   "s_cbranch_scc1 9f\n\t" \
   "global_store_dword v[22:23], v60, off nt\n\t" \
-  "v_lshl_add_u64 v[22:23], %[stride], 0, v[22:23]\n\t" \
+  "v_lshl_add_u64 v[22:23], %[rstride], 0, v[22:23]\n\t" \
   "s_add_i32 s36, s36, 1\n\t" \
   "s_cmp_ge_i32 s36, %[n]\n\t" \
   "s_cbranch_scc1 9f\n\t" \
   "global_store_dword v[22:23], v62, off nt\n\t" \
-  "v_lshl_add_u64 v[22:23], %[stride], 0, v[22:23]\n\t" \
+  "v_lshl_add_u64 v[22:23], %[rstride], 0, v[22:23]\n\t" \
   "s_add_i32 s36, s36, 1\n\t" \
   "s_cmp_ge_i32 s36, %[n]\n\t" \
   "s_cbranch_scc1 9f\n\t" \
   "global_store_dword v[22:23], v64, off nt\n\t" \
-  "v_lshl_add_u64 v[22:23], %[stride], 0, v[22:23]\n\t" \
+  "v_lshl_add_u64 v[22:23], %[rstride], 0, v[22:23]\n\t" \
   "s_add_i32 s36, s36, 1\n\t" \
   "s_cmp_ge_i32 s36, %[n]\n\t" \
   "s_cbranch_scc1 9f\n\t" \
   "global_store_dword v[22:23], v66, off nt\n\t" \
-  "v_lshl_add_u64 v[22:23], %[stride], 0, v[22:23]\n\t" \
+  "v_lshl_add_u64 v[22:23], %[rstride], 0, v[22:23]\n\t" \
   "s_add_i32 s36, s36, 1\n\t" \
   "s_cmp_ge_i32 s36, %[n]\n\t" \
   "s_cbranch_scc1 9f\n\t" \
   "global_store_dword v[22:23], v68, off nt\n\t" \
-  "v_lshl_add_u64 v[22:23], %[stride], 0, v[22:23]\n\t" \
+  "v_lshl_add_u64 v[22:23], %[rstride], 0, v[22:23]\n\t" \
   "s_add_i32 s36, s36, 1\n\t" \
   "s_cmp_ge_i32 s36, %[n]\n\t" \
   "s_cbranch_scc1 9f\n\t" \
   "global_store_dword v[22:23], v70, off nt\n\t" \
-  "v_lshl_add_u64 v[22:23], %[stride], 0, v[22:23]\n\t" \
+  "v_lshl_add_u64 v[22:23], %[rstride], 0, v[22:23]\n\t" \
   "s_add_i32 s36, s36, 1\n\t" \
   "s_cmp_ge_i32 s36, %[n]\n\t" \
   "s_cbranch_scc1 9f\n\t" \
   "global_store_dword v[22:23], v72, off nt\n\t" \
-  "v_lshl_add_u64 v[22:23], %[stride], 0, v[22:23]\n\t" \
+  "v_lshl_add_u64 v[22:23], %[rstride], 0, v[22:23]\n\t" \
   "s_add_i32 s36, s36, 1\n\t" \
   "s_cmp_ge_i32 s36, %[n]\n\t" \
   "s_cbranch_scc1 9f\n\t" \
   "global_store_dword v[22:23], v74, off nt\n\t" \
-  "v_lshl_add_u64 v[22:23], %[stride], 0, v[22:23]\n\t" \
+  "v_lshl_add_u64 v[22:23], %[rstride], 0, v[22:23]\n\t" \
   "s_add_i32 s36, s36, 1\n\t" \
   "s_cmp_ge_i32 s36, %[n]\n\t" \
   "s_cbranch_scc1 9f\n\t" \
   "global_store_dword v[22:23], v76, off nt\n\t" \
-  "v_lshl_add_u64 v[22:23], %[stride], 0, v[22:23]\n\t" \
+  "v_lshl_add_u64 v[22:23], %[rstride], 0, v[22:23]\n\t" \
   "s_add_i32 s36, s36, 1\n\t" \
   "s_cmp_ge_i32 s36, %[n]\n\t" \
   "s_cbranch_scc1 9f\n\t" \
   "global_store_dword v[22:23], v78, off nt\n\t" \
-  "v_lshl_add_u64 v[22:23], %[stride], 0, v[22:23]\n\t" \
+  "v_lshl_add_u64 v[22:23], %[rstride], 0, v[22:23]\n\t" \
   "s_add_i32 s36, s36, 1\n\t" \
   "s_cmp_ge_i32 s36, %[n]\n\t" \
   "s_cbranch_scc1 9f\n\t" \
   "global_store_dword v[22:23], v80, off nt\n\t" \
-  "v_lshl_add_u64 v[22:23], %[stride], 0, v[22:23]\n\t" \
+  "v_lshl_add_u64 v[22:23], %[rstride], 0, v[22:23]\n\t" \
   "s_add_i32 s36, s36, 1\n\t" \
   "s_cmp_ge_i32 s36, %[n]\n\t" \
   "s_cbranch_scc1 9f\n\t" \
   "global_store_dword v[22:23], v82, off nt\n\t" \
-  "v_lshl_add_u64 v[22:23], %[stride], 0, v[22:23]\n\t" \
+  "v_lshl_add_u64 v[22:23], %[rstride], 0, v[22:23]\n\t" \
   "s_add_i32 s36, s36, 1\n\t" \
   "s_cmp_ge_i32 s36, %[n]\n\t" \
   "s_cbranch_scc1 9f\n\t" \
   "global_store_dword v[22:23], v84, off nt\n\t" \
-  "v_lshl_add_u64 v[22:23], %[stride], 0, v[22:23]\n\t" \
+  "v_lshl_add_u64 v[22:23], %[rstride], 0, v[22:23]\n\t" \
   "s_add_i32 s36, s36, 1\n\t" \
   "s_cmp_ge_i32 s36, %[n]\n\t" \
   "s_cbranch_scc1 9f\n\t" \
   "global_store_dword v[22:23], v86, off nt\n\t" \
-  "v_lshl_add_u64 v[22:23], %[stride], 0, v[22:23]\n\t" \
+  "v_lshl_add_u64 v[22:23], %[rstride], 0, v[22:23]\n\t" \
   "s_add_i32 s36, s36, 1\n\t" \
   "s_cmp_ge_i32 s36, %[n]\n\t" \
   "s_cbranch_scc1 9f\n\t" \
   "global_store_dword v[22:23], v88, off nt\n\t" \
-  "v_lshl_add_u64 v[22:23], %[stride], 0, v[22:23]\n\t" \
+  "v_lshl_add_u64 v[22:23], %[rstride], 0, v[22:23]\n\t" \
   "s_add_i32 s36, s36, 1\n\t" \
   "s_cmp_ge_i32 s36, %[n]\n\t" \
   "s_cbranch_scc1 9f\n\t" \
   "global_store_dword v[22:23], v90, off nt\n\t" \
-  "v_lshl_add_u64 v[22:23], %[stride], 0, v[22:23]\n\t" \
+  "v_lshl_add_u64 v[22:23], %[rstride], 0, v[22:23]\n\t" \
   "s_add_i32 s36, s36, 1\n\t" \
   "s_cmp_ge_i32 s36, %[n]\n\t" \
   "s_cbranch_scc1 9f\n\t" \
   "global_store_dword v[22:23], v92, off nt\n\t" \
-  "v_lshl_add_u64 v[22:23], %[stride], 0, v[22:23]\n\t" \
+  "v_lshl_add_u64 v[22:23], %[rstride], 0, v[22:23]\n\t" \
   "s_add_i32 s36, s36, 1\n\t" \
   "s_cmp_ge_i32 s36, %[n]\n\t" \
   "s_cbranch_scc1 9f\n\t" \
   "global_store_dword v[22:23], v94, off nt\n\t" \
-  "v_lshl_add_u64 v[22:23], %[stride], 0, v[22:23]\n\t" \
+  "v_lshl_add_u64 v[22:23], %[rstride], 0, v[22:23]\n\t" \
   "s_add_i32 s36, s36, 1\n\t" \
   "s_cmp_ge_i32 s36, %[n]\n\t" \
   "s_cbranch_scc1 9f\n\t" \
   "global_store_dword v[22:23], v96, off nt\n\t" \
-  "v_lshl_add_u64 v[22:23], %[stride], 0, v[22:23]\n\t" \
+  "v_lshl_add_u64 v[22:23], %[rstride], 0, v[22:23]\n\t" \
   "s_add_i32 s36, s36, 1\n\t" \
   "s_cmp_ge_i32 s36, %[n]\n\t" \
   "s_cbranch_scc1 9f\n\t" \
   "global_store_dword v[22:23], v98, off nt\n\t" \
-  "v_lshl_add_u64 v[22:23], %[stride], 0, v[22:23]\n\t" \
+  "v_lshl_add_u64 v[22:23], %[rstride], 0, v[22:23]\n\t" \
   "s_add_i32 s36, s36, 1\n\t" \
   "s_cmp_ge_i32 s36, %[n]\n\t" \
   "s_cbranch_scc1 9f\n\t" \
   "global_store_dword v[22:23], v100, off nt\n\t" \
-  "v_lshl_add_u64 v[22:23], %[stride], 0, v[22:23]\n\t" \
+  "v_lshl_add_u64 v[22:23], %[rstride], 0, v[22:23]\n\t" \
   "s_add_i32 s36, s36, 1\n\t" \
   "s_cmp_ge_i32 s36, %[n]\n\t" \
   "s_cbranch_scc1 9f\n\t" \
   "global_store_dword v[22:23], v102, off nt\n\t" \
-  "v_lshl_add_u64 v[22:23], %[stride], 0, v[22:23]\n\t" \
+  "v_lshl_add_u64 v[22:23], %[rstride], 0, v[22:23]\n\t" \
   "s_add_i32 s36, s36, 1\n\t" \
   "s_cmp_ge_i32 s36, %[n]\n\t" \
   "s_cbranch_scc1 9f\n\t" \
   "global_store_dword v[22:23], v104, off nt\n\t" \
-  "v_lshl_add_u64 v[22:23], %[stride], 0, v[22:23]\n\t" \
+  "v_lshl_add_u64 v[22:23], %[rstride], 0, v[22:23]\n\t" \
   "s_add_i32 s36, s36, 1\n\t" \
   "s_cmp_ge_i32 s36, %[n]\n\t" \
   "s_cbranch_scc1 9f\n\t" \
   "global_store_dword v[22:23], v106, off nt\n\t" \
-  "v_lshl_add_u64 v[22:23], %[stride], 0, v[22:23]\n\t" \
+  "v_lshl_add_u64 v[22:23], %[rstride], 0, v[22:23]\n\t" \
   "s_add_i32 s36, s36, 1\n\t" \
   "s_cmp_ge_i32 s36, %[n]\n\t" \
   "s_cbranch_scc1 9f\n\t" \
   "global_store_dword v[22:23], v108, off nt\n\t" \
-  "v_lshl_add_u64 v[22:23], %[stride], 0, v[22:23]\n\t" \
+  "v_lshl_add_u64 v[22:23], %[rstride], 0, v[22:23]\n\t" \
   "s_add_i32 s36, s36, 1\n\t" \
   "s_cmp_ge_i32 s36, %[n]\n\t" \
   "s_cbranch_scc1 9f\n\t" \
   "global_store_dword v[22:23], v110, off nt\n\t" \
-  "v_lshl_add_u64 v[22:23], %[stride], 0, v[22:23]\n\t" \
+  "v_lshl_add_u64 v[22:23], %[rstride], 0, v[22:23]\n\t" \
   "s_add_i32 s36, s36, 1\n\t" \
   "s_cmp_ge_i32 s36, %[n]\n\t" \
   "s_cbranch_scc1 9f\n\t" \
   "global_store_dword v[22:23], v112, off nt\n\t" \
-  "v_lshl_add_u64 v[22:23], %[stride], 0, v[22:23]\n\t" \
+  "v_lshl_add_u64 v[22:23], %[rstride], 0, v[22:23]\n\t" \
   "s_add_i32 s36, s36, 1\n\t" \
   "s_cmp_ge_i32 s36, %[n]\n\t" \
   "s_cbranch_scc1 9f\n\t" \
   "global_store_dword v[22:23], v114, off nt\n\t" \
-  "v_lshl_add_u64 v[22:23], %[stride], 0, v[22:23]\n\t" \
+  "v_lshl_add_u64 v[22:23], %[rstride], 0, v[22:23]\n\t" \
   "s_add_i32 s36, s36, 1\n\t" \
   "s_cmp_ge_i32 s36, %[n]\n\t" \
   "s_cbranch_scc1 9f\n\t" \
   "global_store_dword v[22:23], v116, off nt\n\t" \
-  "v_lshl_add_u64 v[22:23], %[stride], 0, v[22:23]\n\t" \
+  "v_lshl_add_u64 v[22:23], %[rstride], 0, v[22:23]\n\t" \
   "s_add_i32 s36, s36, 1\n\t" \
   "s_cmp_ge_i32 s36, %[n]\n\t" \
   "s_cbranch_scc1 9f\n\t" \
   "global_store_dword v[22:23], v118, off nt\n\t" \
-  "v_lshl_add_u64 v[22:23], %[stride], 0, v[22:23]\n\t" \
+  "v_lshl_add_u64 v[22:23], %[rstride], 0, v[22:23]\n\t" \
   "s_add_i32 s36, s36, 1\n\t" \
   "s_cmp_ge_i32 s36, %[n]\n\t" \
   "s_cbranch_scc1 9f\n\t" \
   "global_store_dword v[22:23], v120, off nt\n\t" \
-  "v_lshl_add_u64 v[22:23], %[stride], 0, v[22:23]\n\t" \
+  "v_lshl_add_u64 v[22:23], %[rstride], 0, v[22:23]\n\t" \
   "s_add_i32 s36, s36, 1\n\t" \
   "s_cmp_ge_i32 s36, %[n]\n\t" \
   "s_cbranch_scc1 9f\n\t" \
   "global_store_dword v[22:23], v122, off nt\n\t" \
-  "v_lshl_add_u64 v[22:23], %[stride], 0, v[22:23]\n\t" \
+  "v_lshl_add_u64 v[22:23], %[rstride], 0, v[22:23]\n\t" \
   "s_add_i32 s36, s36, 1\n\t" \
   "s_cmp_ge_i32 s36, %[n]\n\t" \
   "s_cbranch_scc1 9f\n\t" \
   "global_store_dword v[22:23], v124, off nt\n\t" \
-  "v_lshl_add_u64 v[22:23], %[stride], 0, v[22:23]\n\t" \
+  "v_lshl_add_u64 v[22:23], %[rstride], 0, v[22:23]\n\t" \
   "s_add_i32 s36, s36, 1\n\t" \
   "s_cmp_ge_i32 s36, %[n]\n\t" \
   "s_cbranch_scc1 9f\n\t" \
   "global_store_dword v[22:23], v126, off nt\n\t" \
-  "v_lshl_add_u64 v[22:23], %[stride], 0, v[22:23]\n\t" \
+  "v_lshl_add_u64 v[22:23], %[rstride], 0, v[22:23]\n\t" \
   "s_add_i32 s36, s36, 1\n\t" \
   "9:\n\t"
 
@@ -7642,6 +7644,66 @@
   "v_mov_b32 v126, 0\n\t" \
   "v_mov_b32 v127, 0\n\t"
 
+#define TL_ASM_PARTIAL \
+  "v_lshrrev_b32 v24, 3, %[lane8]\n\t" \
+  "v_lshrrev_b32 v25, 5, v24\n\t" \
+  "v_and_b32 v24, 31, v24\n\t" \
+  "v_lshlrev_b32 v24, 4, v24\n\t" \
+  "s_lshr_b32 s94, %[m0wave], 10\n\t" \
+  "v_add_u32 v25, s94, v25\n\t" \
+  "s_and_b32 s95, %[nfull], 1\n\t" \
+  "s_lshl_b32 s95, s95, 10\n\t" \
+  "s_add_u32 s95, s95, %[m0wave]\n\t" \
+  "v_add_u32 v26, 0, v25\n\t" \
+  "v_min_u32 v26, %[plast], v26\n\t" \
+  "v_mul_lo_u32 v26, v26, %[rowb]\n\t" \
+  "v_add3_u32 v26, v26, %[poff], v24\n\t" \
+  "s_mov_b32 m0, s95\n\t" \
+  "s_add_u32 s95, s95, 0x8000\n\t" \
+  "buffer_load_dwordx4 v26, %[srd], 0 offen lds\n\t" \
+  "v_add_u32 v27, 32, v25\n\t" \
+  "v_min_u32 v27, %[plast], v27\n\t" \
+  "v_mul_lo_u32 v27, v27, %[rowb]\n\t" \
+  "v_add3_u32 v27, v27, %[poff], v24\n\t" \
+  "s_mov_b32 m0, s95\n\t" \
+  "s_add_u32 s95, s95, 0x8000\n\t" \
+  "buffer_load_dwordx4 v27, %[srd], 0 offen lds\n\t" \
+  "v_add_u32 v28, 64, v25\n\t" \
+  "v_min_u32 v28, %[plast], v28\n\t" \
+  "v_mul_lo_u32 v28, v28, %[rowb]\n\t" \
+  "v_add3_u32 v28, v28, %[poff], v24\n\t" \
+  "s_mov_b32 m0, s95\n\t" \
+  "s_add_u32 s95, s95, 0x8000\n\t" \
+  "buffer_load_dwordx4 v28, %[srd], 0 offen lds\n\t" \
+  "v_add_u32 v29, 96, v25\n\t" \
+  "v_min_u32 v29, %[plast], v29\n\t" \
+  "v_mul_lo_u32 v29, v29, %[rowb]\n\t" \
+  "v_add3_u32 v29, v29, %[poff], v24\n\t" \
+  "s_mov_b32 m0, s95\n\t" \
+  "s_add_u32 s95, s95, 0x8000\n\t" \
+  "buffer_load_dwordx4 v29, %[srd], 0 offen lds\n\t" \
+  "v_add_u32 v30, 128, v25\n\t" \
+  "v_min_u32 v30, %[plast], v30\n\t" \
+  "v_mul_lo_u32 v30, v30, %[rowb]\n\t" \
+  "v_add3_u32 v30, v30, %[poff], v24\n\t" \
+  "s_mov_b32 m0, s95\n\t" \
+  "s_add_u32 s95, s95, 0x8000\n\t" \
+  "buffer_load_dwordx4 v30, %[srd], 0 offen lds\n\t"
+
+#define TL_ASM_BEGIN "s_cmp_eq_u32 %[nfull], 0\n\t" "s_cbranch_scc1 55f\n\t" TL_ASM_TILE0 "s_branch 56f\n\t" "55:\n\t" "s_cmp_eq_u32 %[haspart], 0\n\t" "s_cbranch_scc1 56f\n\t" TL_ASM_PARTIAL "56:\n\t" "s_waitcnt vmcnt(0)\n\t" "s_barrier\n\t" "s_mov_b32 %[t0], 0\n\t"
+
+#define TL_ASM_CHUNK_HEAD "50:\n\t" "v_lshrrev_b32 v24, 3, %[lane8]\n\t" "v_add_u32 v24, %[t0], v24\n\t" "v_min_u32 v24, %[ntiles], v24\n\t" "v_lshlrev_b32 v24, 2, v24\n\t" "global_load_dword %[offreg], v24, %[myoff]\n\t" "s_mov_b32 %[obase], %[t0]\n\t" "s_add_u32 %[te], %[t0], 61\n\t" "s_min_u32 %[te], %[te], %[ntiles]\n\t" "s_sub_u32 s88, %[nfull], 1\n\t" "s_cmp_eq_u32 %[haspart], 0\n\t" "s_cbranch_scc1 52f\n\t" "s_cmp_lt_i32 %[t0], s88\n\t" "s_cbranch_scc0 52f\n\t" "s_cmp_lt_i32 s88, %[te]\n\t" "s_cbranch_scc0 52f\n\t" "s_mov_b32 %[te], s88\n\t" "52:\n\t" "s_waitcnt vmcnt(0)\n\t" "s_cmp_eq_u32 %[haspart], 0\n\t" "s_cbranch_scc1 51f\n\t" "s_cmp_eq_u32 %[t0], s88\n\t" "s_cbranch_scc0 51f\n\t" TL_ASM_PARTIAL "51:\n\t" "s_add_u32 s88, %[t0], 0\n\t" "s_min_u32 s88, s88, %[ntiles]\n\t" "s_sub_u32 s88, s88, %[obase]\n\t" "s_nop 3\n\t" "v_readlane_b32 %[o0], %[offreg], s88\n\t" "s_add_u32 s88, %[t0], 1\n\t" "s_min_u32 s88, s88, %[ntiles]\n\t" "s_sub_u32 s88, s88, %[obase]\n\t" "s_nop 3\n\t" "v_readlane_b32 %[o1], %[offreg], s88\n\t" "s_add_u32 s88, %[t0], 2\n\t" "s_min_u32 s88, s88, %[ntiles]\n\t" "s_sub_u32 s88, s88, %[obase]\n\t" "s_nop 3\n\t" "v_readlane_b32 %[o2], %[offreg], s88\n\t" "s_cmp_eq_u32 %[t0], 0\n\t" "s_cbranch_scc0 53f\n\t" "s_sub_u32 s88, %[o2], %[o0]\n\t" "v_lshrrev_b32 v24, 3, %[lane8]\n\t" "v_cmp_gt_u32 vcc, s88, v24\n\t" "v_cndmask_b32 v24, 0, v24, vcc\n\t" "v_lshlrev_b32 v24, 6, v24\n\t" "s_lshl_b32 s94, %[o0], 6\n\t" "s_lshr_b32 s95, %[o0], 26\n\t" "s_add_u32 s94, s94, %[blo]\n\t" "s_addc_u32 s95, s95, %[bhi]\n\t" "global_load_dword v23, v24, s[94:95]\n\t" "53:\n\t"
+
+#define TL_ASM_CHUNK_TAIL \
+  "s_mov_b32 %[t0], %[te]\n\t" \
+  "s_cmp_lt_u32 %[t0], %[ntiles]\n\t" \
+  "s_cbranch_scc1 50b\n\t" \
+  "s_waitcnt vmcnt(0) lgkmcnt(0)\n\t"
+
+#define TL_ASM_STORES "s_mov_b64 s[34:35], exec\n\t" "v_add_u32 v24, 8, %[lane8]\n\t" "v_cmp_ge_u32 vcc, %[lim], v24\n\t" "s_and_b64 exec, s[34:35], vcc\n\t" "s_cbranch_execz 60f\n\t" "s_cmp_eq_u32 %[mapped], 0\n\t" "s_cbranch_scc1 61f\n\t" TL_ASM_STORE_PERM "s_branch 60f\n\t" "61:\n\t" TL_ASM_STORE "60:\n\t" "s_mov_b64 exec, s[34:35]\n\t" "v_add_u32 v24, 4, %[lane8]\n\t" "v_cmp_eq_u32 vcc, %[lim], v24\n\t" "s_and_b64 exec, s[34:35], vcc\n\t" "s_cbranch_execz 62f\n\t" "s_cmp_eq_u32 %[mapped], 0\n\t" "s_cbranch_scc1 63f\n\t" TL_ASM_STORE1_PERM "s_branch 62f\n\t" "63:\n\t" TL_ASM_STORE1 "62:\n\t" "s_mov_b64 exec, s[34:35]\n\t"
+
+#define TL_ASM_STORES_F64 "s_mov_b64 s[34:35], exec\n\t" "v_add_u32 v24, 8, %[lane8]\n\t" "v_cmp_ge_u32 vcc, %[lim], v24\n\t" "s_and_b64 exec, s[34:35], vcc\n\t" "s_cbranch_execz 60f\n\t" "s_cmp_eq_u32 %[mapped], 0\n\t" "s_cbranch_scc1 61f\n\t" TL_ASM_STORE_PERM "s_branch 60f\n\t" "61:\n\t" TL_ASM_STORE "60:\n\t" "s_mov_b64 exec, s[34:35]\n\t"
+
 #define TL_CLOB_SGPR "s36", "s37", "s38", "s39", "s40", "s41", "s42", "s43", "s44", "s45", "s46", "s47", "s48", "s49", "s50", "s51", "s52", "s53", "s54", "s55", "s56", "s57", "s58", "s59", "s60", "s61", "s62", "s63", "s64", "s65", "s66", "s67", "s68", "s69", "s70", "s71", "s72", "s73", "s74", "s75", "s76", "s77", "s78", "s79", "s80", "s81", "s82", "s83", "s84", "s85", "s86", "s87", "s88", "s89", "s90", "s91", "s92", "s93", "s94", "s95"
 
 #define TL_CLOB_TMP "v22", "v23", "v24", "v25", "v26", "v27", "v28", "v29", "v30", "v31", "v32", "v33", "v34", "v35", "v36", "v37", "v38", "v39", "v40", "v41", "v42", "v43", "v44", "v45", "v46", "v47", "v48", "v49", "v50", "v51", "v52", "v53", "v54", "v55"
```

New measurement: 29900 GFLOP/s, median of 6. About the same (+0.1%).
